# aaichert/EpipolarConsistency

Hardware: AMD Instinct MI355X
Metric: ECC evaluations/sec (N=400, 1024^2 projections) (higher is better)
Workload: dtype f32

## Files before the change

epipolarconsistency_amd/_lib.py:

```python
import ctypes as C
import os

_HERE = os.path.dirname(os.path.abspath(__file__))
LIB_PATH = os.environ.get("ECC_HIP_LIB") or os.path.join(_HERE, "libecc_hip.so")

ECC_OK = 0
FILTER_DERIVATIVE, FILTER_RAMP, FILTER_NONE = 0, 1, 2
POST_IDENTITY, POST_SQUARE_ROOT, POST_LOGARITHM = 0, 1, 2
RADON_EXACT, RADON_FMA = 0, 1
SAMPLING_AUTO, SAMPLING_POLYNOMIAL, SAMPLING_PER_SAMPLE, SAMPLING_REFERENCE = 0, 1, 2, 3
LOSS_HUBER, LOSS_TRUNCATED, LOSS_GEMAN_MCCLURE = 0, 1, 2


class EccError(RuntimeError):
    def __init__(self, code, message):
        super().__init__("libecc_hip error %d: %s" % (code, message))
        self.code = code


class PreprocessConfig(C.Structure):
    _fields_ = [("process", C.c_int32), ("normalize", C.c_int32), ("bias", C.c_double), ("scale", C.c_double),
                ("apply_log", C.c_int32), ("gaussian_sigma", C.c_double), ("half_kernel_width", C.c_int32),
                ("flip_u", C.c_int32), ("flip_v", C.c_int32), ("zero", C.c_int32 * 4), ("feather", C.c_int32 * 4),
                ("n_blanks", C.c_int32), ("blanks", C.c_void_p)]


class LineWeightsConfig(C.Structure):
    _fields_ = [("dilate_px", C.c_int32), ("guard_bins", C.c_int32), ("zero_at_px", C.c_float)]


_lib = None

_vp, _i, _i64, _d = C.c_void_p, C.c_int, C.c_int64, C.c_double
_pi, _pd, _pf = C.POINTER(C.c_int), C.POINTER(C.c_double), C.POINTER(C.c_float)
SIGNATURES = {
    "ecc_last_error": (C.c_char_p, []),
    "ecc_version": (_i, []),
    "ecc_device_count": (_i, []),
    "ecc_ctx_create": (_i, [_i, _vp, C.POINTER(_vp)]),
    "ecc_ctx_destroy": (_i, [_vp]),
    "ecc_ctx_synchronize": (_i, [_vp]),
    "ecc_radon_compute": (_i, [_vp, _vp, _i, _i, _i, _i, _i, _i, _i, C.POINTER(_vp)]),
    "ecc_radon_compute_batch": (_i, [_vp, _vp, _i, _i, _i, _i, _i, _i, _i, _i, C.POINTER(_vp)]),
    "ecc_radon_compute_into": (_i, [_vp, _vp, _i, _i, _i, _i, _i, _i, _i, _vp]),
    "ecc_radon_set_arithmetic": (_i, [_vp, _i]),
    "ecc_radon_get_arithmetic": (_i, [_vp, _pi]),
    "ecc_radon_compute_linear": (_i, [_vp, _vp, _i, _i, _i, _i, _i, _i, _vp]),
    "ecc_dtr_from_device_linear": (_i, [_vp, _vp, _i, _i, _i, _i, _i, C.POINTER(_vp)]),
    "ecc_metric_evaluate_external": (_i, [_vp, _i, _vp, _vp, _i, _vp, _vp, _vp, C.c_float, C.c_float, _i]),
    "ecc_dtr_from_host": (_i, [_vp, _vp, _i, _i, _i, _i, _i, C.POINTER(_vp)]),
    "ecc_dtr_readback": (_i, [_vp, _vp]),
    "ecc_dtr_info": (_i, [_vp, _pi, _pi, _pi, _pi, _pi, _pd, _pd]),
    "ecc_dtr_device_view": (_i, [_vp, C.POINTER(_vp), _pi, _pi]),
    "ecc_dtr_slab_floats": (_i64, [_i, _i]),
    "ecc_dtr_wrap_device": (_i, [_vp, _vp, _i, _i, _i, _i, _i, C.POINTER(_vp)]),
    "ecc_dtr_destroy": (_i, [_vp]),
    "ecc_line_weights_defaults": (None, [_vp]),
    "ecc_radon_line_weights": (_i, [_vp, _vp, _i, _i, _i, _i, _i, _i, _vp, C.POINTER(_vp)]),
    "ecc_radon_line_weights_into": (_i, [_vp, _vp, _i, _i, _i, _i, _i, _vp, _vp]),
    "ecc_dtr_line_weights": (_i, [_vp, _vp, _vp, C.POINTER(_vp)]),
    "ecc_metric_create": (_i, [_vp, _i, C.POINTER(_vp), C.POINTER(_vp)]),
    "ecc_metric_destroy": (_i, [_vp]),
    "ecc_metric_refresh_dtrs": (_i, [_vp, _i, _i]),
    "ecc_metric_set_projections": (_i, [_vp, _vp, _i]),
    "ecc_metric_debug_geometry": (_i, [_vp, _vp, _vp]),
    "ecc_metric_set_params": (_i, [_vp, _d, _d, _i]),
    "ecc_metric_set_sampling": (_i, [_vp, _i]),
    "ecc_metric_set_incremental": (_i, [_vp, _i]),
    "ecc_metric_set_record_reuse": (_i, [_vp, _i]),
    "ecc_metric_set_small_eval": (_i, [_vp, _i]),
    "ecc_metric_set_host_join": (_i, [_vp, _i]),
    "ecc_metric_publish_scalar": (_i, [_vp, _vp]),
    "ecc_metric_wait_scalar": (_i, [_vp, _pd]),
    "ecc_metric_last_evaluated_pairs": (_i, [_vp, C.POINTER(_i64)]),
    "ecc_metric_device_bytes": (_i, [_vp, C.POINTER(_i64), C.POINTER(_i64), C.POINTER(_i64)]),
    "ecc_metric_get_object_radius": (_i, [_vp, _pd]),
    "ecc_metric_evaluate_all": (_i, [_vp, _vp, _pd]),
    "ecc_metric_evaluate_poses": (_i, [_vp, _i, _vp, _i, _vp]),
    "ecc_metric_evaluate_poses_strided": (_i, [_vp, _i, _vp, _i, _i, _i, _vp]),
    "ecc_metric_evaluate_pose_deltas": (_i, [_vp, _i, _vp, _vp, _vp, _vp]),
    "ecc_metric_set_pose_batching": (_i, [_vp, _i]),
    "ecc_metric_last_batched_poses": (_i, [_vp, C.POINTER(_i64)]),
    "ecc_metric_evaluate_gradient": (_i, [_vp, _i, _i, _vp, _vp, _vp, _vp, _vp, _vp]),
    "ecc_metric_last_gradient_path": (_i, [_vp, C.POINTER(_i)]),
    "ecc_metric_evaluate_gram": (_i, [_vp, _i, _vp, _vp]),
    "ecc_metric_evaluate_view_coefficients": (_i, [_vp, _i, _vp, _pd, _vp, _vp]),
    "ecc_metric_evaluate_view_hessian": (_i, [_vp, _i, _vp, _vp]),
    "ecc_metric_evaluate_weighted": (_i, [_vp, _pd, _pd, _vp]),
    "ecc_metric_evaluate_weighted_pairs": (_i, [_vp, _vp, _i, _pd, _pd, _vp]),
    "ecc_metric_evaluate_weighted_pose_deltas": (_i, [_vp, _i, _vp, _vp, _vp, _vp, _vp]),
    "ecc_metric_evaluate_transforms": (_i, [_vp, _i, _i, _vp, _vp, _vp]),
    "ecc_metric_evaluate_weighted_transforms": (_i, [_vp, _i, _i, _vp, _vp, _vp, _vp]),
    "ecc_metric_evaluate_robust": (_i, [_vp, _i, C.c_float, _pd, _pd, _vp]),
    "ecc_metric_evaluate_robust_pairs": (_i, [_vp, _vp, _i, _i, C.c_float, _pd, _pd, _vp]),
    "ecc_host_robust_scale": (_d, [_vp, _i64, _d]),
    "ecc_metric_evaluate_robust_map": (_i, [_vp, _i, C.c_float, _vp, _i, _vp, _vp, _pd, _pd, _vp]),
    "ecc_metric_evaluate_robust_map_pairs": (_i, [_vp, _vp, _i, _i, C.c_float, _vp, _i, _vp, _vp, _pd, _pd, _vp]),
    "ecc_metric_robust_map_weights": (_i, [_vp, C.c_float, C.c_float, _vp]),
    "ecc_debug_robust_map_fixed": (_i, [_vp, _vp, _i64]),
    "ecc_metric_evaluate_weighted_robust_map": (_i, [_vp, _i, C.c_float, _vp, _i, _vp, _vp, _pd, _pd, _pd, _vp]),
    "ecc_metric_evaluate_weighted_robust_map_pairs": (_i, [_vp, _vp, _i, _i, C.c_float, _vp, _i, _vp, _vp, _pd, _pd, _pd, _vp]),
    "ecc_metric_weighted_robust_map_weights": (_i, [_vp, C.c_float, C.c_float, _vp]),
    "ecc_metric_evaluate_weighted_robust": (_i, [_vp, _i, C.c_float, _pd, _pd, _pd, _vp]),
    "ecc_metric_evaluate_weighted_robust_pairs": (_i, [_vp, _vp, _i, _i, C.c_float, _pd, _pd, _pd, _vp]),
    "ecc_host_weighted_robust_scale": (_d, [_vp, _i64, _d]),
    "ecc_metric_evaluate_robust_pose_deltas": (_i, [_vp, _i, _vp, _vp, _vp, _i, C.c_float, _vp, _vp]),
    "ecc_metric_evaluate_robust_transforms": (_i, [_vp, _i, _i, _vp, _i, C.c_float, _vp, _vp, _vp]),
    "ecc_metric_last_batched_transforms": (_i, [_vp, C.POINTER(_i64)]),
    "ecc_host_compose_transform": (None, [_vp, _vp, _vp]),
    "ecc_metric_evaluate_range": (_i, [_vp, _i64, _i64, _vp, _pd]),
    "ecc_metric_evaluate_range_async": (_i, [_vp, _i64, _i64, _vp, _vp]),
    "ecc_metric_evaluate_pairs": (_i, [_vp, _vp, _i, _vp, _pd]),
    "ecc_metric_debug_K01": (_i, [_vp, _i64, _i64, _vp]),
    "ecc_metric_debug_polynomials": (_i, [_vp, _i64, _i64, _vp]),
    "ecc_metric_pair_samples_bound": (_i, [_vp, _pi]),
    "ecc_metric_evaluate_for_image_pair": (_i, [_vp, _i, _i, _i, _pi, _vp, _vp, _vp, _vp, _vp, _vp, _pd]),
    "ecc_get_ij": (None, [_i64, _i, _pi, _pi]),
    "ecc_host_pinvT": (None, [_vp, _vp]),
    "ecc_host_source_position": (None, [_vp, _vp]),
    "ecc_host_object_radius": (_d, [_vp, _i, _i]),
    "ecc_direct_create": (_i, [_vp, _i, _vp, _i, _i, _i, C.POINTER(_vp)]),
    "ecc_direct_destroy": (_i, [_vp]),
    "ecc_direct_update_images": (_i, [_vp]),
    "ecc_direct_set_projections": (_i, [_vp, _vp, _i]),
    "ecc_direct_set_params": (_i, [_vp, _d, _d, _i]),
    "ecc_direct_get_object_radius": (_i, [_vp, _pd]),
    "ecc_direct_evaluate": (_i, [_vp, _vp, _pd]),
    "ecc_direct_lines_bound": (_i, [_vp, _pi]),
    "ecc_direct_evaluate_for_image_pair": (_i, [_vp, _i, _i, _i, _pi, _vp, _vp, _vp, _vp, _pd]),
    "ecc_direct_evaluate_for_image_pair_kappas": (_i, [_vp, _i, _i, _i, _vp, _vp, _vp, _vp, _pd]),
    "ecc_preprocess_defaults": (None, [_vp]),
    "ecc_preprocess": (_i, [_vp, _vp, _i, _vp, _i, _i, _i, _vp, _vp]),
    "ecc_host_intrinsics": (None, [_vp, _pf, _pf, _pf]),
    "ecc_host_angular_range": (None, [_vp, _vp, _d, _pd, _pd]),
    "ecc_host_angular_step": (_d, [_vp, _vp, _i, _i]),
    "ecc_host_iso_center": (None, [_vp, _i, _vp]),
    "ecc_host_line_to_sample_dtr": (_i, [_vp, C.c_float]),
    "ecc_group_create": (_i, [_i, _vp, C.POINTER(_vp)]),
    "ecc_group_destroy": (_i, [_vp]),
    "ecc_group_size": (_i, [_vp]),
    "ecc_group_ctx": (_i, [_vp, _i, C.POINTER(_vp)]),
    "ecc_group_radon_compute_batch": (_i, [_vp, _vp, _i, _i, _i, _i, _i, _i, _i, C.POINTER(_vp)]),
    "ecc_pair_shard": (None, [_i64, _i, _i, C.POINTER(_i64), C.POINTER(_i64)]),
    "ecc_pair_shards_balanced": (_i, [_vp, _i, _d, _i, _vp]),
    "ecc_metric_balanced_shards": (_i, [_vp, _i, _vp]),
    "ecc_comm_available": (_i, []),
    "ecc_comm_unique_id": (_i, [_vp]),
    "ecc_comm_create": (_i, [_vp, _vp, _i, _i, _vp]),
    "ecc_comm_destroy": (_i, [_vp]),
    "ecc_metric_evaluate_range_allreduce": (_i, [_vp, _vp, _i64, _i64, _vp]),
    "ecc_group_metric_rebalance": (_i, [_vp]),
    "ecc_group_metric_evaluate_poses": (_i, [_vp, _i, _vp, _i, _vp]),
    "ecc_group_metric_create": (_i, [_vp, _i, C.POINTER(_vp), C.POINTER(_vp)]),
    "ecc_group_debug_force_replica": (_i, [_i]),
    "ecc_group_metric_destroy": (_i, [_vp]),
    "ecc_group_metric_set_projections": (_i, [_vp, _vp, _i]),
    "ecc_group_metric_set_params": (_i, [_vp, _d, _d, _i]),
    "ecc_group_metric_set_sampling": (_i, [_vp, _i]),
    "ecc_group_metric_set_incremental": (_i, [_vp, _i]),
    "ecc_group_metric_get_object_radius": (_i, [_vp, _pd]),
    "ecc_group_metric_evaluate_all": (_i, [_vp, _vp, _pd]),
    "ecc_group_metric_rank_metric": (_i, [_vp, _i, C.POINTER(_vp)]),
    "ecc_exchange_open": (_i, [C.c_char_p, _i, _i, C.POINTER(C.c_void_p)]),
    "ecc_exchange_sum": (_i, [_vp, _d, _pd]),
    "ecc_exchange_close": (_i, [_vp]),
    "ecc_debug_set_poly_tolerance": (_i, [_vp, C.c_float]),
    "ecc_debug_set_small_eval_bound": (_i, [_vp, _i64]),
    "ecc_debug_set_result_polling": (_i, [_i]),
    "ecc_debug_set_quad_copies": (_i, [_vp, _i]),
    "ecc_debug_set_gradient_launch": (_i, [_vp, _i]),
    "ecc_ctx_set_quad_copies": (_i, [_vp, _i]),
    "ecc_debug_small_stamps": (_i, [_vp, _i]),
    "ecc_debug_step_stamps": (_i, [_vp, _vp]),
    "ecc_ctx_enable_timing": (_i, [_vp, _i]),
    "ecc_ctx_last_kernel_ms": (_i, [_vp, _i, _pf]),
}


def lib():
    global _lib
    if _lib is None:
        if not os.path.exists(LIB_PATH):
            raise ImportError(
                "%s is missing: build it with `python -m epipolarconsistency_amd.build` "
                "(hipcc, gfx950). There is no CPU fallback." % LIB_PATH)
        if not os.environ.get("ECC_NO_TORCH_PRELOAD"):
            try:
                import torch
                if torch.cuda.is_available():
                    torch.cuda.init()
            except ImportError:
                pass
        L = C.CDLL(LIB_PATH)
        for name, (res, args) in SIGNATURES.items():
            f = getattr(L, name)
            f.restype = res
            f.argtypes = args
        _lib = L
    return _lib


def check(code):
    if code != ECC_OK:
        raise EccError(code, lib().ecc_last_error().decode("utf-8", "replace"))
```

epipolarconsistency_amd/api.py:

```python
import ctypes as C

import numpy as np

from . import _lib
from ._lib import (FILTER_DERIVATIVE, FILTER_NONE, FILTER_RAMP, POST_IDENTITY, POST_LOGARITHM,
                   POST_SQUARE_ROOT, EccError, check)


def pack_projection_matrices(Ps):
    return _Ps_colmajor(Ps)


def _Ps_colmajor(Ps):
    A = np.asarray(Ps, dtype=np.float64).reshape(-1, 3, 4)
    return np.ascontiguousarray(A.transpose(0, 2, 1)).reshape(-1, 12)


def _is_torch(x):
    return type(x).__module__.startswith("torch")


class Context:

    def __init__(self, device=0, stream=None):
        self._h = C.c_void_p()
        check(_lib.lib().ecc_ctx_create(int(device), C.c_void_p(stream or 0), C.byref(self._h)))
        self.device = int(device)

    def synchronize(self):
        check(_lib.lib().ecc_ctx_synchronize(self._h))

    def enable_timing(self, on=True):
        check(_lib.lib().ecc_ctx_enable_timing(self._h, 1 if on else 0))

    def last_kernel_ms(self, which):
        ms = C.c_float()
        check(_lib.lib().ecc_ctx_last_kernel_ms(self._h, {"pairs": 0, "radon": 1, "preprocess": 2}[which], C.byref(ms)))
        return ms.value

    def debugSetQuadCopies(self, on=True):
        check(_lib.lib().ecc_debug_set_quad_copies(self._h, 1 if on else 0))
        return self

    def setQuadCopies(self, mode="auto"):
        check(_lib.lib().ecc_ctx_set_quad_copies(self._h, {"auto": -1, "off": 0, "on": 1}[mode]))
        return self

    def setRadonArithmetic(self, mode="exact"):
        check(_lib.lib().ecc_radon_set_arithmetic(self._h, {"exact": _lib.RADON_EXACT, "fma": _lib.RADON_FMA}[mode]))
        return self

    def getRadonArithmetic(self):
        v = C.c_int()
        check(_lib.lib().ecc_radon_get_arithmetic(self._h, C.byref(v)))
        return {_lib.RADON_EXACT: "exact", _lib.RADON_FMA: "fma"}[v.value]

    def close(self):
        if self._h:
            _lib.lib().ecc_ctx_destroy(self._h)
            self._h = C.c_void_p()

    def __del__(self):
        try:
            self.close()
        except Exception:
            pass


class PreProccess:

    class _NS:
        def __init__(self, **kw):
            self.__dict__.update(kw)

    def __init__(self):
        self.intensity = self._NS(normalize=False, bias=0.0, scale=1.0, apply_log=False)
        self.lowpass = self._NS(gaussian_sigma=1.84, half_kernel_width=5)
        self.image_geometry = self._NS(flip_u=False, flip_v=False)
        self.border = self._NS(zero=[1, 1, 1, 1], feather=[16, 16, 16, 16], blanks=[])

    def _config(self, process=True):
        cfg = _lib.PreprocessConfig()
        _lib.lib().ecc_preprocess_defaults(C.byref(cfg))
        cfg.process = 1 if process else 0
        cfg.normalize, cfg.bias, cfg.scale = int(self.intensity.normalize), self.intensity.bias, self.intensity.scale
        cfg.apply_log = int(self.intensity.apply_log)
        cfg.gaussian_sigma, cfg.half_kernel_width = self.lowpass.gaussian_sigma, int(self.lowpass.half_kernel_width)
        cfg.flip_u, cfg.flip_v = int(self.image_geometry.flip_u), int(self.image_geometry.flip_v)
        cfg.zero = (C.c_int32 * 4)(*[int(v) for v in self.border.zero])
        cfg.feather = (C.c_int32 * 4)(*[int(v) for v in self.border.feather])
        bl = np.ascontiguousarray(np.asarray(self.border.blanks, np.int32).reshape(-1, 4))
        cfg.n_blanks = len(bl)
        cfg.blanks = bl.ctypes.data if len(bl) else None
        return cfg, bl

    def _run(self, ctx, images, Ps, out, process):
        cfg, keep = self._config(process)
        Pp = None if Ps is None else _Ps_colmajor(Ps)
        if _is_torch(images):
            import torch
            assert images.dtype == torch.float32 and images.is_contiguous() and images.is_cuda and images.dim() == 3
            out = images if out is None else out
            assert out.shape == images.shape and out.is_contiguous() and out.is_cuda
            n, n_v, n_u = images.shape
            a, b, on_dev = images.data_ptr(), out.data_ptr(), 1
        else:
            images = np.ascontiguousarray(images, np.float32)
            assert images.ndim == 3
            out = np.empty_like(images) if out is None else out
            n, n_v, n_u = images.shape
            a, b, on_dev = images.ctypes.data, out.ctypes.data, 0
        assert Pp is None or len(Pp) == n
        check(_lib.lib().ecc_preprocess(ctx._h, C.c_void_p(a), on_dev, C.c_void_p(b), n, n_u, n_v, C.byref(cfg),
                                        C.c_void_p(Pp.ctypes.data) if Pp is not None else None))
        del keep
        return out

    def process(self, ctx, images, Ps=None, out=None):
        return self._run(ctx, images, Ps, out, True)

    def apply_weight_cos_principal_ray(self, ctx, images, Ps, out=None):
        return self._run(ctx, images, Ps, out, False)


class RadonIntermediate:
    Derivative, Ramp, None_ = FILTER_DERIVATIVE, FILTER_RAMP, FILTER_NONE
    Identity, SquareRoot, Logarithm = POST_IDENTITY, POST_SQUARE_ROOT, POST_LOGARITHM

    def __init__(self, ctx, handle):
        self.ctx = ctx
        self._h = handle
        self._keep = None

    @classmethod
    def compute(cls, ctx, image, size_alpha, size_t, filter=FILTER_DERIVATIVE, post_process=POST_IDENTITY):
        return cls.compute_batch(ctx, image[None] if not _is_torch(image) else image.unsqueeze(0),
                                 size_alpha, size_t, filter, post_process)[0]

    @classmethod
    def compute_batch(cls, ctx, images, size_alpha, size_t, filter=FILTER_DERIVATIVE, post_process=POST_IDENTITY):
        if _is_torch(images):
            import torch
            assert images.dtype == torch.float32 and images.is_contiguous() and images.is_cuda
            n, n_v, n_u = images.shape
            ptr, on_dev, keep = images.data_ptr(), 1, images
        else:
            keep = np.ascontiguousarray(images, np.float32)
            n, n_v, n_u = keep.shape
            ptr, on_dev = keep.ctypes.data, 0
        hs = (C.c_void_p * n)()
        check(_lib.lib().ecc_radon_compute_batch(ctx._h, C.c_void_p(ptr), on_dev, n, n_u, n_v, size_alpha,
                                                 size_t, filter, post_process, hs))
        if on_dev:
            ctx.synchronize()
        return [cls(ctx, C.c_void_p(h)) for h in hs]

    @classmethod
    def compute_into(cls, ctx, images, slabs, size_alpha, size_t, filter=FILTER_DERIVATIVE,
                     post_process=POST_IDENTITY):
        n, n_v, n_u = images.shape
        assert images.is_contiguous() and slabs.is_contiguous()
        assert slabs.shape[0] == n and slabs.shape[1] == slab_floats(size_alpha, size_t)
        check(_lib.lib().ecc_radon_compute_into(ctx._h, C.c_void_p(images.data_ptr()), n, n_u, n_v, size_alpha,
                                                size_t, filter, post_process, C.c_void_p(slabs.data_ptr())))
        return [cls.wrap_device(ctx, slabs[k], size_alpha, size_t, n_u, n_v, filter) for k in range(n)]

    @classmethod
    def from_host(cls, ctx, data, n_u, n_v, filter=FILTER_DERIVATIVE):
        data = np.ascontiguousarray(data, np.float32)
        n_t, n_alpha = data.shape
        h = C.c_void_p()
        check(_lib.lib().ecc_dtr_from_host(ctx._h, C.c_void_p(data.ctypes.data), n_alpha, n_t, n_u, n_v, filter,
                                           C.byref(h)))
        return cls(ctx, h)

    @classmethod
    def line_weights_from(cls, lengths_dtr, zero_at_px=1.0, guard_bins=1, ctx=None):
        ctx = lengths_dtr.ctx if ctx is None else ctx
        cfg = _line_weights_config(zero_at_px, guard_bins, 0)
        h = C.c_void_p()
        check(_lib.lib().ecc_dtr_line_weights(ctx._h, lengths_dtr._h, C.byref(cfg), C.byref(h)))
        return cls(ctx, h)

    @classmethod
    def load(cls, ctx, path):
        from . import nrrd
        data, info = nrrd.read_dtr(path)
        return cls.from_host(ctx, data, info["n_u"], info["n_v"], info["filter"]), info

    def save(self, path, projection_matrix=None):
        from . import nrrd
        nrrd.write_dtr(path, self.readback(), self.getOriginalImageSize(0), self.getOriginalImageSize(1),
                       self.getFilter(), projection_matrix)

    @classmethod
    def wrap_device(cls, ctx, slab, n_alpha, n_t, n_u, n_v, filter=FILTER_DERIVATIVE):
        h = C.c_void_p()
        check(_lib.lib().ecc_dtr_wrap_device(ctx._h, C.c_void_p(slab.data_ptr()), n_alpha, n_t, n_u, n_v, filter,
                                             C.byref(h)))
        r = cls(ctx, h)
        r._keep = slab
        return r

    def _info(self):
        a, t, u, v, f = (C.c_int() for _ in range(5))
        ba, bd = C.c_double(), C.c_double()
        check(_lib.lib().ecc_dtr_info(self._h, C.byref(a), C.byref(t), C.byref(u), C.byref(v), C.byref(f),
                                      C.byref(ba), C.byref(bd)))
        return a.value, t.value, u.value, v.value, f.value, ba.value, bd.value

    def getRadonBinNumber(self, dim):
        a, t = self._info()[:2]
        return t if dim else a

    def getOriginalImageSize(self, dim):
        u, v = self._info()[2:4]
        return v if dim else u

    def getRadonBinSize(self, dim=1):
        ba, bd = self._info()[5:7]
        return bd if dim else ba

    def getFilter(self):
        return self._info()[4]

    def isDerivative(self):
        return self.getFilter() == FILTER_DERIVATIVE

    def readback(self):
        a, t = self._info()[:2]
        out = np.empty((t, a), np.float32)
        check(_lib.lib().ecc_dtr_readback(self._h, C.c_void_p(out.ctypes.data)))
        self._raw_cpu = out
        return out

    def clearRawData(self):
        self._raw_cpu = None

    def data(self):
        return getattr(self, "_raw_cpu", None)

    def replaceRadonIntermediateData(self, radon_intermediate_image):
        a = np.ascontiguousarray(radon_intermediate_image, np.float32)
        assert a.ndim == 2
        info = self._info()
        fresh = RadonIntermediate.from_host(self.ctx, a, info[2], info[3], filter=info[4])
        self.close()
        self._h, fresh._h = fresh._h, C.c_void_p()
        self._keep = None
        self._raw_cpu = a.copy()

    def tex2D(self, s, t):
        raw = self.data()
        if raw is None:
            raise ValueError("call readback() first")
        n_t, n_alpha = raw.shape
        x, y = (n_alpha - 1) * float(np.float32(s)), (n_t - 1) * float(np.float32(t))

        def cell(v, n):
            i = int(v)
            f = v - i
            if i < 0:
                i, f = 0, 0.0
            if i > n - 2:
                i, f = n - 2, 1.0
            return i, f
        ix, fx = cell(x, n_alpha)
        iy, fy = cell(y, n_t)
        if fx == 0 and fy == 0:
            return float(np.float32(raw[iy, ix]))
        r = ((1.0 - fy) * ((1.0 - fx) * float(raw[iy, ix]) + fx * float(raw[iy, ix + 1]))
             + fy * ((1.0 - fx) * float(raw[iy + 1, ix]) + fx * float(raw[iy + 1, ix + 1])))
        return float(np.float32(r))

    def sample(self, line):
        l = np.ascontiguousarray(line, np.float32).reshape(3).copy()
        range_t = np.float32(self.getRadonBinSize(1)) * np.float32(self.getRadonBinNumber(1))
        folded = _lib.lib().ecc_host_line_to_sample_dtr(C.c_void_p(l.ctypes.data), C.c_float(float(range_t)))
        try:
            line[:3] = l
        except TypeError:
            pass
        v = self.tex2D(l[0], l[1])
        return -v if (folded and self.isDerivative()) else v

    def device_view(self):
        base, pitch, rows = C.c_void_p(), C.c_int(), C.c_int()
        check(_lib.lib().ecc_dtr_device_view(self._h, C.byref(base), C.byref(pitch), C.byref(rows)))
        return base.value, pitch.value, rows.value

    def close(self):
        if self._h and self.ctx._h:
            _lib.lib().ecc_dtr_destroy(self._h)
        self._h = C.c_void_p()

    def __del__(self):
        try:
            self.close()
        except Exception:
            pass


def _pack_pose_lists(moved_views, moved_Ps):
    off = [0]
    views = []
    rows = []
    for vk, Pk in zip(moved_views, moved_Ps):
        vk = [int(v) for v in np.atleast_1d(vk)]
        Pk = np.asarray(Pk, np.float64)
        Pk = Pk.reshape(len(vk), 12) if (Pk.shape[-1] == 12 and Pk.ndim <= 2) else _Ps_colmajor(Pk)
        views += vk
        rows.append(Pk)
        off.append(len(views))
    flat = np.concatenate(rows) if rows and len(views) else np.zeros((0, 12))
    return off, views, flat


def _check_pose_lists(moved_offsets, moved_views, moved_Ps):
    off = np.ascontiguousarray(moved_offsets, np.int32)
    views = np.ascontiguousarray(moved_views, np.int32)
    flat = np.ascontiguousarray(moved_Ps, np.float64).reshape(-1, 12)
    if len(off) < 1 or int(off[-1]) != len(views) or len(flat) != len(views):
        raise ValueError("moved_offsets / moved_views / moved_Ps disagree")
    return off, views, flat


def _ptr(a):
    return C.c_void_p(a.ctypes.data) if (a is not None and a.size) else None


def _idx4_list(idx4):
    idx = np.ascontiguousarray(idx4, np.int32)
    if idx.size % 4 or (idx.ndim == 2 and idx.shape[1] != 4) or idx.ndim > 2:
        raise ValueError("idx4 must hold (P0, P1, D0, D1) tuples")
    return idx.reshape(-1, 4)


def _transforms_colmajor(Ts):
    T = np.asarray(Ts, dtype=np.float64)
    if T.ndim == 2 and T.shape == (4, 4):
        T = T[None]
    if T.ndim != 3 or T.shape[1:] != (4, 4):
        raise ValueError("Ts must be (K, 4, 4)")
    return np.ascontiguousarray(T.transpose(0, 2, 1)).reshape(-1, 16)


def _with_pairs(results, pairs, want_pairs):
    return results + (pairs,) if want_pairs else results


def _pose_lists_call(fn, handle, moved_offsets, moved_views, moved_Ps, extra, n_results):
    off, views, flat = _check_pose_lists(moved_offsets, moved_views, moved_Ps)
    results = tuple(np.zeros(len(off) - 1, np.float64) for _ in range(n_results))
    check(fn(handle, len(off) - 1, C.c_void_p(off.ctypes.data), _ptr(views), _ptr(flat), *extra,
             *[C.c_void_p(r.ctypes.data) for r in results]))
    return results


class MetricRadonIntermediate:

    def __init__(self, ctx, Ps=None, dtrs=None):
        self.ctx = ctx
        self._h = C.c_void_p()
        self._dtrs = []
        self._Ps = None
        self._params = [0.0, 0.0, 0]
        d = type(self).default_sampling
        self._sampling = 0 if d is None else (self._SAMPLING[d] if isinstance(d, str) else int(d))
        self._incremental = False
        self._record_reuse = None
        self._small_eval = None
        self._host_join = None
        self._debug = {}
        self._ptr_cache = {}
        self._mean = C.c_double()
        self._mean_ref = C.byref(self._mean)
        if dtrs is not None:
            self.setRadonIntermediates(dtrs)
        if Ps is not None:
            self.setProjectionMatrices(Ps)

    def setRadonIntermediates(self, dtrs):
        if self._h:
            _lib.lib().ecc_metric_destroy(self._h)
            self._h = C.c_void_p()
        self._dtrs = list(dtrs)
        hs = (C.c_void_p * len(self._dtrs))(*[d._h for d in self._dtrs])
        check(_lib.lib().ecc_metric_create(self.ctx._h, len(self._dtrs), hs, C.byref(self._h)))
        check(_lib.lib().ecc_metric_set_params(self._h, *self._params))
        check(_lib.lib().ecc_metric_set_sampling(self._h, self._sampling))
        check(_lib.lib().ecc_metric_set_incremental(self._h, int(self._incremental)))
        if self._record_reuse is not None:
            check(_lib.lib().ecc_metric_set_record_reuse(self._h, int(self._record_reuse)))
        if self._small_eval is not None:
            check(_lib.lib().ecc_metric_set_small_eval(self._h, int(self._small_eval)))
        if self._host_join is not None:
            check(_lib.lib().ecc_metric_set_host_join(self._h, int(self._host_join)))
        self._apply_debug()
        if self._Ps is not None:
            self.setProjectionMatrices(self._Ps)
        return self

    def _apply_debug(self):
        if "poly_tolerance" in self._debug:
            check(_lib.lib().ecc_debug_set_poly_tolerance(self._h, float(self._debug["poly_tolerance"])))
        if "small_eval_bound" in self._debug:
            check(_lib.lib().ecc_debug_set_small_eval_bound(self._h, int(self._debug["small_eval_bound"])))
        if "gradient_launch" in self._debug:
            check(_lib.lib().ecc_debug_set_gradient_launch(self._h, int(self._debug["gradient_launch"])))

    def debugSetGradientLaunch(self, on=True):
        self._debug["gradient_launch"] = 1 if on else 0
        if self._h:
            self._apply_debug()
        return self

    def debugSetPolyTolerance(self, tol_bins):
        self._debug["poly_tolerance"] = float(tol_bins)
        if self._h:
            self._apply_debug()
        return self

    def debugSetSmallEvalBound(self, max_pairs):
        self._debug["small_eval_bound"] = int(max_pairs)
        if self._h:
            self._apply_debug()
        return self

    def getRadonIntermediates(self):
        return self._dtrs

    def refreshRadonIntermediates(self, first=0, count=None):
        count = len(self._dtrs) - first if count is None else count
        check(_lib.lib().ecc_metric_refresh_dtrs(self._h, int(first), int(count)))
        return self

    def setProjectionMatrices(self, Ps):
        hit = self._ptr_cache.get(id(Ps))
        if hit is not None and hit[0] is Ps and hit[2] == Ps.shape:
            self._Ps = Ps
            if self._h:
                check(_lib.lib().ecc_metric_set_projections(self._h, hit[1], hit[2][0]))
            return self
        if isinstance(Ps, np.ndarray) and Ps.ndim == 2 and Ps.shape[1] == 12 and Ps.dtype == np.float64 \
                and Ps.flags["C_CONTIGUOUS"]:
            self._Ps = Ps
            if len(self._ptr_cache) >= 1024:
                self._ptr_cache.clear()
            self._ptr_cache[id(Ps)] = (Ps, C.c_void_p(Ps.ctypes.data), Ps.shape)
        else:
            self._Ps = _Ps_colmajor(Ps)
        if self._h:
            check(_lib.lib().ecc_metric_set_projections(self._h, C.c_void_p(self._Ps.ctypes.data), len(self._Ps)))
        return self

    def getProjectionMatrices(self):
        return [] if self._Ps is None else [p.reshape(4, 3).T.copy() for p in self._Ps]

    def getNumberOfProjetions(self):
        return 0 if self._Ps is None else len(self._Ps)

    def _push_params(self):
        if self._h:
            check(_lib.lib().ecc_metric_set_params(self._h, *self._params))

    def setObjectRadius(self, radius_mm=0.0):
        self._params[0] = float(radius_mm)
        self._push_params()
        return self

    def getObjectRadius(self):
        r = C.c_double()
        check(_lib.lib().ecc_metric_get_object_radius(self._h, C.byref(r)))
        return r.value

    def setEpipolarPlaneStep(self, dkappa_rad=0.0):
        self._params[1] = float(dkappa_rad)
        self._push_params()
        return self

    setdKappa = setEpipolarPlaneStep

    def useCorrelation(self, corr=True):
        self._params[2] = 1 if corr else 0
        self._push_params()
        return self

    default_sampling = None
    _SAMPLING = {"auto": 0, "polynomial": 1, "per_sample": 2, "reference": 3}

    def setSampling(self, mode="auto"):
        self._sampling = self._SAMPLING[mode] if isinstance(mode, str) else int(mode)
        if self._h:
            check(_lib.lib().ecc_metric_set_sampling(self._h, self._sampling))
        return self

    def setIncremental(self, enable=True):
        self._incremental = bool(enable)
        if self._h:
            check(_lib.lib().ecc_metric_set_incremental(self._h, int(self._incremental)))
        return self

    def setRecordReuse(self, on=True, always=False):
        self._record_reuse = (2 if always else 1) if on else 0
        if self._h:
            check(_lib.lib().ecc_metric_set_record_reuse(self._h, int(self._record_reuse)))
        return self

    def setSmallEval(self, on=True):
        self._small_eval = 1 if on else 0
        if self._h:
            check(_lib.lib().ecc_metric_set_small_eval(self._h, self._small_eval))
        return self

    def setHostJoin(self, on=True):
        self._host_join = 1 if on else 0
        if self._h:
            check(_lib.lib().ecc_metric_set_host_join(self._h, self._host_join))
        return self

    def device_bytes(self):
        a, b, c = C.c_int64(0), C.c_int64(0), C.c_int64(0)
        check(_lib.lib().ecc_metric_device_bytes(self._h, C.byref(a), C.byref(b), C.byref(c)))
        return {"paired_copies": a.value, "quad_copies": b.value, "other": c.value}

    def last_evaluated_pairs(self):
        v = C.c_int64()
        check(_lib.lib().ecc_metric_last_evaluated_pairs(self._h, C.byref(v)))
        return v.value

    def evaluate(self, arg=None, out=None):
        L = _lib.lib()
        if arg is None:
            check(L.ecc_metric_evaluate_all(self._h, None, self._mean_ref))
            return self._mean.value
        mean = C.c_double()
        if arg is None or (isinstance(arg, np.ndarray) and arg.dtype == np.float32 and arg.ndim == 2
                           and out is None and arg.shape[0] == arg.shape[1] == self.getNumberOfProjetions()):
            cost = arg
            if cost is not None and not cost.flags["C_CONTIGUOUS"]:
                raise ValueError("cost image must be C-contiguous float32")
            check(L.ecc_metric_evaluate_all(self._h, C.c_void_p(cost.ctypes.data if cost is not None else 0),
                                            C.byref(mean)))
            return mean.value
        if isinstance(arg, (set, frozenset)):
            views = sorted(arg)
            idx = [(a, b, a, b) for k, a in enumerate(views) for b in views[k + 1:]]
        else:
            idx = arg
        hit_i, hit_o = self._ptr_cache.get(id(idx)), self._ptr_cache.get(id(out))
        if hit_i is not None and hit_o is not None and hit_i[0] is idx and hit_o[0] is out and hit_i[2] == idx.shape \
                and hit_o[2] == out.shape:
            check(L.ecc_metric_evaluate_pairs(self._h, hit_i[1], hit_i[2][0], hit_o[1], self._mean_ref))
            return self._mean.value
        cacheable = isinstance(idx, np.ndarray) and idx.dtype == np.int32 and idx.ndim == 2 and idx.shape[1] == 4 \
            and idx.flags["C_CONTIGUOUS"] and isinstance(out, np.ndarray) and out.flags["C_CONTIGUOUS"]
        idx0 = idx
        idx = np.ascontiguousarray(idx, np.int32).reshape(-1, 4)
        if out is None:
            out = np.empty(len(idx), np.float32)
        assert out.dtype == np.float32 and out.size >= len(idx)
        pi, po = C.c_void_p(idx.ctypes.data), C.c_void_p(out.ctypes.data)
        if cacheable:
            if len(self._ptr_cache) >= 1024:
                self._ptr_cache.clear()
            self._ptr_cache[id(idx0)] = (idx0, pi, idx0.shape)
            self._ptr_cache[id(out)] = (out, po, out.shape)
        check(L.ecc_metric_evaluate_pairs(self._h, pi, len(idx), po, C.byref(mean)))
        return mean.value

    def evaluate_poses(self, poses, first=0, stride=1):
        if isinstance(poses, np.ndarray) and poses.ndim == 3 and poses.shape[2] == 12 and poses.dtype == np.float64 \
                and poses.flags["C_CONTIGUOUS"]:
            flat = poses
        else:
            flat = np.ascontiguousarray(np.stack([p if (isinstance(p, np.ndarray) and p.ndim == 2 and p.shape[1] == 12)
                                                  else _Ps_colmajor(p) for p in poses]), np.float64)
        means = np.zeros(len(flat), np.float64)
        check(_lib.lib().ecc_metric_evaluate_poses_strided(self._h, len(flat), C.c_void_p(flat.ctypes.data), flat.shape[1],
                                                           int(first), int(stride), C.c_void_p(means.ctypes.data)))
        mine = range(int(first), len(flat), int(stride))
        if len(mine):
            self._Ps = flat[mine[-1]]
        return means

    def evaluate_pose_deltas(self, moved_views, moved_Ps):
        return self.evaluate_pose_deltas_packed(*_pack_pose_lists(moved_views, moved_Ps))

    def evaluate_pose_deltas_packed(self, moved_offsets, moved_views, moved_Ps):
        return _pose_lists_call(_lib.lib().ecc_metric_evaluate_pose_deltas, self._h, moved_offsets, moved_views, moved_Ps, (), 1)[0]

    def evaluate_weighted_pose_deltas(self, moved_views, moved_Ps):
        return self.evaluate_weighted_pose_deltas_packed(*_pack_pose_lists(moved_views, moved_Ps))

    def evaluate_weighted_pose_deltas_packed(self, moved_offsets, moved_views, moved_Ps):
        return _pose_lists_call(_lib.lib().ecc_metric_evaluate_weighted_pose_deltas, self._h, moved_offsets, moved_views, moved_Ps, (), 2)

    def evaluate_robust_pose_deltas(self, moved_views, moved_Ps, loss, delta):
        return self.evaluate_robust_pose_deltas_packed(*_pack_pose_lists(moved_views, moved_Ps), loss, delta)

    def evaluate_robust_pose_deltas_packed(self, moved_offsets, moved_views, moved_Ps, loss, delta):
        return _pose_lists_call(_lib.lib().ecc_metric_evaluate_robust_pose_deltas, self._h, moved_offsets, moved_views, moved_Ps,
                                (int(loss), float(delta)), 2)

    def evaluate_weighted_pairs(self, idx4, want_pairs=False):
        idx = _idx4_list(idx4)
        value, coverage = C.c_double(0.0), C.c_double(0.0)
        pairs = np.zeros((len(idx), 2), np.float32) if want_pairs else None
        check(_lib.lib().ecc_metric_evaluate_weighted_pairs(self._h, _ptr(idx), len(idx),
                                                            C.byref(value), C.byref(coverage),
                                                            _ptr(pairs)))
        return _with_pairs((value.value, coverage.value), pairs, want_pairs)

    def setPoseBatching(self, on=True):
        check(_lib.lib().ecc_metric_set_pose_batching(self._h, 1 if on else 0))
        return self

    def last_batched_poses(self):
        v = C.c_int64(0)
        check(_lib.lib().ecc_metric_last_batched_poses(self._h, C.byref(v)))
        return v.value

    def evaluate_gradient(self, view, Ps_plus, Ps_minus, h, want_probes=False):
        def rows(Ps):
            Ps = np.asarray(Ps, np.float64)
            return np.ascontiguousarray(Ps.reshape(-1, 12) if (Ps.shape[-1] == 12 and Ps.ndim <= 2) else _Ps_colmajor(Ps))
        plus, minus = rows(Ps_plus), rows(Ps_minus)
        h = np.ascontiguousarray(np.atleast_1d(h), np.float64)
        p = len(h)
        if p < 1 or len(plus) != p or len(minus) != p:
            raise ValueError("Ps_plus / Ps_minus / h disagree")
        value = C.c_double(0.0)
        grad, probes = np.zeros(p, np.float64), np.zeros(2 * p, np.float64)
        check(_lib.lib().ecc_metric_evaluate_gradient(self._h, int(view), p, C.c_void_p(plus.ctypes.data), C.c_void_p(minus.ctypes.data),
                                                      C.c_void_p(h.ctypes.data), C.byref(value), C.c_void_p(grad.ctypes.data),
                                                      C.c_void_p(probes.ctypes.data) if want_probes else None))
        return (value.value, grad, probes) if want_probes else (value.value, grad)

    def evaluate_gradient_rigid(self, view, steps, want_probes=False):
        from .geometry import compose_transform, rigid_transform
        steps = np.asarray(steps, np.float64)
        if steps.shape != (6,):
            raise ValueError("steps: (tx, ty, tz, rx, ry, rz)")
        if self._Ps is None or not 0 <= int(view) < len(self._Ps):
            raise ValueError("view outside the projection matrices")
        P = self._Ps[int(view)].reshape(4, 3).T
        names = ("tx", "ty", "tz", "rx", "ry", "rz")
        plus = [compose_transform(P, rigid_transform(**{names[k]: steps[k]})) for k in range(6)]
        minus = [compose_transform(P, rigid_transform(**{names[k]: -steps[k]})) for k in range(6)]
        return self.evaluate_gradient(view, plus, minus, steps, want_probes)

    def last_gradient_path(self):
        v = C.c_int(0)
        check(_lib.lib().ecc_metric_last_gradient_path(self._h, C.byref(v)))
        return v.value

    def evaluate_gram(self, n_channels, want_pairs=False):
        K = int(n_channels)
        n = 0 if self._Ps is None else len(self._Ps)
        G = np.zeros((max(K, 0), max(K, 0)), np.float64)
        pairs = np.zeros((n * (n - 1) // 2, max(K, 0) * (max(K, 0) + 1) // 2), np.float32) if want_pairs else None
        check(_lib.lib().ecc_metric_evaluate_gram(self._h, K, _ptr(pairs),
                                                  C.c_void_p(G.ctypes.data) if G.size else None))
        return (G, pairs) if want_pairs else G

    def evaluate_view_coefficients(self, coeffs, want_pairs=False):
        a = np.ascontiguousarray(coeffs, np.float32)
        if a.ndim != 2:
            raise ValueError("coeffs must be (n_channels, n_views)")
        K, n = a.shape
        if self._Ps is not None and n != len(self._Ps):
            raise ValueError("coeffs must be (n_channels, n_views)")
        value = C.c_double(0.0)
        grad = np.zeros((K, n), np.float64)
        pairs = np.zeros((n * (n - 1) // 2, 1 + 2 * K), np.float32) if want_pairs else None
        check(_lib.lib().ecc_metric_evaluate_view_coefficients(self._h, K, C.c_void_p(a.ctypes.data) if a.size else None, C.byref(value),
                                                               C.c_void_p(grad.ctypes.data) if grad.size else None,
                                                               _ptr(pairs)))
        return (value.value, grad, pairs) if want_pairs else (value.value, grad)

    def evaluate_view_hessian(self, n_channels, want_pairs=False, want_matrix=True):
        if not want_pairs and not want_matrix:
            raise ValueError("nothing asked for: want_matrix or want_pairs")
        K = int(n_channels)
        n = 0 if self._Ps is None else len(self._Ps)
        Kp = max(K, 0)
        H = np.zeros((n * Kp, n * Kp) if n * Kp else (1, 1), np.float64) if want_matrix else None
        blocks = None
        if want_pairs:
            blocks = np.zeros((n * (n - 1) // 2, Kp * (Kp + 1) + Kp * Kp) if n > 1 and Kp else (1, 1), np.float64)
        check(_lib.lib().ecc_metric_evaluate_view_hessian(self._h, K, C.c_void_p(H.ctypes.data) if want_matrix else None,
                                                          C.c_void_p(blocks.ctypes.data) if want_pairs else None))
        return (H, blocks) if (want_pairs and want_matrix) else (H if want_matrix else blocks)

    def evaluate_weighted(self, want_pairs=False):
        n = 0 if self._Ps is None else len(self._Ps)
        value, coverage = C.c_double(0.0), C.c_double(0.0)
        pairs = np.zeros((n * (n - 1) // 2, 2), np.float32) if want_pairs else None
        check(_lib.lib().ecc_metric_evaluate_weighted(self._h, C.byref(value), C.byref(coverage),
                                                      _ptr(pairs)))
        return _with_pairs((value.value, coverage.value), pairs, want_pairs)

    def evaluate_robust(self, loss, delta, want_pairs=False):
        n = 0 if self._Ps is None else len(self._Ps)
        value, mass = C.c_double(0.0), C.c_double(0.0)
        pairs = np.zeros((n * (n - 1) // 2, 3), np.float32) if want_pairs else None
        check(_lib.lib().ecc_metric_evaluate_robust(self._h, int(loss), float(delta), C.byref(value), C.byref(mass),
                                                    _ptr(pairs)))
        return _with_pairs((value.value, mass.value), pairs, want_pairs)

    def evaluate_robust_pairs(self, idx4, loss, delta, want_pairs=False):
        idx = _idx4_list(idx4)
        value, mass = C.c_double(0.0), C.c_double(0.0)
        pairs = np.zeros((len(idx), 3), np.float32) if want_pairs else None
        check(_lib.lib().ecc_metric_evaluate_robust_pairs(self._h, _ptr(idx), len(idx),
                                                          int(loss), float(delta), C.byref(value), C.byref(mass),
                                                          _ptr(pairs)))
        return _with_pairs((value.value, mass.value), pairs, want_pairs)

    def _robust_map_views(self, views):
        if views is None:
            return None, len(self._dtrs)
        v = np.ascontiguousarray(views, np.int32).reshape(-1)
        if len(v) == 0:
            raise ValueError("views: None for every view, or at least one index")
        return v, len(v)

    def _robust_map_planes(self, k):
        n_alpha, n_t = (self._dtrs[0].getRadonBinNumber(0), self._dtrs[0].getRadonBinNumber(1)) if self._dtrs else (0, 0)
        return np.zeros((k, n_t, n_alpha), np.float32), np.zeros((k, n_t, n_alpha), np.float32)

    def evaluate_robust_map(self, loss, delta, views=None, want_pairs=False):
        n = 0 if self._Ps is None else len(self._Ps)
        v, k = self._robust_map_views(views)
        if views is None:
            k = n
        hits, rejected = self._robust_map_planes(k)
        value, mass = C.c_double(0.0), C.c_double(0.0)
        pairs = np.zeros((n * (n - 1) // 2, 3), np.float32) if want_pairs else None
        check(_lib.lib().ecc_metric_evaluate_robust_map(self._h, int(loss), float(delta), _ptr(v), 0 if v is None else len(v),
                                                        _ptr(hits), _ptr(rejected), C.byref(value), C.byref(mass), _ptr(pairs)))
        self._robust_map_count = k
        return _with_pairs((value.value, mass.value, hits, rejected), pairs, want_pairs)

    def evaluate_robust_map_pairs(self, idx4, loss, delta, views=None, want_pairs=False):
        idx = _idx4_list(idx4)
        v, k = self._robust_map_views(views)
        hits, rejected = self._robust_map_planes(k)
        value, mass = C.c_double(0.0), C.c_double(0.0)
        pairs = np.zeros((len(idx), 3), np.float32) if want_pairs else None
        check(_lib.lib().ecc_metric_evaluate_robust_map_pairs(self._h, _ptr(idx), len(idx), int(loss), float(delta), _ptr(v),
                                                              0 if v is None else len(v), _ptr(hits), _ptr(rejected), C.byref(value),
                                                              C.byref(mass), _ptr(pairs)))
        self._robust_map_count = k
        return _with_pairs((value.value, mass.value, hits, rejected), pairs, want_pairs)

    def robust_map_weights(self, min_hits=1.0, gain=1.0):
        k = getattr(self, "_robust_map_count", 0)
        hs = (C.c_void_p * max(k, 1))()
        check(_lib.lib().ecc_metric_robust_map_weights(self._h, float(min_hits), float(gain), hs))
        return [RadonIntermediate(self.ctx, C.c_void_p(h)) for h in hs[:k]]

    def robust_map_fixed(self):
        k = getattr(self, "_robust_map_count", 0)
        n_alpha, n_t = self._dtrs[0].getRadonBinNumber(0), self._dtrs[0].getRadonBinNumber(1)
        pitch = slab_floats(n_alpha, n_t) // (n_alpha + 2)
        raw = np.zeros((2 * max(k, 1), n_alpha + 2, pitch), np.uint64)
        check(_lib.lib().ecc_debug_robust_map_fixed(self._h, _ptr(raw), raw.size))
        q = raw[:, :, :n_t + 2].copy()
        q[:, 1] += q[:, 0]
        q[:, -2] += q[:, -1]
        q[:, :, 1] += q[:, :, 0]
        q[:, :, -2] += q[:, :, -1]
        bins = np.ascontiguousarray(q[:2 * k, 1:-1, 1:-1].transpose(0, 2, 1))
        return bins[:k], bins[k:]

    def _weighted_map_views(self, views):
        if views is None:
            return None, len(self._dtrs) // 2
        return self._robust_map_views(views)

    def evaluate_weighted_robust_map(self, loss, delta, views=None, want_pairs=False):
        n = 0 if self._Ps is None else len(self._Ps)
        v, k = self._weighted_map_views(views)
        hits, rejected = self._robust_map_planes(k)
        value, coverage, mass = C.c_double(0.0), C.c_double(0.0), C.c_double(0.0)
        pairs = np.zeros((n * (n - 1) // 2, 4), np.float32) if want_pairs else None
        check(_lib.lib().ecc_metric_evaluate_weighted_robust_map(self._h, int(loss), float(delta), _ptr(v), 0 if v is None else len(v),
                                                                 _ptr(hits), _ptr(rejected), C.byref(value), C.byref(coverage),
                                                                 C.byref(mass), _ptr(pairs)))
        self._robust_map_count = k
        return _with_pairs((value.value, coverage.value, mass.value, hits, rejected), pairs, want_pairs)

    def evaluate_weighted_robust_map_pairs(self, idx4, loss, delta, views=None, want_pairs=False):
        idx = _idx4_list(idx4)
        v, k = self._weighted_map_views(views)
        hits, rejected = self._robust_map_planes(k)
        value, coverage, mass = C.c_double(0.0), C.c_double(0.0), C.c_double(0.0)
        pairs = np.zeros((len(idx), 4), np.float32) if want_pairs else None
        check(_lib.lib().ecc_metric_evaluate_weighted_robust_map_pairs(self._h, _ptr(idx), len(idx), int(loss), float(delta), _ptr(v),
                                                                       0 if v is None else len(v), _ptr(hits), _ptr(rejected),
                                                                       C.byref(value), C.byref(coverage), C.byref(mass), _ptr(pairs)))
        self._robust_map_count = k
        return _with_pairs((value.value, coverage.value, mass.value, hits, rejected), pairs, want_pairs)

    def weighted_robust_map_weights(self, min_hits=1.0, gain=1.0):
        k = getattr(self, "_robust_map_count", 0)
        hs = (C.c_void_p * max(k, 1))()
        check(_lib.lib().ecc_metric_weighted_robust_map_weights(self._h, float(min_hits), float(gain), hs))
        return [RadonIntermediate(self.ctx, C.c_void_p(h)) for h in hs[:k]]

    def evaluate_weighted_robust(self, loss, delta, want_pairs=False):
        n = 0 if self._Ps is None else len(self._Ps)
        value, coverage, mass = C.c_double(0.0), C.c_double(0.0), C.c_double(0.0)
        pairs = np.zeros((n * (n - 1) // 2, 4), np.float32) if want_pairs else None
        check(_lib.lib().ecc_metric_evaluate_weighted_robust(self._h, int(loss), float(delta), C.byref(value), C.byref(coverage), C.byref(mass),
                                                             _ptr(pairs)))
        return _with_pairs((value.value, coverage.value, mass.value), pairs, want_pairs)

    def evaluate_weighted_robust_pairs(self, idx4, loss, delta, want_pairs=False):
        idx = _idx4_list(idx4)
        value, coverage, mass = C.c_double(0.0), C.c_double(0.0), C.c_double(0.0)
        pairs = np.zeros((len(idx), 4), np.float32) if want_pairs else None
        check(_lib.lib().ecc_metric_evaluate_weighted_robust_pairs(self._h, _ptr(idx), len(idx),
                                                                   int(loss), float(delta), C.byref(value), C.byref(coverage), C.byref(mass),
                                                                   _ptr(pairs)))
        return _with_pairs((value.value, coverage.value, mass.value), pairs, want_pairs)

    def evaluate_transforms(self, n_source, Ts, want_pairs=False):
        flat = _transforms_colmajor(Ts)
        n_source = int(n_source)
        K, n = len(flat), self.getNumberOfProjetions()
        means = np.zeros(K, np.float64)
        pairs = np.zeros((K, max(n - n_source, 0), max(n_source, 0)), np.float32) if want_pairs else None
        check(_lib.lib().ecc_metric_evaluate_transforms(self._h, n_source, K, C.c_void_p(flat.ctypes.data if K else 0),
                                                        C.c_void_p(means.ctypes.data if K else 0),
                                                        _ptr(pairs)))
        return (means, pairs) if want_pairs else means

    def evaluate_weighted_transforms(self, n_source, Ts, want_pairs=False):
        flat = _transforms_colmajor(Ts)
        n_source = int(n_source)
        K, n = len(flat), self.getNumberOfProjetions()
        values, coverages = np.zeros(K, np.float64), np.zeros(K, np.float64)
        pairs = np.zeros((K, max(n - n_source, 0), max(n_source, 0), 2), np.float32) if want_pairs else None
        check(_lib.lib().ecc_metric_evaluate_weighted_transforms(self._h, n_source, K, C.c_void_p(flat.ctypes.data if K else 0),
                                                                 C.c_void_p(values.ctypes.data if K else 0),
                                                                 C.c_void_p(coverages.ctypes.data if K else 0),
                                                                 _ptr(pairs)))
        return _with_pairs((values, coverages), pairs, want_pairs)

    def evaluate_robust_transforms(self, n_source, Ts, loss, delta, want_pairs=False):
        flat = _transforms_colmajor(Ts)
        n_source = int(n_source)
        K, n = len(flat), self.getNumberOfProjetions()
        values, masses = np.zeros(K, np.float64), np.zeros(K, np.float64)
        pairs = np.zeros((K, max(n - n_source, 0), max(n_source, 0), 3), np.float32) if want_pairs else None
        check(_lib.lib().ecc_metric_evaluate_robust_transforms(self._h, n_source, K, C.c_void_p(flat.ctypes.data if K else 0),
                                                               int(loss), float(delta),
                                                               C.c_void_p(values.ctypes.data if K else 0),
                                                               C.c_void_p(masses.ctypes.data if K else 0),
                                                               _ptr(pairs)))
        return _with_pairs((values, masses), pairs, want_pairs)

    def last_batched_transforms(self):
        v = C.c_int64(0)
        check(_lib.lib().ecc_metric_last_batched_transforms(self._h, C.byref(v)))
        return v.value

    def evaluateForImagePair(self, i, j):
        L = _lib.lib()
        cap = C.c_int()
        check(L.ecc_metric_pair_samples_bound(self._h, C.byref(cap)))
        cap = cap.value
        s0, s1, kap = (np.empty(cap, np.float32) for _ in range(3))
        r0, r1 = np.empty((cap, 2), np.float32), np.empty((cap, 2), np.float32)
        K01 = np.empty(16, np.float32)
        n, ecc = C.c_int(), C.c_double()
        check(L.ecc_metric_evaluate_for_image_pair(
            self._h, int(i), int(j), cap, C.byref(n), C.c_void_p(s0.ctypes.data), C.c_void_p(s1.ctypes.data),
            C.c_void_p(kap.ctypes.data), C.c_void_p(r0.ctypes.data), C.c_void_p(r1.ctypes.data),
            C.c_void_p(K01.ctypes.data), C.byref(ecc)))
        n = n.value
        return ecc.value, dict(redundant_samples0=s0[:n], redundant_samples1=s1[:n], kappas=kap[:n],
                               radon_samples0=r0[:n], radon_samples1=r1[:n], K01=K01)

    def balanced_shards(self, world):
        b = np.zeros(int(world) + 1, np.int64)
        check(_lib.lib().ecc_metric_balanced_shards(self._h, int(world), C.c_void_p(b.ctypes.data)))
        return [int(v) for v in b]

    def evaluate_range(self, first, count, want_pairs=False):
        s = C.c_double()
        vals = np.empty(count, np.float32) if want_pairs else None
        check(_lib.lib().ecc_metric_evaluate_range(self._h, int(first), int(count),
                                                   C.c_void_p(vals.ctypes.data if want_pairs else 0), C.byref(s)))
        return (s.value, vals) if want_pairs else s.value

    def evaluate_range_allreduce(self, comm, first, count):
        check(_lib.lib().ecc_metric_evaluate_range_allreduce(self._h, comm._h, int(first), int(count), self._mean_ref))
        return self._mean.value

    def evaluate_range_async(self, first, count, sum_tensor, pair_tensor=None):
        check(_lib.lib().ecc_metric_evaluate_range_async(
            self._h, int(first), int(count), C.c_void_p(pair_tensor.data_ptr() if pair_tensor is not None else 0),
            C.c_void_p(sum_tensor.data_ptr())))

    def publish_scalar(self, value_tensor):
        check(_lib.lib().ecc_metric_publish_scalar(self._h, C.c_void_p(value_tensor.data_ptr())))

    def wait_scalar(self):
        v = C.c_double()
        check(_lib.lib().ecc_metric_wait_scalar(self._h, C.byref(v)))
        return v.value

    def debug_geometry(self):
        n = self.getNumberOfProjetions()
        PinvTs, Cs = np.empty((n, 12), np.float32), np.empty((n, 4), np.float32)
        check(_lib.lib().ecc_metric_debug_geometry(self._h, C.c_void_p(PinvTs.ctypes.data), C.c_void_p(Cs.ctypes.data)))
        return PinvTs, Cs

    def debug_K01(self, first, count):
        out = np.empty((count, 16), np.float32)
        check(_lib.lib().ecc_metric_debug_K01(self._h, int(first), int(count), C.c_void_p(out.ctypes.data)))
        return out

    def debug_polynomials(self, first, count):
        n = 4 + 2 * 13 + 2 * 12
        out = np.empty((count, n), np.float32)
        check(_lib.lib().ecc_metric_debug_polynomials(self._h, int(first), int(count), C.c_void_p(out.ctypes.data)))
        return [dict(poly_ok=bool(r[0]), degree=int(r[0]), clamp_free=bool(r[0] != int(r[0])), x_scale=float(r[1]), fold=r[2:4] > 0, ca=r[4:30].reshape(2, 13).astype(np.float64),
                     cd=r[30:54].reshape(2, 12).astype(np.float64)) for r in out]

    def close(self):
        if self._h and self.ctx._h:
            _lib.lib().ecc_metric_destroy(self._h)
        self._h = C.c_void_p()

    def __del__(self):
        try:
            self.close()
        except Exception:
            pass


class _BorrowedContext:

    def __init__(self, handle, device, group):
        self._h, self.device, self._group = handle, device, group

    def synchronize(self):
        check(_lib.lib().ecc_ctx_synchronize(self._h))

    def close(self):
        self._h = C.c_void_p()


class Group:

    def __init__(self, devices):
        devices = [int(d) for d in devices]
        arr = (C.c_int * len(devices))(*devices)
        self._h = C.c_void_p()
        check(_lib.lib().ecc_group_create(len(devices), arr, C.byref(self._h)))
        self.devices = devices
        self._ctxs = {}

    def __len__(self):
        return _lib.lib().ecc_group_size(self._h)

    def context(self, rank):
        if rank not in self._ctxs:
            h = C.c_void_p()
            check(_lib.lib().ecc_group_ctx(self._h, int(rank), C.byref(h)))
            self._ctxs[rank] = _BorrowedContext(h, self.devices[rank], self)
        return self._ctxs[rank]

    def compute_batch(self, images, size_alpha, size_t, filter=FILTER_DERIVATIVE, post_process=POST_IDENTITY):
        keep = np.ascontiguousarray(images, np.float32)
        n, n_v, n_u = keep.shape
        hs = (C.c_void_p * n)()
        check(_lib.lib().ecc_group_radon_compute_batch(self._h, C.c_void_p(keep.ctypes.data), n, n_u, n_v, size_alpha,
                                                       size_t, filter, post_process, hs))
        chunk = (n + len(self.devices) - 1) // len(self.devices)
        ctxs = [self.context(r) for r in range(len(self.devices))]
        return [RadonIntermediate(ctxs[k // chunk], C.c_void_p(h)) for k, h in enumerate(hs)]

    def close(self):
        if self._h:
            for c in self._ctxs.values():
                c.close()
            self._ctxs = {}
            _lib.lib().ecc_group_destroy(self._h)
            self._h = C.c_void_p()

    def __del__(self):
        try:
            self.close()
        except Exception:
            pass


def pair_shard(n_pairs, world, rank):
    a, b = C.c_int64(), C.c_int64()
    _lib.lib().ecc_pair_shard(int(n_pairs), int(world), int(rank), C.byref(a), C.byref(b))
    return a.value, b.value


def pair_shards_balanced(Ps, object_radius_mm, world):
    if isinstance(Ps, np.ndarray) and Ps.ndim == 2 and Ps.shape[1] == 12:
        flat = np.ascontiguousarray(Ps, np.float64)
    else:
        flat = _Ps_colmajor(Ps)
    b = np.zeros(int(world) + 1, np.int64)
    check(_lib.lib().ecc_pair_shards_balanced(C.c_void_p(flat.ctypes.data), len(flat), float(object_radius_mm), int(world),
                                              C.c_void_p(b.ctypes.data)))
    return [int(v) for v in b]


class GroupMetricRadonIntermediate:

    def __init__(self, group, Ps=None, dtrs=None):
        self.group = group
        self._h = C.c_void_p()
        self._dtrs = []
        self._Ps = None
        if dtrs is not None:
            self.setRadonIntermediates(dtrs)
        if Ps is not None:
            self.setProjectionMatrices(Ps)

    def setRadonIntermediates(self, dtrs):
        self.close()
        self._dtrs = list(dtrs)
        hs = (C.c_void_p * len(self._dtrs))(*[d._h for d in self._dtrs])
        check(_lib.lib().ecc_group_metric_create(self.group._h, len(self._dtrs), hs, C.byref(self._h)))
        d = MetricRadonIntermediate.default_sampling
        if d is not None:
            self.setSampling(d)
        if self._Ps is not None:
            self.setProjectionMatrices(self._Ps)
        return self

    def setProjectionMatrices(self, Ps):
        if isinstance(Ps, np.ndarray) and Ps.ndim == 2 and Ps.shape[1] == 12 and Ps.dtype == np.float64 \
                and Ps.flags["C_CONTIGUOUS"]:
            self._Ps = Ps
        else:
            self._Ps = _Ps_colmajor(Ps)
        if self._h:
            check(_lib.lib().ecc_group_metric_set_projections(self._h, C.c_void_p(self._Ps.ctypes.data), len(self._Ps)))
        return self

    def getNumberOfProjetions(self):
        return 0 if self._Ps is None else len(self._Ps)

    def setObjectRadius(self, radius_mm=0.0, dkappa=0.0, use_corr=False):
        check(_lib.lib().ecc_group_metric_set_params(self._h, float(radius_mm), float(dkappa), 1 if use_corr else 0))
        return self

    def getObjectRadius(self):
        r = C.c_double()
        check(_lib.lib().ecc_group_metric_get_object_radius(self._h, C.byref(r)))
        return r.value

    def setSampling(self, mode="auto"):
        mode = MetricRadonIntermediate._SAMPLING[mode] if isinstance(mode, str) else int(mode)
        check(_lib.lib().ecc_group_metric_set_sampling(self._h, mode))
        return self

    def setIncremental(self, enable=True):
        check(_lib.lib().ecc_group_metric_set_incremental(self._h, int(bool(enable))))
        return self

    def last_evaluated_pairs(self):
        total = 0
        for r in range(len(self.group)):
            m, v = C.c_void_p(), C.c_int64()
            check(_lib.lib().ecc_group_metric_rank_metric(self._h, r, C.byref(m)))
            check(_lib.lib().ecc_metric_last_evaluated_pairs(m, C.byref(v)))
            total += v.value
        return total

    def evaluate_poses(self, poses):
        flat = np.ascontiguousarray(np.stack([p if (isinstance(p, np.ndarray) and p.ndim == 2 and p.shape[1] == 12)
                                              else _Ps_colmajor(p) for p in poses]), np.float64)
        means = np.zeros(len(flat), np.float64)
        check(_lib.lib().ecc_group_metric_evaluate_poses(self._h, len(flat), C.c_void_p(flat.ctypes.data), flat.shape[1],
                                                         C.c_void_p(means.ctypes.data)))
        return means

    def rebalance(self):
        check(_lib.lib().ecc_group_metric_rebalance(self._h))
        return self

    def evaluate(self, cost=None):
        mean = C.c_double()
        if cost is not None:
            n = self.getNumberOfProjetions()
            assert cost.dtype == np.float32 and cost.flags["C_CONTIGUOUS"] and cost.shape == (n, n)
        check(_lib.lib().ecc_group_metric_evaluate_all(self._h, C.c_void_p(cost.ctypes.data if cost is not None else 0),
                                                       C.byref(mean)))
        return mean.value

    def close(self):
        if self._h and self.group._h:
            _lib.lib().ecc_group_metric_destroy(self._h)
        self._h = C.c_void_p()

    def __del__(self):
        try:
            self.close()
        except Exception:
            pass


class MetricDirect:

    def __init__(self, ctx, Ps, images):
        self.ctx = ctx
        self._h = C.c_void_p()
        self._params = [0.0, 0.0, 0]
        self._Ps = None
        self.setProjectionImages(images)
        if Ps is not None:
            self.setProjectionMatrices(Ps)

    def setProjectionImages(self, images):
        if self._h:
            _lib.lib().ecc_direct_destroy(self._h)
            self._h = C.c_void_p()
        if _is_torch(images):
            import torch
            assert images.dtype == torch.float32 and images.is_contiguous() and images.is_cuda and images.dim() == 3
            self._keep, ptr, on_dev = images, images.data_ptr(), 1
        else:
            self._keep = np.ascontiguousarray(images, np.float32)
            assert self._keep.ndim == 3
            ptr, on_dev = self._keep.ctypes.data, 0
        n, n_v, n_u = self._keep.shape
        self._n = n
        check(_lib.lib().ecc_direct_create(self.ctx._h, n, C.c_void_p(ptr), on_dev, n_u, n_v, C.byref(self._h)))
        check(_lib.lib().ecc_direct_set_params(self._h, *self._params))
        if self._Ps is not None:
            self.setProjectionMatrices(self._Ps)
        return self

    def setProjectionMatrices(self, Ps):
        self._Ps = _Ps_colmajor(Ps)
        check(_lib.lib().ecc_direct_set_projections(self._h, C.c_void_p(self._Ps.ctypes.data), len(self._Ps)))
        return self

    def getNumberOfProjetions(self):
        return self._n

    def updateImages(self):
        check(_lib.lib().ecc_direct_update_images(self._h))
        return self

    def _push(self):
        check(_lib.lib().ecc_direct_set_params(self._h, *self._params))
        return self

    def setObjectRadius(self, radius_mm=0.0):
        self._params[0] = float(radius_mm)
        return self._push()

    def getObjectRadius(self):
        r = C.c_double()
        check(_lib.lib().ecc_direct_get_object_radius(self._h, C.byref(r)))
        return r.value

    def setEpipolarPlaneStep(self, dkappa_rad=0.0):
        self._params[1] = float(dkappa_rad)
        return self._push()

    def setFanBeamConsistency(self, fbcc=True):
        self._params[2] = 1 if fbcc else 0
        return self._push()

    def evaluate(self, cost=None):
        s = C.c_double()
        if cost is not None:
            assert cost.dtype == np.float32 and cost.flags["C_CONTIGUOUS"] and cost.shape == (self._n, self._n)
        check(_lib.lib().ecc_direct_evaluate(self._h, C.c_void_p(cost.ctypes.data if cost is not None else 0), C.byref(s)))
        return s.value

    def evaluateForImagePair(self, i, j, kappas=None):
        L = _lib.lib()
        if kappas is not None:
            kap = np.ascontiguousarray(kappas, np.float32).reshape(-1)
            s0, s1, lines = np.empty(len(kap), np.float32), np.empty(len(kap), np.float32), np.empty((len(kap), 6), np.float32)
            m = C.c_double()
            check(L.ecc_direct_evaluate_for_image_pair_kappas(self._h, int(i), int(j), len(kap), C.c_void_p(kap.ctypes.data),
                                                              C.c_void_p(s0.ctypes.data), C.c_void_p(s1.ctypes.data),
                                                              C.c_void_p(lines.ctypes.data), C.byref(m)))
            return m.value, dict(redundant_samples0=s0, redundant_samples1=s1, kappas=kap, lines=lines)
        cap = C.c_int()
        check(L.ecc_direct_lines_bound(self._h, C.byref(cap)))
        cap = cap.value
        s0, s1, kap = (np.empty(cap, np.float32) for _ in range(3))
        lines = np.empty((cap, 6), np.float32)
        n, m = C.c_int(), C.c_double()
        check(L.ecc_direct_evaluate_for_image_pair(self._h, int(i), int(j), cap, C.byref(n), C.c_void_p(s0.ctypes.data),
                                                   C.c_void_p(s1.ctypes.data), C.c_void_p(kap.ctypes.data),
                                                   C.c_void_p(lines.ctypes.data), C.byref(m)))
        n = n.value
        return m.value, dict(redundant_samples0=s0[:n], redundant_samples1=s1[:n], kappas=kap[:n], lines=lines[:n])

    def close(self):
        if self._h and self.ctx._h:
            _lib.lib().ecc_direct_destroy(self._h)
        self._h = C.c_void_p()

    def __del__(self):
        try:
            self.close()
        except Exception:
            pass


def slab_floats(n_alpha, n_t):
    return _lib.lib().ecc_dtr_slab_floats(int(n_alpha), int(n_t))


def get_ij(ij, n):
    i, j = C.c_int(), C.c_int()
    _lib.lib().ecc_get_ij(int(ij), int(n), C.byref(i), C.byref(j))
    return i.value, j.value


def host_pinvT(P):
    P = np.ascontiguousarray(np.asarray(P, np.float64).reshape(3, 4).T).reshape(12)
    out = np.empty(12, np.float32)
    _lib.lib().ecc_host_pinvT(C.c_void_p(P.ctypes.data), C.c_void_p(out.ctypes.data))
    return out


def host_source_position(P):
    P = np.ascontiguousarray(np.asarray(P, np.float64).reshape(3, 4).T).reshape(12)
    out = np.empty(4, np.float32)
    _lib.lib().ecc_host_source_position(C.c_void_p(P.ctypes.data), C.c_void_p(out.ctypes.data))
    return out


def host_object_radius(P, n_u, n_v):
    P = np.ascontiguousarray(np.asarray(P, np.float64).reshape(3, 4).T).reshape(12)
    return _lib.lib().ecc_host_object_radius(C.c_void_p(P.ctypes.data), int(n_u), int(n_v))


def host_intrinsics(P):
    P = np.ascontiguousarray(np.asarray(P, np.float64).reshape(3, 4).T).reshape(12)
    a, b, c = C.c_float(), C.c_float(), C.c_float()
    _lib.lib().ecc_host_intrinsics(C.c_void_p(P.ctypes.data), C.byref(a), C.byref(b), C.byref(c))
    return a.value, b.value, c.value


def _P12(P):
    return np.ascontiguousarray(np.asarray(P, np.float64).reshape(3, 4).T).reshape(12)


def estimateAngularRange(P0, P1, object_radius_mm):
    a, b, A, B = C.c_double(), C.c_double(), _P12(P0), _P12(P1)
    _lib.lib().ecc_host_angular_range(C.c_void_p(A.ctypes.data), C.c_void_p(B.ctypes.data), float(object_radius_mm),
                                      C.byref(a), C.byref(b))
    return a.value, b.value


def estimateAngularStep(P0, P1, n_u, n_v):
    A, B = _P12(P0), _P12(P1)
    return _lib.lib().ecc_host_angular_step(C.c_void_p(A.ctypes.data), C.c_void_p(B.ctypes.data), int(n_u), int(n_v))


def estimateIsoCenter(Ps):
    flat = _Ps_colmajor(Ps)
    O = np.zeros(4)
    _lib.lib().ecc_host_iso_center(C.c_void_p(flat.ctypes.data), len(flat), C.c_void_p(O.ctypes.data))
    return O


estimateObjectRadius = host_object_radius


def gram_value(G, a):
    G = np.asarray(G, np.float64)
    a = np.asarray(a, np.float64).reshape(-1)
    if G.ndim != 2 or G.shape != (len(a), len(a)):
        raise ValueError("G must be (K, K) and a (K,)")
    return float(a @ (G @ a))


def gram_minimizer(G, fixed=0, value=1.0):
    G = np.asarray(G, np.float64)
    if G.ndim != 2 or G.shape[0] != G.shape[1] or G.shape[0] < 1:
        raise ValueError("G must be (K, K)")
    K = G.shape[0]
    fixed = int(fixed)
    if not 0 <= fixed < K:
        raise ValueError("fixed outside [0, K)")
    free = [c for c in range(K) if c != fixed]
    a = np.zeros(K, np.float64)
    a[fixed] = float(value)
    if free:
        H = 0.5 * (G[np.ix_(free, free)] + G[np.ix_(free, free)].T)
        np.linalg.cholesky(H)
        a[free] = np.linalg.solve(H, -float(value) * 0.5 * (G[free, fixed] + G[fixed, free]))
    return a, gram_value(G, a)


def minimize_view_coefficients(metric, K, start, free, tol=1e-4, max_iter=None):
    a = np.array(start, np.float64)
    mask = np.asarray(free, bool)
    if a.ndim != 2 or a.shape[0] != int(K) or mask.shape != a.shape:
        raise ValueError("start and free must be (K, n_views)")
    n_free = int(mask.sum())
    if max_iter is None:
        max_iter = 2 * n_free + 10

    def gradient(coeffs):
        value, grad = metric.evaluate_view_coefficients(coeffs)[:2]
        return float(value), np.asarray(grad, np.float64)[mask]
    value, g0 = gradient(a)
    scale = float(np.max(np.abs(g0))) if n_free else 0.0
    iterations = 0
    if scale == 0.0:
        return a, value, iterations
    r = -g0
    p = r.copy()
    rr = float(r @ r)
    direction = np.zeros_like(a)
    while np.max(np.abs(r)) > tol * scale:
        if iterations >= max_iter:
            raise RuntimeError("minimize_view_coefficients: %d products did not reach the tolerance" % iterations)
        direction[mask] = p
        Hp = gradient(direction)[1]
        iterations += 1
        pHp = float(p @ Hp)
        if not pHp > 0.0:
            raise np.linalg.LinAlgError("the metric has no minimum over the free coefficients: a direction with p . H p <= 0")
        alpha = rr / pHp
        a[mask] += alpha * p
        r -= alpha * Hp
        rr_new = float(r @ r)
        p = r + (rr_new / rr) * p
        rr = rr_new
    return a, metric.evaluate_view_coefficients(a)[0], iterations


def line_weights_from_lengths(lengths, zero_at_px=1.0, guard_bins=1):
    L = np.asarray(lengths, np.float32)
    if L.ndim != 2:
        raise ValueError("lengths must be (n_t, n_alpha)")
    if not zero_at_px > 0:
        raise ValueError("zero_at_px must be positive")
    g = int(guard_bins)
    if g < 0:
        raise ValueError("guard_bins must not be negative")
    w = np.clip(np.float32(1.0) - L / np.float32(zero_at_px), np.float32(0.0), np.float32(1.0)).astype(np.float32)
    if g:
        padded = np.pad(w, g, mode="edge")
        n_t, n_alpha = w.shape
        out = w
        for dj in range(2 * g + 1):
            for di in range(2 * g + 1):
                out = np.minimum(out, padded[dj:dj + n_t, di:di + n_alpha])
        w = out
    return np.ascontiguousarray(w, np.float32)


def line_weights(ctx, flagged, size_alpha, size_t, zero_at_px=1.0, guard_bins=1):
    arr = np.asarray(flagged, np.float32)
    single = arr.ndim == 2
    if arr.ndim not in (2, 3):
        raise ValueError("flagged must be (n_v, n_u) or (n, n_v, n_u)")
    stack = arr[None] if single else arr
    n_v, n_u = stack.shape[1:]
    out = []
    for d in RadonIntermediate.compute_batch(ctx, stack, size_alpha, size_t, FILTER_NONE, POST_IDENTITY):
        w = line_weights_from_lengths(d.readback(), zero_at_px, guard_bins)
        d.close()
        out.append(RadonIntermediate.from_host(ctx, w, n_u, n_v, FILTER_NONE))
    return out[0] if single else out


def robust_scale(pair_terms, k=1.0):
    rows = np.ascontiguousarray(pair_terms, np.float32)
    if rows.ndim != 2 or rows.shape[1] != 3:
        raise ValueError("pair_terms must be (n_pairs, 3) rows {c, u, r}")
    return float(_lib.lib().ecc_host_robust_scale(C.c_void_p(rows.ctypes.data) if len(rows) else None, len(rows), float(k)))


def weighted_robust_scale(pair_terms, k=1.0):
    rows = np.ascontiguousarray(pair_terms, np.float32)
    if rows.ndim != 2 or rows.shape[1] != 4:
        raise ValueError("pair_terms must be (n_pairs, 4) rows {c, u, k, r}")
    return float(_lib.lib().ecc_host_weighted_robust_scale(C.c_void_p(rows.ctypes.data) if len(rows) else None, len(rows), float(k)))


def refine_line_weights(ctx, Ps, data, weights=None, loss=_lib.LOSS_TRUNCATED, k=0.5, passes=2, min_hits=1.0, gain=1.0, sampling="auto"):
    data = list(data)
    n = len(data)
    if int(passes) < 1:
        raise ValueError("passes must be at least 1")
    if weights is not None and len(weights) != n:
        raise ValueError("weights: one intermediate per view, or None")
    current, owned = (None if weights is None else list(weights)), False
    delta, records = None, []
    try:
        for _ in range(int(passes)):
            m = MetricRadonIntermediate(ctx, Ps, data if current is None else data + current).setSampling(sampling)
            try:
                if current is None:
                    delta = robust_scale(m.evaluate_robust(loss, float("inf"), want_pairs=True)[2], k)
                    _, mass, hits, rej = m.evaluate_robust_map(loss, delta)
                    coverage, new = 1.0, m.robust_map_weights(min_hits, gain)
                else:
                    if delta is None:
                        delta = weighted_robust_scale(m.evaluate_weighted_robust(loss, float("inf"), want_pairs=True)[3], k)
                    _, coverage, mass, hits, rej = m.evaluate_weighted_robust_map(loss, delta)
                    new = m.weighted_robust_map_weights(min_hits, gain)
            finally:
                m.close()
            if owned:
                for w in current:
                    w.close()
            current, owned = new, True
            h, r = hits.astype(np.float64).sum(axis=(1, 2)), rej.astype(np.float64).sum(axis=(1, 2))
            records.append(dict(delta=delta, coverage=coverage, inlier_mass=mass, rejected_share=np.where(h > 0, r / np.where(h > 0, h, 1.0), 0.0)))
    except BaseException:
        if owned:
            for w in current:
                w.close()
        raise
    return current, records


def _line_weights_config(zero_at_px, guard_bins, dilate_px):
    cfg = _lib.LineWeightsConfig()
    _lib.lib().ecc_line_weights_defaults(C.byref(cfg))
    cfg.zero_at_px, cfg.guard_bins, cfg.dilate_px = float(zero_at_px), int(guard_bins), int(dilate_px)
    return cfg


def line_weights_device(ctx, flagged, size_alpha, size_t, zero_at_px=1.0, guard_bins=1, dilate_px=0, out=None):
    cfg = _line_weights_config(zero_at_px, guard_bins, dilate_px)
    if _is_torch(flagged):
        import torch
        assert flagged.dtype == torch.float32 and flagged.is_contiguous() and flagged.is_cuda
        stack, on_dev = flagged, 1
    else:
        stack, on_dev = np.ascontiguousarray(flagged, np.float32), 0
    if len(stack.shape) not in (2, 3):
        raise ValueError("flagged must be (n_v, n_u) or (n, n_v, n_u)")
    single = len(stack.shape) == 2
    if single:
        stack = stack[None]
    n, n_v, n_u = (int(v) for v in stack.shape)
    ptr = stack.data_ptr() if on_dev else stack.ctypes.data
    if out is not None:
        if not on_dev:
            raise ValueError("out= needs flagged on the device")
        assert out.is_contiguous() and out.is_cuda and tuple(out.shape) == (n, slab_floats(size_alpha, size_t))
        check(_lib.lib().ecc_radon_line_weights_into(ctx._h, C.c_void_p(ptr), n, n_u, n_v, size_alpha, size_t, C.byref(cfg),
                                                     C.c_void_p(out.data_ptr())))
        made = [RadonIntermediate.wrap_device(ctx, out[k], size_alpha, size_t, n_u, n_v, FILTER_NONE) for k in range(n)]
    else:
        hs = (C.c_void_p * n)()
        check(_lib.lib().ecc_radon_line_weights(ctx._h, C.c_void_p(ptr), on_dev, n, n_u, n_v, size_alpha, size_t, C.byref(cfg), hs))
        if on_dev:
            ctx.synchronize()
        made = [RadonIntermediate(ctx, C.c_void_p(h)) for h in hs]
    return made[0] if single else made


def view_hessian_value(H, a):
    H = np.asarray(H, np.float64)
    a = np.asarray(a, np.float64).reshape(-1)
    if H.ndim != 2 or H.shape != (len(a), len(a)):
        raise ValueError("H must be (n K, n K) and a hold n K coefficients")
    return float(a @ (H @ a))


def view_hessian_minimizer(H, start, free):
    H = np.asarray(H, np.float64)
    a = np.array(start, np.float64)
    mask = np.asarray(free, bool)
    if a.ndim != 2 or mask.shape != a.shape or H.shape != (a.size, a.size):
        raise ValueError("start and free must be (K, n_views) and H (n K, n K)")
    F = mask.reshape(-1)
    if F.any():
        flat = a.reshape(-1)
        HFF = 0.5 * (H[np.ix_(F, F)] + H[np.ix_(F, F)].T)
        np.linalg.cholesky(HFF)
        flat[F] = np.linalg.solve(HFF, -0.5 * (H[np.ix_(F, ~F)] + H[np.ix_(~F, F)].T) @ flat[~F])
    return a, view_hessian_value(H, a)
```

epipolarconsistency_amd/csrc/ecc_capi.hip:

```cpp
#include "ecc_capi_internal.h"

#include <condition_variable>
#include <mutex>
#include <thread>

#define ECC_EXPORT extern "C" __attribute__((visibility("default")))

namespace {
thread_local std::string g_last_error;
}

extern "C" int ecc_set_error(int code, const char* msg)
{
    g_last_error = msg ? msg : "";
    return code;
}

namespace ecc_internal {

constexpr double ECC_SPIN_SECONDS = 2.0;

double now_seconds()
{
    return std::chrono::duration<double>(std::chrono::steady_clock::now().time_since_epoch()).count();
}

hipError_t wait_stream_spin(hipStream_t stream)
{
    double t0 = 0.0;
    for (unsigned spins = 0;; ++spins) {
        const hipError_t e = hipStreamQuery(stream);
        if (e != hipErrorNotReady) return e;
        if ((spins & 0x3ff) == 0x3ff) {
            const double t = now_seconds();
            if (t0 == 0.0) t0 = t;
            else if (t - t0 > ECC_SPIN_SECONDS) return hipStreamSynchronize(stream);
        }
    }
}

constexpr uint64_t ECC_RESULT_PENDING = 0x7ff8ecc0dead0001ull;

std::atomic<bool> g_result_polling{true};
bool result_polling_enabled() { return g_result_polling.load(std::memory_order_relaxed); }

void arm_result(ecc_metric* m)
{
    if (m->small_pending_count > 0) {
        (void)hipStreamSynchronize(m->ctx->stream);
        m->small_pending_count = 0;
    }
    reinterpret_cast<volatile uint64_t*>(m->sum_h.host)[0] = ECC_RESULT_PENDING;
    std::atomic_thread_fence(std::memory_order_seq_cst);
}

hipError_t wait_result(ecc_metric* m, hipStream_t stream, double* value)
{
    if (!result_polling_enabled()) {
        const hipError_t e = wait_stream_spin(stream);
        std::memcpy(value, m->sum_h.host, sizeof(double));
        return e;
    }
    const volatile uint64_t* slot = reinterpret_cast<const volatile uint64_t*>(m->sum_h.host);
    double t0 = 0.0;
    for (unsigned spins = 0;; ++spins) {
        const uint64_t bits = *slot;
        if (bits != ECC_RESULT_PENDING) {
            std::memcpy(value, &bits, sizeof(double));
            return hipSuccess;
        }
        if ((spins & 0xfff) == 0xfff) {
            const double t = now_seconds();
            if (t0 == 0.0) t0 = t;
            else if (t - t0 > ECC_SPIN_SECONDS) {
                const hipError_t e = hipStreamSynchronize(stream);
                const uint64_t b2 = *slot;
                std::memcpy(value, &b2, sizeof(double));
                if (e == hipSuccess && b2 == ECC_RESULT_PENDING) return hipErrorUnknown;
                return e;
            }
        }
    }
}

int set_device(const ecc_ctx* ctx)
{
    HIP_TRY(hipSetDevice(ctx->device));
    return ECC_OK;
}

int ensure_poly_tables(ecc_ctx* ctx)
{
    if (ctx->poly_d) return ECC_OK;
    constexpr int N = ECC_POLY_DEG + 1;
    EccPolyTables t;
    for (int j = 0; j < N; ++j) t.nodes[j] = std::cos(3.14159265358979323846 * (j + 0.5) / N);
    const double checks[ECC_POLY_CHECKS] = {-1.0, 0.13, 1.0};
    for (int j = 0; j < ECC_POLY_CHECKS; ++j) t.checks[j] = checks[j];
    constexpr int H = ECC_POLY_DEG / 2;
    auto invert_vandermonde = [&](int n, double* out) {
        long double M[H + 1][2 * (H + 1)];
        for (int j = 0; j < n; ++j) {
            const long double z = (long double)t.nodes[j] * (long double)t.nodes[j];
            long double pw = 1;
            for (int k = 0; k < n; ++k) {
                M[j][k] = pw;
                pw *= z;
                M[j][n + k] = j == k ? 1 : 0;
            }
        }
        for (int col = 0; col < n; ++col) {
            int piv = col;
            for (int r = col + 1; r < n; ++r)
                if (fabsl(M[r][col]) > fabsl(M[piv][col])) piv = r;
            for (int k = 0; k < 2 * n; ++k) std::swap(M[col][k], M[piv][k]);
            const long double d = M[col][col];
            for (int k = 0; k < 2 * n; ++k) M[col][k] /= d;
            for (int r = 0; r < n; ++r) {
                if (r == col) continue;
                const long double f = M[r][col];
                for (int k = 0; k < 2 * n; ++k) M[r][k] -= f * M[col][k];
            }
        }
        for (int k = 0; k < n; ++k)
            for (int j = 0; j < n; ++j) out[k * n + j] = (double)M[k][n + j];
    };
    t.nodes[H] = 0.0;
    invert_vandermonde(H + 1, t.Ae);
    invert_vandermonde(H, t.Ao);
    for (int k = 0; k <= ECC_TRIG_STEPS; ++k) {
        const double a = 3.14159265358979323846 * k / (2.0 * ECC_TRIG_STEPS);
        t.sc[k][0] = k == 0 ? 0.0 : k == ECC_TRIG_STEPS ? 1.0 : std::sin(a);
        t.sc[k][1] = k == 0 ? 1.0 : k == ECC_TRIG_STEPS ? 0.0 : std::cos(a);
    }
    HIP_TRY(hipMalloc((void**)&ctx->poly_d, sizeof(EccPolyTables)));
    HIP_TRY(hipMemcpyAsync(ctx->poly_d, &t, sizeof(t), hipMemcpyHostToDevice, ctx->stream));
    HIP_TRY(hipStreamSynchronize(ctx->stream));
    return ECC_OK;
}

}

using namespace ecc_internal;
ECC_EXPORT const char* ecc_last_error(void) { return g_last_error.c_str(); }

ECC_EXPORT int ecc_version(void) { return ECC_HIP_VERSION; }
ECC_EXPORT int ecc_device_count(void)
{
    int n = 0;
    if (hipGetDeviceCount(&n) != hipSuccess) {
        (void)hipGetLastError();
        return 0;
    }
    return n;
}

ECC_EXPORT int ecc_host_line_to_sample_dtr(float* line, float range_t)
{
    const float Pi = 3.14159265359f;
    const float length = std::sqrt(line[0] * line[0] + line[1] * line[1]);
    line[0] = (float)std::atan2((double)line[1], (double)line[0]) / Pi;
    if (line[0] < 0) line[0] += 2;
    line[1] = -(line[2] / length) / range_t + 0.5f;
    if (line[0] > 1) {
        line[0] = line[0] - 1.f;
        line[1] = 1.f - line[1];
        return 1;
    }
    return 0;
}

ECC_EXPORT void ecc_get_ij(int64_t ij, int n, int* i, int* j)
{
    double nn = (double)n - 0.5;
    int64_t r = (int64_t)std::floor(nn - std::sqrt(nn * nn - 2.0 * (double)ij));
    if (r < 0) r = 0;
    if (r > n - 2) r = n - 2;
    while (r > 0 && r * n - r * (r + 1) / 2 > ij) --r;
    while ((r + 1) * n - (r + 1) * (r + 2) / 2 <= ij) ++r;
    *i = (int)r;
    *j = (int)(ij - (r * n - r * (r + 1) / 2) + r + 1);
}
ECC_EXPORT void ecc_host_pinvT(const double* P, float* PinvT12) { ecc_host::pinv_transpose(P, PinvT12); }
ECC_EXPORT void ecc_host_source_position(const double* P, float* C4) { ecc_host::source_position(P, C4); }
ECC_EXPORT double ecc_host_object_radius(const double* P, int n_u, int n_v)
{
    return ecc_host::object_radius(P, n_u, n_v);
}

ECC_EXPORT int ecc_ctx_create(int device, void* stream, ecc_ctx** out)
{
    if (!out) return fail(ECC_ERR_INVALID_ARGUMENT, "out is null");
    int n = ecc_device_count();
    if (n <= 0) return fail(ECC_ERR_NO_DEVICE, "no HIP device visible; this library has no CPU fallback");
    if (device < 0 || device >= n) return fail(ECC_ERR_INVALID_ARGUMENT, "device index out of range");
    HIP_TRY(hipSetDevice(device));
    ecc_ctx* c = new (std::nothrow) ecc_ctx();
    if (!c) return fail(ECC_ERR_OUT_OF_MEMORY, "host allocation failed");
    c->device = device;
    c->stream = (hipStream_t)stream;
    *out = c;
    return ECC_OK;
}

ECC_EXPORT int ecc_ctx_destroy(ecc_ctx* ctx)
{
    if (!ctx) return ECC_OK;
    (void)hipSetDevice(ctx->device);
    (void)hipStreamSynchronize(ctx->stream);
    if (ctx->trig_d) (void)hipFree(ctx->trig_d);
    if (ctx->ramp_d) (void)hipFree(ctx->ramp_d);
    if (ctx->poly_d) (void)hipFree(ctx->poly_d);
    if (ctx->pre_tables_d) (void)hipFree(ctx->pre_tables_d);
    if (ctx->pre_tables_h) (void)hipHostFree(ctx->pre_tables_h);
    if (ctx->pre_ev) (void)hipEventDestroy(ctx->pre_ev);
    for (float* b : ctx->pre_scratch_d)
        if (b) (void)hipFree(b);
    if (ctx->radon_T_d) (void)hipFree(ctx->radon_T_d);
    if (ctx->linear_scratch_d) (void)hipFree(ctx->linear_scratch_d);
    if (ctx->line_weights_scratch_d) (void)hipFree(ctx->line_weights_scratch_d);
    for (auto& e : ctx->ev)
        if (e) (void)hipEventDestroy(e);
    delete ctx;
    return ECC_OK;
}

ECC_EXPORT int ecc_ctx_synchronize(ecc_ctx* ctx)
{
    if (!ctx) return fail(ECC_ERR_INVALID_ARGUMENT, "ctx is null");
    int rc = set_device(ctx);
    if (rc) return rc;
    HIP_TRY(hipStreamSynchronize(ctx->stream));
    return ECC_OK;
}

ECC_EXPORT int ecc_debug_set_result_polling(int on)
{
    g_result_polling.store(on != 0, std::memory_order_relaxed);
    return ECC_OK;
}

ECC_EXPORT int ecc_ctx_set_quad_copies(ecc_ctx* ctx, int mode)
{
    if (!ctx) return fail(ECC_ERR_INVALID_ARGUMENT, "context is null");
    if (mode != ECC_QUAD_COPIES_AUTO && mode != ECC_QUAD_COPIES_OFF && mode != ECC_QUAD_COPIES_ON)
        return fail(ECC_ERR_INVALID_ARGUMENT, "quad-copy mode must be ECC_QUAD_COPIES_AUTO, _OFF or _ON");
    ctx->quad_copies = mode;
    return ECC_OK;
}

ECC_EXPORT int ecc_debug_set_quad_copies(ecc_ctx* ctx, int on) { return ecc_ctx_set_quad_copies(ctx, on ? ECC_QUAD_COPIES_ON : ECC_QUAD_COPIES_OFF); }

ECC_EXPORT int ecc_ctx_enable_timing(ecc_ctx* ctx, int enable)
{
    if (!ctx) return fail(ECC_ERR_INVALID_ARGUMENT, "ctx is null");
    int rc = set_device(ctx);
    if (rc) return rc;
    if (enable)
        for (auto& e : ctx->ev)
            if (!e) HIP_TRY(hipEventCreate(&e));
    ctx->timing = enable != 0;
    ctx->ev_valid[0] = ctx->ev_valid[1] = ctx->ev_valid[2] = false;
    return ECC_OK;
}

ECC_EXPORT int ecc_ctx_last_kernel_ms(ecc_ctx* ctx, int which, float* ms)
{
    if (!ctx || !ms || which < 0 || which > 2) return fail(ECC_ERR_INVALID_ARGUMENT, "bad argument");
    if (!ctx->timing || !ctx->ev_valid[which]) return fail(ECC_ERR_INVALID_ARGUMENT, "no timed launch recorded");
    int rc = set_device(ctx);
    if (rc) return rc;
    HIP_TRY(hipEventSynchronize(ctx->ev[2 * which + 1]));
    HIP_TRY(hipEventElapsedTime(ms, ctx->ev[2 * which], ctx->ev[2 * which + 1]));
    return ECC_OK;
}
```

epipolarconsistency_amd/csrc/ecc_capi_internal.h:

```cpp
#ifndef ECC_CAPI_INTERNAL_H
#define ECC_CAPI_INTERNAL_H

#include <hip/hip_runtime.h>

#include <algorithm>
#include <atomic>
#include <chrono>
#include <cmath>
#include <cstdio>
#include <cstdlib>
#include <cstring>
#include <functional>
#include <limits>
#include <memory>
#include <new>
#include <string>
#include <vector>

#include "../../include/ecc_hip.h"
#include "ecc_host_geometry.h"
#include "ecc_layout.h"
#include "ecc_view_changes.h"

extern "C" hipError_t ecc_launch_radon(const EccRadonParams* p, int derivative, hipStream_t stream);
extern "C" hipError_t ecc_launch_dtr_border(float* slabs, int64_t slab_stride, int n_img, int n_alpha, int n_t,
                                            int pitch, hipStream_t stream);
extern "C" hipError_t ecc_launch_ramp(float* slabs, int64_t slab_stride, int n_img, int n_alpha, int n_t, int pitch,
                                      const double* h2_d, hipStream_t stream);
extern "C" hipError_t ecc_launch_dtr_import(const float* src, float* slab, int n_alpha, int n_t, int pitch,
                                            hipStream_t stream);
extern "C" hipError_t ecc_launch_dtr_export(const float* slab, float* dst, int n_alpha, int n_t, int pitch,
                                            hipStream_t stream);
extern "C" hipError_t ecc_launch_build_paired(const float* const* slabs_tbl_d, float* paired_d, int64_t paired_stride, int n,
                                              int rows, int pitch, hipStream_t stream);
extern "C" hipError_t ecc_launch_build_quad(const float* const* slabs_tbl_d, float* quads_d, int64_t quad_stride_floats, int n,
                                            int rows, int pitch, hipStream_t stream);
extern "C" hipError_t ecc_launch_k01(const EccPairParams* p, hipStream_t stream);
extern "C" hipError_t ecc_launch_k01_radii(const EccPairParams* p, const float* radii_d, int period, hipStream_t stream);
extern "C" hipError_t ecc_launch_k01_patched(const EccPairParams* p, const EccSmallEval* x, hipStream_t stream);
extern "C" hipError_t ecc_launch_pairs(const EccPairParams* p, hipStream_t stream);
extern "C" int ecc_small_eval_plan(const EccPairParams* p, long long forced_bound, int* wpp, size_t* lds_bytes);
extern "C" hipError_t ecc_launch_small_eval(const EccPairParams* p, const EccSmallEval* x, hipStream_t stream);
extern "C" int ecc_small_poses_plan(const EccPairParams* p, int Q, int* wpp, size_t* lds_bytes);
extern "C" hipError_t ecc_launch_small_poses(const EccPairParams* p, const EccSmallEval* x, const EccSmallPoses* y, hipStream_t stream);
extern "C" hipError_t ecc_launch_preprocess(const EccPreprocessParams* p, hipStream_t stream);
extern "C" size_t ecc_preprocess_lds_bytes(int k);
extern "C" hipError_t ecc_launch_direct_views(const double* Ps_d, int n, EccDirectView* views, int n_u, int n_v,
                                              hipStream_t stream);
extern "C" hipError_t ecc_launch_direct_transpose(const float* src, float* dst, int n, int W, int H, hipStream_t stream);
extern "C" hipError_t ecc_launch_direct_batch(const EccDirectParams* p, double* total, hipStream_t stream);
extern "C" hipError_t ecc_launch_pair_samples(const EccPairSamplesParams* p, hipStream_t stream);
extern "C" hipError_t ecc_launch_sum_pairs(const float* vals, long long count, double* out, void* scratch, hipStream_t stream);
extern "C" hipError_t ecc_launch_sum_pairs_to_host(const float* vals, long long count, double* out, float* values_host, hipStream_t stream);
extern "C" hipError_t ecc_launch_publish_scalar(const double* value_d, double* host_slot_dev, hipStream_t stream);
extern "C" size_t ecc_sum_scratch_bytes();
extern "C" hipError_t ecc_launch_pairs_weighted(const EccPairParams* p, const EccWeightedParams* g, hipStream_t stream);
extern "C" hipError_t ecc_launch_pairs_robust(const EccPairParams* p, const EccRobustParams* g, hipStream_t stream);
extern "C" hipError_t ecc_launch_pairs_weighted_robust(const EccPairParams* p, const EccWeightedRobustParams* g, hipStream_t stream);
extern "C" hipError_t ecc_launch_sum_weighted_poses(const float* base_cols, long long base_stride, long long count, int n, int Q,
                                                    const int32_t* lists_d, int K, const float* val_cols, long long vals_stride, int slices,
                                                    double* partial_d, double* out_host_dev, hipStream_t stream);
extern "C" hipError_t ecc_launch_sum_weighted_transforms(const float* val_cols, long long col_stride, long long count, int K, int slices,
                                                         double* partial_d, double* out_host_dev, hipStream_t stream);
extern "C" hipError_t ecc_launch_dilate_max(const float* src, float* dst, int64_t stride, int n_img, int n_u, int n_v, int radius,
                                            hipStream_t stream);
extern "C" hipError_t ecc_launch_clip_min(const float* lengths, int64_t lengths_stride, float* dst, int64_t dst_stride, int n_img,
                                          int n_alpha, int n_t, int pitch, int radius, float zero_at_px, hipStream_t stream);
extern "C" hipError_t ecc_launch_e1(const double* Ps_d, int n, float* PinvTs_d, float* Cs_d, hipStream_t stream);

#ifndef ECC_POSE_BATCH_MAX_ENTRIES
#define ECC_POSE_BATCH_MAX_ENTRIES (1 << 20)
#endif

#define ECC_EXPORT extern "C" __attribute__((visibility("default")))

extern "C" int ecc_set_error(int code, const char* msg);
namespace {
inline int fail(int code, const std::string& msg) { return ecc_set_error(code, msg.c_str()); }
}

#define HIP_TRY(expr)                                                                             \
    do {                                                                                          \
        hipError_t _e = (expr);                                                                   \
        if (_e != hipSuccess) {                                                                   \
            (void)hipGetLastError();                                                              \
            return fail(_e == hipErrorOutOfMemory ? ECC_ERR_OUT_OF_MEMORY : ECC_ERR_HIP,          \
                        std::string(#expr) + ": " + hipGetErrorString(_e));                       \
        }                                                                                         \
    } while (0)

struct EccSlab {
    float* ptr = nullptr;
    int device = 0;
    ~EccSlab()
    {
        if (ptr) {
            (void)hipSetDevice(device);
            (void)hipFree(ptr);
        }
    }
};
typedef EccSlab Slab;

struct ecc_ctx {
    int device = 0;
    hipStream_t stream = nullptr;
    bool timing = false;
    int radon_arithmetic = ECC_RADON_EXACT;
    int quad_copies = ECC_QUAD_COPIES_AUTO;
    hipEvent_t ev[6] = {nullptr, nullptr, nullptr, nullptr, nullptr, nullptr};
    bool ev_valid[3] = {false, false, false};
    float* trig_d = nullptr;
    int trig_n_alpha = 0;
    double* ramp_d = nullptr;
    int ramp_n_t = 0;
    EccPolyTables* poly_d = nullptr;
    char* pre_tables_d = nullptr;
    char* pre_tables_h = nullptr;
    size_t pre_tables_cap = 0;
    hipEvent_t pre_ev = nullptr;
    bool pre_ev_recorded = false;
    float* pre_scratch_d[2] = {nullptr, nullptr};
    size_t pre_scratch_cap[2] = {0, 0};
    float* radon_T_d = nullptr;
    size_t radon_T_cap = 0;
    float* linear_scratch_d = nullptr;
    size_t linear_scratch_cap = 0;
    float* line_weights_scratch_d = nullptr;
    size_t line_weights_scratch_cap = 0;
};

struct ecc_dtr {
    ecc_ctx* ctx = nullptr;
    std::shared_ptr<Slab> owner;
    float* base = nullptr;
    int n_alpha = 0, n_t = 0, n_u = 0, n_v = 0, filter = 0, pitch = 0;
};

namespace ecc_internal {
hipError_t wait_stream_spin(hipStream_t stream);

template <class T>
struct DeviceArray {
    T* ptr = nullptr;
    int64_t cap = 0;
    DeviceArray() = default;
    DeviceArray(const DeviceArray&) = delete;
    DeviceArray& operator=(const DeviceArray&) = delete;
    ~DeviceArray() { reset(); }
    void reset()
    {
        if (ptr) (void)hipFree((void*)ptr);
        ptr = nullptr;
        cap = 0;
    }
    int ensure(int64_t need, hipStream_t stream)
    {
        if (cap >= need && ptr) return ECC_OK;
        if (ptr) {
            HIP_TRY(hipStreamSynchronize(stream));
            HIP_TRY(hipFree((void*)ptr));
            ptr = nullptr;
            cap = 0;
        }
        HIP_TRY(alloc(need));
        return ECC_OK;
    }
    hipError_t alloc(int64_t n)
    {
        const hipError_t e = hipMalloc((void**)&ptr, (size_t)n * sizeof(T));
        if (e != hipSuccess) ptr = nullptr;
        cap = e == hipSuccess ? n : 0;
        return e;
    }
    int64_t bytes() const { return cap * (int64_t)sizeof(T); }
};

template <class T>
struct PinnedArray {
    T* host = nullptr;
    T* dev = nullptr;
    int64_t cap = 0;
    unsigned flags;
    explicit PinnedArray(unsigned alloc_flags = hipHostMallocMapped) : flags(alloc_flags) {}
    PinnedArray(const PinnedArray&) = delete;
    PinnedArray& operator=(const PinnedArray&) = delete;
    ~PinnedArray()
    {
        if (host) (void)hipHostFree(host);
    }
    int ensure(int64_t need, int64_t floor, hipStream_t stream)
    {
        if (cap >= need) return ECC_OK;
        if (host) {
            HIP_TRY(wait_stream_spin(stream));
            HIP_TRY(hipHostFree(host));
            host = dev = nullptr;
            cap = 0;
        }
        HIP_TRY(alloc(std::max<int64_t>(2 * need, floor)));
        return ECC_OK;
    }
    hipError_t alloc(int64_t n)
    {
        hipError_t e = hipHostMalloc((void**)&host, sizeof(T) * (size_t)n, flags);
        if (e != hipSuccess) host = nullptr;
        else e = hipHostGetDevicePointer((void**)&dev, host, 0);
        if (e == hipSuccess) cap = n;
        return e;
    }
};

template <class Key>
struct Kept {
    bool valid = false;
    int64_t first = 0, count = 0;
    int n_views = 0;
    Key key{};
    std::vector<double> Ps;
    bool matches(int64_t f, int64_t c, int n, const Key& k) const
    {
        return valid && first == f && count == c && n_views == n && key == k && (int64_t)Ps.size() == 12 * (int64_t)n;
    }
    void take(int64_t f, int64_t c, int n, const Key& k, const double* Pcur)
    {
        Ps.assign(Pcur, Pcur + 12 * (size_t)n);
        first = f;
        count = c;
        n_views = n;
        key = k;
    }
    void update(const std::vector<int>& views, const double* Pcur)
    {
        for (int v : views) std::memcpy(Ps.data() + 12 * (size_t)v, Pcur + 12 * (size_t)v, sizeof(double) * 12);
    }
};
struct RecordKey {
    int mode;
    float radius, dkappa, tol;
    bool operator==(const RecordKey& o) const { return mode == o.mode && radius == o.radius && dkappa == o.dkappa && tol == o.tol; }
};
struct ValueKey {
    int use_corr, sampling;
    double radius, dkappa;
    bool operator==(const ValueKey& o) const
    {
        return use_corr == o.use_corr && sampling == o.sampling && radius == o.radius && dkappa == o.dkappa;
    }
};
}

struct ecc_metric {
    template <class T>
    using DeviceArray = ecc_internal::DeviceArray<T>;
    template <class T>
    using PinnedArray = ecc_internal::PinnedArray<T>;
    ecc_ctx* ctx = nullptr;
    std::vector<ecc_dtr*> dtrs;
    int n_alpha = 0, n_t = 0, n_u = 0, n_v = 0, pitch = 0;
    bool is_derivative = true;
    float step_alpha = 0, step_t = 0;
    double object_radius_mm = 0, dkappa = 0;
    int use_corr = 0;
    int sampling = ECC_SAMPLING_AUTO;
    int n_views = 0;
    std::vector<double> P_first;
    DeviceArray<const float*> dtr_table_d;
    DeviceArray<float> paired_d;
    DeviceArray<const float*> paired_table_d;
    DeviceArray<float> quads_d;
    DeviceArray<const float*> quads_table_d;
    int64_t quad_floats = 0;
    std::vector<const float*> quads_table_h;
    bool quads_possible = false;
    bool quads_decided = true;
    DeviceArray<float> Cs_d;
    DeviceArray<float> PinvTs_d;
    int geom_capacity = 0;
    DeviceArray<float> pair_values_d;
    DeviceArray<float> cost_d;
    DeviceArray<int32_t> indices_d;
    DeviceArray<float> K01_d;
    DeviceArray<EccPairRecord> records_d;
    DeviceArray<double> sum_d;
    DeviceArray<char> sum_scratch_d;
    PinnedArray<double> Ps_h[2];
    uint64_t set_generation = 0;
    uint64_t done_generation = 0;
    PinnedArray<double> sum_h{hipHostMallocMapped | hipHostMallocCoherent};
    int incremental = 0;
    ecc_internal::Kept<ecc_internal::ValueKey> cache;
    DeviceArray<float> cache_values_d;
    PinnedArray<int32_t> list_h;
    std::vector<int> scratch_changed;
    ecc_view_changes::PairList scratch_pairs;
    int64_t last_evaluated_pairs = 0;
    int record_reuse = 1;
    bool e1_pending = false;
    std::vector<double> dev_Ps;
    bool dev_valid = false;
    mutable double radius_cache = 0.0;
    mutable double radius_cache_P[12] = {0};
    mutable bool radius_cache_valid = false;
    bool eager_e1 = false;
    ecc_internal::Kept<ecc_internal::RecordKey> rec;
    PinnedArray<int32_t> reuse_h[2];
    hipEvent_t reuse_ev[2] = {nullptr, nullptr};
    bool reuse_ev_used[2] = {false, false};
    uint64_t reuse_gen = 0;
    std::vector<int> scratch_patched;
    std::vector<int> scratch_stale;
    std::vector<int32_t> scratch_patch_of;
    hipStream_t side_stream = nullptr;
    hipEvent_t fork_ev = nullptr, join_ev = nullptr;
    int host_join = 1;
    bool quiet = false;
    uint64_t queue_seq = 0, publish_seq = 0, publish_generation = 0;
    int small_eval = 1;
    int64_t small_max_pairs = -1;
    float economise_tol = ECC_POLY_ECONOMISE_TOL_BINS;
    PinnedArray<int32_t> sidx_h;
    PinnedArray<float> svals_h;
    DeviceArray<unsigned> small_ticket_d;
    int64_t small_pending_count = 0;
    int pose_batching = 1;
    PinnedArray<char> pose_h;
    DeviceArray<float> pose_PinvTs_d;
    DeviceArray<float> pose_Cs_d;
    DeviceArray<int32_t> pose_idx_d;
    DeviceArray<EccPairRecord> pose_records_d;
    DeviceArray<float> pose_values_d;
    DeviceArray<double> pose_partial_d;
    DeviceArray<int32_t> pose_lists_d;
    int64_t last_batched_poses = 0;
    int gradient_launch = 0;
    int last_gradient_path = 0;
    DeviceArray<EccPairRecord> gram_records_d;
    DeviceArray<float> gram_values_d;
    DeviceArray<double> gram_partial_d;
    DeviceArray<float> coeff_d;
    DeviceArray<double> coeff_sums_d;
    DeviceArray<double> view_moments_d;
    DeviceArray<double> view_hessian_d;
    DeviceArray<float> transform_radii_d;
    int64_t last_batched_transforms = 0;
    DeviceArray<unsigned long long> map_fixed_d;
    DeviceArray<int32_t> map_slot_d;
    DeviceArray<float> map_planes_d;
    int map_n_mapped = 0;
    bool map_valid = false;
    bool map_weighted = false;
    int map_n_slots = 0;
    double stamps[ECC_STEP_STAMPS] = {0};
};

inline void ecc_mark_busy(ecc_metric* m)
{
    m->quiet = false;
    ++m->queue_seq;
}

inline void ecc_stamp(ecc_metric* m, int k)
{
    m->stamps[k] = std::chrono::duration<double>(std::chrono::steady_clock::now().time_since_epoch()).count();
}

namespace ecc_internal {

int radon_check_args(ecc_ctx* ctx, const float* image, int n, int n_u, int n_v, int n_alpha, int n_t, int filter, int post,
                     ecc_dtr** out);
int radon_launch_stack(ecc_ctx* ctx, const float* images_d, int n, int n_u, int n_v, int n_alpha, int n_t, int filter, int post,
                       float* slabs, int64_t slab_stride);
int make_weight_handles(ecc_ctx* ctx, const std::shared_ptr<Slab>& owner, int n, int n_alpha, int n_t, int n_u, int n_v, ecc_dtr** out);
void arm_result(ecc_metric* m);
hipError_t wait_result(ecc_metric* m, hipStream_t stream, double* value);
int set_device(const ecc_ctx* ctx);
int ensure_poly_tables(ecc_ctx* ctx);
void decide_quad_copies(ecc_metric* m);
int ensure_e1(ecc_metric* m);
int fill_pair_params(ecc_metric* m, EccPairParams* p, int64_t mode_count, bool need_e1 = true);
int launch_range(ecc_metric* m, int64_t first, int64_t count, float* pair_values_d, float* cost_d, float* K01_d, double* sum_d,
                 bool synchronous = false, bool host_join = false);
int evaluate_cached(ecc_metric* m, int64_t first, int64_t count, double* sum_d, float** vals_out);

int sum_poses(ecc_metric* m, const float* base_vals_d, int K, int Q, volatile uint64_t* out, double* out_dev, double* sums);
bool pose_keeps_radius(const ecc_metric* m, double base_radius, int c, const int32_t* views, const double* moved_Ps);
int check_lists(const ecc_metric* m, int n_poses, const int32_t* off, const int32_t* views);
int stage_pose_grid(ecc_metric* m, const double* base, int K, const int32_t* off, const int32_t* views, const double* moved_Ps,
                    int result_words, volatile uint64_t** out, double** out_dev);
hipError_t launch_pose_list(ecc_metric* m, int K, int Q, int result_words);
void arm_pose_results(volatile uint64_t* out, int K);
int wait_pose_results(ecc_ctx* ctx, volatile uint64_t* out, int K, double* sums, const char* batch_noun = "pose");
int pose_deltas_sequential(ecc_metric* m, const std::vector<int>& rest, const int32_t* off, const int32_t* views, const double* moved_Ps,
                           const std::function<int(int)>& evaluate_pose);
float radius_of_transform(const ecc_metric* m, const double* base, const double* T);
int stage_transform_grid(ecc_metric* m, const double* base, int n_source, int K, const double* Ts, int result_words,
                         volatile uint64_t** out, double** out_dev);
hipError_t launch_transform_list(ecc_metric* m, int n_source, int K, long long seg, int result_words);
int transforms_sequential(ecc_metric* m, const std::vector<double>& base, int n_source, int n_transforms, const double* Ts,
                          const std::function<int(int, const int32_t*, int)>& evaluate_list);
int transforms_batched(ecc_metric* m, int64_t count, int n_transforms, int64_t max_per_batch, const std::function<int(int64_t, int)>& run_batch);
int channel_form_check(const ecc_metric* m, int n_channels, const char* range_text, const char* corr_text);
int weighted_check(const ecc_metric* m);
int robust_check(const ecc_metric* m, const double* value, int loss, float delta);
int weighted_robust_check(const ecc_metric* m, const double* value, int loss, float delta);

template <class Params>
inline void set_channel_strides(const ecc_metric* m, Params* g)
{
    const int64_t n = m->n_views;
    const int64_t paired_bytes = (int64_t)(m->n_alpha + 1) * m->pitch * 2 * (int64_t)sizeof(float);
    g->paired_channel_bytes = n * paired_bytes;
    g->quad_channel_bytes = n * m->quad_floats * (int64_t)sizeof(float);
}

template <class Launch>
inline hipError_t launch_timed(ecc_ctx* ctx, Launch&& launch)
{
    if (ctx->timing) {
        const hipError_t e = hipEventRecord(ctx->ev[0], ctx->stream);
        if (e != hipSuccess) return e;
    }
    const hipError_t e = launch(ctx->stream);
    if (e != hipSuccess || !ctx->timing) return e;
    const hipError_t e1 = hipEventRecord(ctx->ev[1], ctx->stream);
    if (e1 == hipSuccess) ctx->ev_valid[0] = true;
    return e1;
}

inline hipError_t launch_pairs_timed(ecc_ctx* ctx, const EccPairParams* p, const EccSmallEval* x = nullptr)
{
    return launch_timed(ctx, [&](hipStream_t s) { return x ? ecc_launch_small_eval(p, x, s) : ecc_launch_pairs(p, s); });
}

}

#endif
```

epipolarconsistency_amd/csrc/ecc_pose_diff.h:

```cpp
#ifndef ECC_POSE_DIFF_H
#define ECC_POSE_DIFF_H

#include <algorithm>
#include <cstdint>
#include <cstring>
#include <thread>
#include <vector>

namespace ecc_pose_diff {

struct Result {
    std::vector<int32_t> off;
    std::vector<int32_t> views;
    std::vector<int> batch_pose;
    std::vector<int> rest;
};

inline void diff(const double* Ps_batch, int n_views, const std::vector<int>& mine, const double* base, int max_moved,
                 unsigned max_threads, Result* out)
{
    const size_t pose_doubles = 12 * (size_t)n_views, count = mine.size();
    const size_t bytes = count * pose_doubles * sizeof(double);
    const unsigned hw = std::max(1u, std::thread::hardware_concurrency());
    const size_t T = (bytes < ((size_t)4 << 20) || max_threads < 2) ? 1 : std::min<size_t>({(size_t)max_threads, (size_t)hw, count / 32 + 1});
    std::vector<std::vector<int32_t>> part_views(T);
    std::vector<std::vector<int32_t>> part_count(T);
    auto work = [&](size_t t) {
        const size_t lo = count * t / T, hi = count * (t + 1) / T;
        std::vector<int32_t>&pv = part_views[t], &pc = part_count[t];
        pc.reserve(hi - lo);
        for (size_t q = lo; q < hi; ++q) {
            const double* Pp = Ps_batch + pose_doubles * (size_t)mine[q];
            const size_t before = pv.size();
            for (int v0 = 0; v0 < n_views && pv.size() - before <= (size_t)max_moved; v0 += 8) {
                const int v1 = std::min(n_views, v0 + 8);
                if (std::memcmp(Pp + 12 * (size_t)v0, base + 12 * (size_t)v0, sizeof(double) * 12 * (size_t)(v1 - v0)) == 0) continue;
                for (int v = v0; v < v1; ++v)
                    if (std::memcmp(Pp + 12 * (size_t)v, base + 12 * (size_t)v, sizeof(double) * 12) != 0) pv.push_back(v);
            }
            if (pv.size() - before > (size_t)max_moved) {
                pv.resize(before);
                pc.push_back(-1);
            } else pc.push_back((int32_t)(pv.size() - before));
        }
    };
    if (T == 1) work(0);
    else {
        std::vector<std::thread> th;
        for (size_t t = 1; t < T; ++t) th.emplace_back(work, t);
        work(0);
        for (std::thread& x : th) x.join();
    }
    out->off.assign(1, 0);
    out->views.clear();
    out->batch_pose.clear();
    out->rest.clear();
    for (size_t t = 0; t < T; ++t) {
        const size_t lo = count * t / T;
        size_t at = 0;
        for (size_t q = 0; q < part_count[t].size(); ++q) {
            const int32_t c = part_count[t][q];
            if (c < 0) out->rest.push_back(mine[lo + q]);
            else {
                out->views.insert(out->views.end(), part_views[t].begin() + at, part_views[t].begin() + at + c);
                at += (size_t)c;
                out->batch_pose.push_back(mine[lo + q]);
                out->off.push_back((int32_t)out->views.size());
            }
        }
    }
}

}

#endif
```

epipolarconsistency_amd/csrc/ecc_poses.hip:

```cpp
#include "ecc_capi_internal.h"
#include "ecc_pose_batches.h"
#include "ecc_pose_diff.h"
#include "ecc_sum_order.h"

using namespace ecc_internal;

namespace {

constexpr int SUM_THREADS = ecc_sum::THREADS, SUM_SLICES = ecc_sum::SLICES;
constexpr int STAGE_F4 = 2 * SUM_THREADS;
constexpr size_t POSE_BATCH_MAX_POSES = (1 << 19) / SUM_SLICES;
static_assert(POSE_BATCH_MAX_POSES < 65536, "poses are the y dimension of sum_poses_kernel's grid");

struct PoseLists {
    const int32_t* off;
    const int32_t* views;
};

__global__ __launch_bounds__(256) void pose_list_kernel(PoseLists in, int n, int n_poses, int Q, int32_t* __restrict__ idx,
                                                        int32_t* __restrict__ lists_d, const double* __restrict__ Ps_ext,
                                                        float* __restrict__ PinvTs, float* __restrict__ Cs)
{
    __shared__ int M[ECC_POSE_BATCH_MAX_MOVED];
    if ((int)blockIdx.x >= n_poses) {
        const int role = threadIdx.x >> 6;
        const int v = ((int)blockIdx.x - n_poses) * 64 + (threadIdx.x & 63);
        if (role > 1 || v >= n + Q) return;
        double P[12];
#pragma unroll
        for (int q = 0; q < 12; ++q) P[q] = Ps_ext[12 * (size_t)v + q];
        if (role == 0) {
            float pinvT[12];
            ecc_host::pinv_transpose(P, pinvT);
#pragma unroll
            for (int q = 0; q < 12; ++q) PinvTs[12 * (size_t)v + q] = pinvT[q];
        } else {
            float C[4];
            ecc_host::source_position(P, C);
#pragma unroll
            for (int q = 0; q < 4; ++q) Cs[4 * (size_t)v + q] = C[q];
        }
        return;
    }
    const int k = blockIdx.x;
    const int o0 = in.off[k], c = in.off[k + 1] - o0;
    if ((int)threadIdx.x < c) {
        M[threadIdx.x] = in.views[o0 + threadIdx.x];
        lists_d[n_poses + 1 + o0 + threadIdx.x] = M[threadIdx.x];
    }
    if (threadIdx.x == 0) {
        lists_d[k] = o0;
        if (k == n_poses - 1) lists_d[n_poses] = o0 + c;
    }
    __syncthreads();
    for (int e = threadIdx.x; e < c * n; e += 256) {
        const int a = e / n, u = e - a * n, v = M[a];
        bool hole = u == v;
        int pu = u;
        for (int b = 0; b < c; ++b)
            if (M[b] == u) {
                if (b < a) hole = true;
                else pu = n + o0 + b;
            }
        int4 t = make_int4(0, 0, 0, 0);
        if (!hole) {
            const int pv = n + o0 + a;
            t = u < v ? make_int4(pu, pv, u, v) : make_int4(pv, pu, v, u);
        }
        reinterpret_cast<int4*>(idx)[(size_t)u * Q + o0 + a] = t;
    }
}

template <int SLICES>
__global__ __launch_bounds__(SUM_THREADS) void sum_poses_kernel(const float* __restrict__ base, long long count, int n, int Q,
                                                                const int32_t* __restrict__ lists_d, int n_poses,
                                                                const float* __restrict__ vals, double* __restrict__ partial,
                                                                double* __restrict__ out_host)
{
    __shared__ float stage[4 * STAGE_F4];
    __shared__ float tail[4];
    __shared__ int M[ECC_POSE_BATCH_MAX_MOVED];
    __shared__ double s[SUM_THREADS / 64];
    const int k = blockIdx.y, slice = blockIdx.x, t = threadIdx.x;
    const int o0 = lists_d[k], c = lists_d[k + 1] - o0;
    if (t < c) M[t] = lists_d[n_poses + 1 + o0 + t];
    const long long n4 = count >> 2;
    long long lo, hi;
    ecc_sum::slice_bounds(n4, SLICES, slice, &lo, &hi);
    const bool owns_tail = slice == SLICES - 1;
    const float4* __restrict__ b4 = reinterpret_cast<const float4*>(base);
    ecc_sum::Acc4 a;
    if (owns_tail && t < 4) tail[t] = (n4 << 2) + t < count ? base[(n4 << 2) + t] : 0.f;
    bool first_chunk = true;
    for (long long c0 = lo; c0 < hi || first_chunk; c0 += STAGE_F4) {
        const long long ce = min(hi, c0 + STAGE_F4);
        for (long long kk = c0 + t; kk < ce; kk += SUM_THREADS) reinterpret_cast<float4*>(stage)[kk - c0] = b4[kk];
        __syncthreads();
        for (int e = t; e < c * n; e += SUM_THREADS) {
            const int a = e / n, u = e - a * n, v = M[a];
            bool hole = u == v;
            for (int b = 0; b < a; ++b) hole = hole || M[b] == u;
            if (hole) continue;
            const long long i = u < v ? u : v, j = u < v ? v : u;
            const long long ij = i * n - i * (i + 1) / 2 + (j - i - 1);
            const bool in_chunk = ij >= (c0 << 2) && ij < (ce << 2);
            const bool in_tail = owns_tail && first_chunk && ij >= (n4 << 2);
            if (in_chunk || in_tail) {
                const float val = vals[(size_t)u * Q + o0 + a];
                if (in_chunk) stage[ij - (c0 << 2)] = val;
                else tail[ij - (n4 << 2)] = val;
            }
        }
        __syncthreads();
        for (long long kk = c0 + t; kk < ce; kk += SUM_THREADS) ecc_sum::add(a, reinterpret_cast<const float4*>(stage)[kk - c0]);
        __syncthreads();
        first_chunk = false;
    }
    double acc = ecc_sum::combine(a);
    if (owns_tail && t == 0) ecc_sum::add_tail(acc, tail, n4, count);
    ecc_sum::stage_wave_sums(acc, s);
    if (t == 0) {
        const double part = ecc_sum::waves_in_order(s);
        if (SLICES == 1)
            __hip_atomic_store(reinterpret_cast<unsigned long long*>(out_host) + k, (unsigned long long)__double_as_longlong(part),
                               __ATOMIC_RELAXED, __HIP_MEMORY_SCOPE_SYSTEM);
        else partial[(size_t)k * SLICES + slice] = part;
    }
}

__global__ __launch_bounds__(256) void finish_poses_kernel(const double* __restrict__ partial, int slices, int n_poses,
                                                           double* __restrict__ out_host)
{
    const int k = blockIdx.x * blockDim.x + threadIdx.x;
    if (k >= n_poses) return;
    double tot = 0.0;
    for (int b = 0; b < slices; ++b) tot += partial[(size_t)k * slices + b];
    __hip_atomic_store(reinterpret_cast<unsigned long long*>(out_host) + k, (unsigned long long)__double_as_longlong(tot),
                       __ATOMIC_RELAXED, __HIP_MEMORY_SCOPE_SYSTEM);
}

double clock_now() { return std::chrono::duration<double>(std::chrono::steady_clock::now().time_since_epoch()).count(); }
constexpr uint64_t POSE_PENDING = 0x7ff8ecc0dead0002ull;

size_t align64(size_t x) { return (x + 63) & ~(size_t)63; }

struct PoseBlock {
    size_t Ps, out, off, views, end;
};
PoseBlock pose_block(int64_t n, int K, int Q, int result_words)
{
    PoseBlock b;
    b.Ps = 0;
    b.out = align64(sizeof(double) * 12 * (size_t)(n + Q));
    b.off = b.out + align64(sizeof(double) * (size_t)result_words);
    b.views = b.off + align64(sizeof(int32_t) * (size_t)(K + 1));
    b.end = b.views + align64(sizeof(int32_t) * (size_t)std::max(Q, 1));
    return b;
}

}
namespace ecc_internal {
void arm_pose_results(volatile uint64_t* out, int K)
{
    for (int k = 0; k < K; ++k) out[k] = POSE_PENDING;
    std::atomic_thread_fence(std::memory_order_seq_cst);
}

int wait_pose_results(ecc_ctx* ctx, volatile uint64_t* out, int K, double* sums, const char* batch_noun)
{
    double t0 = 0.0;
    for (unsigned spins = 0;; ++spins) {
        int k = K - 1;
        while (k >= 0 && out[k] != POSE_PENDING) --k;
        if (k < 0) break;
        if ((spins & 0xfff) == 0xfff) {
            const double t = clock_now();
            if (t0 == 0.0) t0 = t;
            else if (t - t0 > 2.0) {
                HIP_TRY(hipStreamSynchronize(ctx->stream));
                for (k = 0; k < K; ++k)
                    if (out[k] == POSE_PENDING) return fail(ECC_ERR_HIP, std::string("the ") + batch_noun + " batch ran and stored no result");
                break;
            }
        }
    }
    std::atomic_thread_fence(std::memory_order_acquire);
    for (int k = 0; k < K; ++k) {
        const uint64_t bits = out[k];
        std::memcpy(&sums[k], &bits, sizeof(double));
    }
    return ECC_OK;
}

int sum_poses(ecc_metric* m, const float* base_vals_d, int K, int Q, volatile uint64_t* out, double* out_dev, double* sums)
{
    ecc_ctx* ctx = m->ctx;
    const int64_t n = m->n_views, n_pairs = n * (n - 1) / 2;
    arm_pose_results(out, K);
    const int slices = ecc_sum::slices(n_pairs, m->sum_scratch_d.ptr != nullptr);
    hipLaunchKernelGGL(slices == 1 ? sum_poses_kernel<1> : sum_poses_kernel<SUM_SLICES>, dim3((unsigned)slices, (unsigned)K), dim3(SUM_THREADS), 0,
                       ctx->stream, base_vals_d, (long long)n_pairs, (int)n, Q, m->pose_lists_d.ptr, K, m->pose_values_d.ptr,
                       m->pose_partial_d.ptr, out_dev);
    HIP_TRY(hipGetLastError());
    if (slices > 1) {
        hipLaunchKernelGGL(finish_poses_kernel, dim3((unsigned)((K + 255) / 256)), dim3(256), 0, ctx->stream, m->pose_partial_d.ptr, slices, K, out_dev);
        HIP_TRY(hipGetLastError());
    }
    return wait_pose_results(ctx, out, K, sums);
}

bool pose_keeps_radius(const ecc_metric* m, double base_radius, int c, const int32_t* views, const double* moved_Ps)
{
    if (m->object_radius_mm > 0 || c < 1 || views[0] != 0) return true;
    return (float)ecc_host::object_radius(moved_Ps, m->n_u, m->n_v) == (float)base_radius;
}

int stage_pose_grid(ecc_metric* m, const double* base, int K, const int32_t* off, const int32_t* views, const double* moved_Ps,
                    int result_words, volatile uint64_t** out, double** out_dev)
{
    ecc_ctx* ctx = m->ctx;
    const int64_t n = m->n_views;
    const int Q = off[K];
    const int64_t entries = n * (int64_t)Q;
    const PoseBlock b = pose_block(n, K, Q, result_words);
    int rc = m->pose_h.ensure((int64_t)b.end, 1 << 16, ctx->stream);
    if (rc) return rc;
    char* const pose_h = m->pose_h.host;
    double* Ps_ext = reinterpret_cast<double*>(pose_h + b.Ps);
    std::memcpy(Ps_ext, base, sizeof(double) * 12 * (size_t)n);
    if (Q > 0) std::memcpy(Ps_ext + 12 * (size_t)n, moved_Ps, sizeof(double) * 12 * (size_t)Q);
    std::memcpy(pose_h + b.off, off, sizeof(int32_t) * (size_t)(K + 1));
    if (Q > 0) std::memcpy(pose_h + b.views, views, sizeof(int32_t) * (size_t)Q);
    std::atomic_thread_fence(std::memory_order_seq_cst);
    *out = reinterpret_cast<volatile uint64_t*>(pose_h + b.out);
    *out_dev = reinterpret_cast<double*>(m->pose_h.dev + b.out);

    rc = m->pose_PinvTs_d.ensure(12 * (n + Q), ctx->stream);
    if (!rc) rc = m->pose_Cs_d.ensure(4 * (n + Q), ctx->stream);
    if (!rc) rc = m->pose_idx_d.ensure(4 * std::max<int64_t>(entries, 1), ctx->stream);
    if (!rc) rc = m->pose_records_d.ensure(std::max<int64_t>(entries, 1), ctx->stream);
    if (!rc) rc = m->pose_lists_d.ensure((int64_t)K + 1 + std::max(Q, 1), ctx->stream);
    return rc;
}

hipError_t launch_pose_list(ecc_metric* m, int K, int Q, int result_words)
{
    const int64_t n = m->n_views;
    const PoseBlock b = pose_block(n, K, Q, result_words);
    const char* const pose_h_dev = m->pose_h.dev;
    PoseLists in = {reinterpret_cast<const int32_t*>(pose_h_dev + b.off), reinterpret_cast<const int32_t*>(pose_h_dev + b.views)};
    const unsigned e1_blocks = n * (int64_t)Q > 0 ? (unsigned)((n + Q + 63) / 64) : 0u;
    hipLaunchKernelGGL(pose_list_kernel, dim3((unsigned)K + e1_blocks), dim3(256), 0, m->ctx->stream, in, (int)n, K, Q, m->pose_idx_d.ptr,
                       m->pose_lists_d.ptr, reinterpret_cast<const double*>(pose_h_dev + b.Ps), m->pose_PinvTs_d.ptr, m->pose_Cs_d.ptr);
    return hipGetLastError();
}
}
namespace {

int run_batch(ecc_metric* m, const double* base, const float* base_vals_d, int K, const int32_t* off, const int32_t* views,
              const double* moved_Ps, double* sums)
{
    ecc_ctx* ctx = m->ctx;
    const int64_t n = m->n_views, n_pairs = n * (n - 1) / 2;
    const int Q = off[K];
    const int64_t entries = n * (int64_t)Q;
    volatile uint64_t* out = nullptr;
    double* out_dev = nullptr;
    int rc = stage_pose_grid(m, base, K, off, views, moved_Ps, K, &out, &out_dev);
    if (!rc) rc = m->pose_values_d.ensure(std::max<int64_t>(entries, 1), ctx->stream);
    if (!rc) rc = m->pose_partial_d.ensure((int64_t)K * SUM_SLICES, ctx->stream);
    if (rc) return rc;

    EccPairParams p;
    rc = fill_pair_params(m, &p, n_pairs, false);
    if (rc) return rc;
    HIP_TRY(launch_pose_list(m, K, Q, K));
    if (entries > 0) {
        p.PinvTs = m->pose_PinvTs_d.ptr;
        p.Cs = m->pose_Cs_d.ptr;
        p.indices = m->pose_idx_d.ptr;
        p.records = m->pose_records_d.ptr;
        p.pair_values = m->pose_values_d.ptr;
        p.first = 0;
        p.count = entries;
        HIP_TRY(ecc_launch_k01(&p, ctx->stream));
        HIP_TRY(launch_pairs_timed(ctx, &p));
    }
    return sum_poses(m, base_vals_d, K, Q, out, out_dev, sums);
}

int poses_two_deep(ecc_metric* m, const std::vector<int>& which, const double* Ps_batch, int n_views, double* means)
{
    ecc_ctx* ctx = m->ctx;
    const int64_t n = n_views, n_pairs = n * (n - 1) / 2;
    const int count = (int)which.size();
    if (count == 0) return ECC_OK;
    int rc = ECC_OK;
    if (m->incremental || !m->sum_h.host || n_pairs <= ECC_SMALL_EVAL_MAX_PAIRS) {
        for (int q = 0; q < count; ++q) {
            rc = ecc_metric_set_projections(m, Ps_batch + (size_t)12 * n * which[q], n_views);
            if (rc) return rc;
            rc = ecc_metric_evaluate_all(m, nullptr, &means[which[q]]);
            if (rc) return rc;
        }
        return ECC_OK;
    }
    rc = m->pair_values_d.ensure(n_pairs, ctx->stream);
    if (rc) return rc;
    volatile uint64_t* slots = reinterpret_cast<volatile uint64_t*>(m->sum_h.host);
    uint64_t gen_of[2] = {0, 0};
    auto collect = [&](int q) -> int {
        const int sl = q & 1;
        double t0 = 0.0;
        for (unsigned spins = 0;; ++spins) {
            const uint64_t bits = slots[sl];
            if (bits != POSE_PENDING) {
                double v;
                std::memcpy(&v, &bits, sizeof(v));
                means[which[q]] = v / (double)n_pairs;
                m->done_generation = gen_of[sl];
                return ECC_OK;
            }
            if ((spins & 0xfff) == 0xfff) {
                const double t = clock_now();
                if (t0 == 0.0) t0 = t;
                else if (t - t0 > 2.0) {
                    HIP_TRY(hipStreamSynchronize(ctx->stream));
                    if (slots[sl] == POSE_PENDING) return fail(ECC_ERR_HIP, "an evaluation ran and stored no result");
                }
            }
        }
    };
    for (int q = 0; q < count; ++q) {
        rc = ecc_metric_set_projections(m, Ps_batch + (size_t)12 * n * which[q], n_views);
        if (rc) return rc;
        const int sl = q & 1;
        slots[sl] = POSE_PENDING;
        std::atomic_thread_fence(std::memory_order_seq_cst);
        gen_of[sl] = m->set_generation;
        rc = launch_range(m, 0, n_pairs, m->pair_values_d.ptr, nullptr, nullptr, m->sum_h.dev + sl, false);
        if (rc) return rc;
        m->small_pending_count = 0;
        if (q >= 1) {
            rc = collect(q - 1);
            if (rc) return rc;
        }
    }
    rc = collect(count - 1);
    if (rc) return rc;
    m->last_evaluated_pairs = n_pairs;
    return ECC_OK;
}

int evaluate_deltas(ecc_metric* m, int n_poses, const int32_t* off, const int32_t* views, const double* moved_Ps, double* means,
                    std::vector<int>* not_batched)
{
    ecc_ctx* ctx = m->ctx;
    const int64_t n = m->n_views, n_pairs = n * (n - 1) / 2;
    ecc_mark_busy(m);
    const double* Pcur = m->Ps_h[m->set_generation & 1].host;
    std::vector<double> base(Pcur, Pcur + 12 * n);
    double base_radius = 0.0;
    ecc_metric_get_object_radius(m, &base_radius);
    float* base_vals_d = nullptr;
    int rc = evaluate_cached(m, 0, n_pairs, nullptr, &base_vals_d);
    if (rc) return rc;
    std::vector<double> sums;
    const int64_t max_cols = std::max<int64_t>(ECC_POSE_BATCH_MAX_ENTRIES / n, ECC_POSE_BATCH_MAX_MOVED);
    rc = ecc_pose_batches::pack(
        n_poses, off, views, moved_Ps, max_cols, POSE_BATCH_MAX_POSES,
        [&](int c, const int32_t* vk, const double* Pk) { return pose_keeps_radius(m, base_radius, c, vk, Pk); },
        [&](const ecc_pose_batches::Batch& b) -> int {
            sums.resize(b.pose.size());
            const int e = run_batch(m, base.data(), base_vals_d, (int)b.pose.size(), b.off.data(), b.views.data(), b.Ps.data(), sums.data());
            if (e) return e;
            for (size_t q = 0; q < b.pose.size(); ++q) means[b.pose[q]] = sums[q] / (double)n_pairs;
            m->last_batched_poses += (int64_t)b.pose.size();
            return ECC_OK;
        },
        not_batched);
    if (rc) return rc;
    HIP_TRY(wait_stream_spin(ctx->stream));
    m->quiet = true;
    return ECC_OK;
}

}
namespace ecc_internal {
int check_lists(const ecc_metric* m, int n_poses, const int32_t* off, const int32_t* views)
{
    if (off[0] != 0) return fail(ECC_ERR_INVALID_ARGUMENT, "moved_offsets[0] must be 0");
    for (int k = 0; k < n_poses; ++k) {
        if (off[k + 1] < off[k]) return fail(ECC_ERR_INVALID_ARGUMENT, "moved_offsets must not decrease");
        for (int q = off[k]; q < off[k + 1]; ++q) {
            if (views[q] < 0 || views[q] >= m->n_views) return fail(ECC_ERR_INVALID_ARGUMENT, "moved view outside [0, n_views)");
            if (q > off[k] && views[q] <= views[q - 1])
                return fail(ECC_ERR_INVALID_ARGUMENT, "the moved views of a pose must be strictly ascending");
        }
    }
    return ECC_OK;
}

int pose_deltas_sequential(ecc_metric* m, const std::vector<int>& rest, const int32_t* off, const int32_t* views, const double* moved_Ps,
                           const std::function<int(int)>& evaluate_pose)
{
    if (rest.empty()) return ECC_OK;
    const int64_t n = m->n_views;
    const double* Pcur = m->Ps_h[m->set_generation & 1].host;
    const std::vector<double> base(Pcur, Pcur + 12 * n);
    std::vector<double> full(base);
    int rc = ECC_OK;
    for (int k : rest) {
        for (int q = off[k]; q < off[k + 1]; ++q) std::memcpy(full.data() + 12 * (size_t)views[q], moved_Ps + 12 * (size_t)q, sizeof(double) * 12);
        rc = ecc_metric_set_projections(m, full.data(), (int)n);
        if (!rc) rc = evaluate_pose(k);
        if (rc) break;
        for (int q = off[k]; q < off[k + 1]; ++q)
            std::memcpy(full.data() + 12 * (size_t)views[q], base.data() + 12 * (size_t)views[q], sizeof(double) * 12);
    }
    const int rb = ecc_metric_set_projections(m, base.data(), (int)n);
    return rc ? rc : rb;
}
}

ECC_EXPORT int ecc_metric_set_pose_batching(ecc_metric* m, int on)
{
    if (!m) return fail(ECC_ERR_INVALID_ARGUMENT, "metric is null");
    m->pose_batching = on ? 1 : 0;
    return ECC_OK;
}

ECC_EXPORT int ecc_metric_last_batched_poses(const ecc_metric* m, int64_t* poses)
{
    if (!m || !poses) return fail(ECC_ERR_INVALID_ARGUMENT, "null argument");
    *poses = m->last_batched_poses;
    return ECC_OK;
}

ECC_EXPORT int ecc_metric_evaluate_pose_deltas(ecc_metric* m, int n_poses, const int32_t* moved_offsets, const int32_t* moved_views,
                                               const double* moved_Ps, double* means)
{
    if (!m || !moved_offsets || !means) return fail(ECC_ERR_INVALID_ARGUMENT, "null argument");
    if (n_poses < 1) return ECC_OK;
    if (moved_offsets[n_poses] > 0 && (!moved_views || !moved_Ps)) return fail(ECC_ERR_INVALID_ARGUMENT, "null argument");
    if (m->n_views < 2) return fail(ECC_ERR_INVALID_ARGUMENT, "need at least two views (the reference divides 0/0 here)");
    if ((int)m->dtrs.size() < m->n_views) return fail(ECC_ERR_INVALID_ARGUMENT, "fewer Radon intermediates than projection matrices");
    int rc = set_device(m->ctx);
    if (rc) return rc;
    rc = check_lists(m, n_poses, moved_offsets, moved_views);
    if (rc) return rc;
    m->last_batched_poses = 0;
    std::vector<int> rest;
    if (m->pose_batching) {
        rc = evaluate_deltas(m, n_poses, moved_offsets, moved_views, moved_Ps, means, &rest);
        if (rc) return rc;
    } else {
        for (int k = 0; k < n_poses; ++k) rest.push_back(k);
    }
    return pose_deltas_sequential(m, rest, moved_offsets, moved_views, moved_Ps,
                                  [&](int k) { return ecc_metric_evaluate_all(m, nullptr, &means[k]); });
}

ECC_EXPORT int ecc_metric_evaluate_poses_strided(ecc_metric* m, int n_poses, const double* Ps_batch, int n_views, int first, int stride,
                                                 double* means)
{
    if (m) ecc_mark_busy(m);
    if (!m || !Ps_batch || !means) return fail(ECC_ERR_INVALID_ARGUMENT, "null argument");
    if (first < 0 || stride < 1) return fail(ECC_ERR_INVALID_ARGUMENT, "first must be >= 0 and stride >= 1");
    if (n_poses < 1 || first >= n_poses) return ECC_OK;
    if (n_views < 2) return fail(ECC_ERR_INVALID_ARGUMENT, "need at least two views (the reference divides 0/0 here)");
    int rc = set_device(m->ctx);
    if (rc) return rc;
    m->last_batched_poses = 0;
    const int64_t n = n_views;
    const size_t pose_doubles = 12 * (size_t)n;
    std::vector<int> mine;
    for (int p = first; p < n_poses; p += stride) mine.push_back(p);
    const int last = mine.back();
    if (!m->pose_batching || mine.size() < 2) return poses_two_deep(m, mine, Ps_batch, n_views, means);

    ecc_pose_diff::Result d;
    std::vector<int32_t>&off = d.off, &views = d.views;
    std::vector<int>&batch_pose = d.batch_pose, &rest = d.rest;
    auto diff_against = [&](const double* base) { ecc_pose_diff::diff(Ps_batch, n_views, mine, base, ECC_POSE_BATCH_MAX_MOVED, 8, &d); };
    bool have_base = m->n_views == n_views && m->set_generation > 0 && (int)m->dtrs.size() >= n_views;
    if (have_base) diff_against(m->Ps_h[m->set_generation & 1].host);
    if (!have_base || 2 * batch_pose.size() < mine.size()) {
        if ((int)m->dtrs.size() < n_views) return fail(ECC_ERR_INVALID_ARGUMENT, "fewer Radon intermediates than projection matrices");
        diff_against(Ps_batch + pose_doubles * (size_t)mine[0]);
        if (2 * batch_pose.size() < mine.size()) return poses_two_deep(m, mine, Ps_batch, n_views, means);
        rc = ecc_metric_set_projections(m, Ps_batch + pose_doubles * (size_t)mine[0], n_views);
        if (rc) return rc;
    }
    std::vector<double> moved_Ps(12 * views.size());
    std::vector<double> batch_means(batch_pose.size());
    for (size_t b = 0; b < batch_pose.size(); ++b)
        for (int q = off[b]; q < off[b + 1]; ++q)
            std::memcpy(moved_Ps.data() + 12 * (size_t)q, Ps_batch + pose_doubles * (size_t)batch_pose[b] + 12 * (size_t)views[q], sizeof(double) * 12);
    std::vector<int> unbatched;
    rc = evaluate_deltas(m, (int)batch_pose.size(), off.data(), views.data(), moved_Ps.data(), batch_means.data(), &unbatched);
    if (rc) return rc;
    for (size_t b = 0; b < batch_pose.size(); ++b) means[batch_pose[b]] = batch_means[b];
    for (int b : unbatched) rest.push_back(batch_pose[b]);
    std::sort(rest.begin(), rest.end());
    rc = poses_two_deep(m, rest, Ps_batch, n_views, means);
    if (rc) return rc;
    if (rest.empty() || rest.back() != last) rc = ecc_metric_set_projections(m, Ps_batch + pose_doubles * (size_t)last, n_views);
    return rc;
}

ECC_EXPORT int ecc_metric_evaluate_poses(ecc_metric* m, int n_poses, const double* Ps_batch, int n_views, double* means)
{
    return ecc_metric_evaluate_poses_strided(m, n_poses, Ps_batch, n_views, 0, 1, means);
}
```

include/ecc_hip.h:

```cpp
#ifndef ECC_HIP_H
#define ECC_HIP_H

#include <stdint.h>

#ifdef __cplusplus
extern "C" {
#endif

#define ECC_HIP_VERSION 100

enum {
    ECC_OK = 0,
    ECC_ERR_INVALID_ARGUMENT = 1,
    ECC_ERR_HIP = 2,
    ECC_ERR_OUT_OF_MEMORY = 3,
    ECC_ERR_NO_DEVICE = 4,
    ECC_ERR_UNSUPPORTED = 5
};

enum { ECC_FILTER_DERIVATIVE = 0, ECC_FILTER_RAMP = 1, ECC_FILTER_NONE = 2 };
enum { ECC_POST_IDENTITY = 0, ECC_POST_SQUARE_ROOT = 1, ECC_POST_LOGARITHM = 2 };

typedef struct ecc_ctx ecc_ctx;
typedef struct ecc_dtr ecc_dtr;
typedef struct ecc_metric ecc_metric;

const char* ecc_last_error(void);
int ecc_version(void);
int ecc_device_count(void);


int ecc_ctx_create(int device, void* stream, ecc_ctx** out);
int ecc_ctx_destroy(ecc_ctx* ctx);
int ecc_ctx_synchronize(ecc_ctx* ctx);

int ecc_radon_compute(ecc_ctx* ctx, const float* image, int image_on_device, int n_u, int n_v,
                      int n_alpha, int n_t, int filter, int post_process, ecc_dtr** out);

int ecc_radon_compute_batch(ecc_ctx* ctx, const float* images, int images_on_device, int n, int n_u,
                            int n_v, int n_alpha, int n_t, int filter, int post_process,
                            ecc_dtr** out);

int ecc_radon_compute_into(ecc_ctx* ctx, const float* images_d, int n, int n_u, int n_v, int n_alpha,
                           int n_t, int filter, int post_process, float* slabs_d);

enum { ECC_RADON_EXACT = 0, ECC_RADON_FMA = 1 };
int ecc_radon_set_arithmetic(ecc_ctx* ctx, int mode);
int ecc_radon_get_arithmetic(const ecc_ctx* ctx, int* mode);

int ecc_radon_compute_linear(ecc_ctx* ctx, const float* image_d, int n_u, int n_v, int n_alpha, int n_t, int filter,
                             int post_process, float* out_linear_d);
int ecc_dtr_from_device_linear(ecc_ctx* ctx, const float* data_d, int n_alpha, int n_t, int n_u, int n_v, int filter,
                               ecc_dtr** out);

int ecc_dtr_from_host(ecc_ctx* ctx, const float* data, int n_alpha, int n_t, int n_u, int n_v,
                      int filter, ecc_dtr** out);
int ecc_dtr_readback(ecc_dtr* dtr, float* host_out);
int ecc_dtr_info(const ecc_dtr* dtr, int* n_alpha, int* n_t, int* n_u, int* n_v, int* filter,
                 double* bin_size_angle, double* bin_size_distance);
int ecc_dtr_device_view(const ecc_dtr* dtr, float** base, int* pitch, int* rows);
int64_t ecc_dtr_slab_floats(int n_alpha, int n_t);
int ecc_dtr_wrap_device(ecc_ctx* ctx, float* base, int n_alpha, int n_t, int n_u, int n_v, int filter,
                        ecc_dtr** out);
int ecc_dtr_destroy(ecc_dtr* dtr);

typedef struct ecc_line_weights_config { int32_t dilate_px; int32_t guard_bins; float zero_at_px; } ecc_line_weights_config;
void ecc_line_weights_defaults(ecc_line_weights_config* cfg);
int ecc_radon_line_weights(ecc_ctx* ctx, const float* flagged, int on_device, int n, int n_u, int n_v,
                           int n_alpha, int n_t, const ecc_line_weights_config* cfg, ecc_dtr** out);
int ecc_radon_line_weights_into(ecc_ctx* ctx, const float* flagged_d, int n, int n_u, int n_v,
                                int n_alpha, int n_t, const ecc_line_weights_config* cfg, float* slabs_d);
int ecc_dtr_line_weights(ecc_ctx* ctx, const ecc_dtr* lengths, const ecc_line_weights_config* cfg, ecc_dtr** out);

typedef struct ecc_preprocess_config {
    int32_t process;
    int32_t normalize;
    double bias, scale;
    int32_t apply_log;
    double gaussian_sigma;
    int32_t half_kernel_width;
    int32_t flip_u, flip_v;
    int32_t zero[4];
    int32_t feather[4];
    int32_t n_blanks;
    const int32_t* blanks;
} ecc_preprocess_config;
void ecc_preprocess_defaults(ecc_preprocess_config* cfg);

int ecc_preprocess(ecc_ctx* ctx, const float* images, int on_device, float* out, int n, int n_u, int n_v,
                   const ecc_preprocess_config* cfg, const double* Ps);
void ecc_host_intrinsics(const double* P, float* sdd_px, float* ppu, float* ppv);

int ecc_metric_create(ecc_ctx* ctx, int n_dtrs, ecc_dtr* const* dtrs, ecc_metric** out);
int ecc_metric_destroy(ecc_metric* m);
int ecc_metric_refresh_dtrs(ecc_metric* m, int first, int count);

int ecc_metric_set_projections(ecc_metric* m, const double* Ps, int n_views);
int ecc_metric_evaluate_external(ecc_metric* m, int num_Ps, const float* Cs_d, const float* PinvTs_d, int num_pairs,
                                 const int32_t* indices_d, float* K01s_d, float* out_d, float object_radius_mm, float dkappa,
                                 int use_corr);
int ecc_metric_debug_geometry(ecc_metric* m, float* PinvTs, float* Cs);

int ecc_metric_set_params(ecc_metric* m, double object_radius_mm, double dkappa, int use_corr);
enum { ECC_SAMPLING_AUTO = 0, ECC_SAMPLING_POLYNOMIAL = 1, ECC_SAMPLING_PER_SAMPLE = 2, ECC_SAMPLING_REFERENCE = 3 };
#define ECC_SAMPLING_AUTO_REFERENCE_PAIRS 512
int ecc_metric_set_sampling(ecc_metric* m, int mode);
int ecc_metric_set_incremental(ecc_metric* m, int enable);
int ecc_metric_last_evaluated_pairs(const ecc_metric* m, int64_t* pairs);
#define ECC_RECORD_REUSE_MIN_PAIRS 4096
#ifndef ECC_RECORD_REUSE_SPLIT_PAIRS
#define ECC_RECORD_REUSE_SPLIT_PAIRS 8192
#endif
int ecc_metric_set_record_reuse(ecc_metric* m, int on);
int ecc_metric_set_host_join(ecc_metric* m, int on);

int ecc_metric_set_small_eval(ecc_metric* m, int on);
int ecc_metric_get_object_radius(const ecc_metric* m, double* radius_mm);

int ecc_metric_evaluate_all(ecc_metric* m, float* cost_nxn, double* mean);
int ecc_metric_evaluate_pose_deltas(ecc_metric* m, int n_poses, const int32_t* moved_offsets, const int32_t* moved_views,
                                    const double* moved_Ps, double* means);
int ecc_metric_evaluate_poses(ecc_metric* m, int n_poses, const double* Ps_batch, int n_views, double* means);
int ecc_metric_evaluate_poses_strided(ecc_metric* m, int n_poses, const double* Ps_batch, int n_views, int first, int stride,
                                      double* means);
int ecc_metric_set_pose_batching(ecc_metric* m, int on);
int ecc_metric_last_batched_poses(const ecc_metric* m, int64_t* poses);

int ecc_metric_evaluate_gradient(ecc_metric* m, int view, int n_params, const double* Ps_plus, const double* Ps_minus,
                                 const double* h, double* value, double* grad, double* probes);
int ecc_metric_last_gradient_path(const ecc_metric* m, int* path);

#define ECC_GRAM_MAX_CHANNELS 4
int ecc_metric_evaluate_gram(ecc_metric* m, int n_channels, float* pair_grams, double* gram);

#define ECC_VIEW_COEFF_MAX_CHANNELS 4
int ecc_metric_evaluate_view_coefficients(ecc_metric* m, int n_channels, const float* coeffs,
                                          double* value, double* grad, float* pair_terms);

#define ECC_VIEW_HESSIAN_MAX_CHANNELS 4
#define ECC_VIEW_HESSIAN_MAX_DIM 8192
int ecc_metric_evaluate_view_hessian(ecc_metric* m, int n_channels, double* hessian, double* pair_blocks);

int ecc_metric_evaluate_weighted(ecc_metric* m, double* value, double* coverage, float* pair_terms);

int ecc_metric_evaluate_weighted_pairs(ecc_metric* m, const int32_t* idx4, int n_pairs, double* value, double* coverage, float* pair_terms);
int ecc_metric_evaluate_weighted_pose_deltas(ecc_metric* m, int n_poses, const int32_t* moved_offsets, const int32_t* moved_views,
                                             const double* moved_Ps, double* values, double* coverages);

int ecc_metric_evaluate_transforms(ecc_metric* m, int n_source, int n_transforms, const double* Ts, double* means,
                                   float* pair_values);
int ecc_metric_last_batched_transforms(const ecc_metric* m, int64_t* transforms);
void ecc_host_compose_transform(const double* P12, const double* T16, double* out12);

int ecc_metric_evaluate_weighted_transforms(ecc_metric* m, int n_source, int n_transforms, const double* Ts, double* values,
                                            double* coverages, float* pair_terms);

enum { ECC_LOSS_HUBER = 0, ECC_LOSS_TRUNCATED = 1, ECC_LOSS_GEMAN_MCCLURE = 2 };
int ecc_metric_evaluate_robust(ecc_metric* m, int loss, float delta, double* value, double* inlier_mass, float* pair_terms);
int ecc_metric_evaluate_robust_pairs(ecc_metric* m, const int32_t* idx4, int n_pairs, int loss, float delta, double* value,
                                     double* inlier_mass, float* pair_terms);
double ecc_host_robust_scale(const float* pair_terms, int64_t n_pairs, double k);

int ecc_metric_evaluate_robust_map(ecc_metric* m, int loss, float delta, const int32_t* views, int n_mapped, float* hits, float* rejected,
                                   double* value, double* inlier_mass, float* pair_terms);
int ecc_metric_evaluate_robust_map_pairs(ecc_metric* m, const int32_t* idx4, int n_pairs, int loss, float delta, const int32_t* views,
                                         int n_mapped, float* hits, float* rejected, double* value, double* inlier_mass, float* pair_terms);
int ecc_metric_robust_map_weights(ecc_metric* m, float min_hits, float gain, ecc_dtr** out);
int ecc_debug_robust_map_fixed(ecc_metric* m, uint64_t* out, int64_t capacity);

int ecc_metric_evaluate_robust_pose_deltas(ecc_metric* m, int n_poses, const int32_t* moved_offsets, const int32_t* moved_views,
                                           const double* moved_Ps, int loss, float delta, double* values, double* inlier_masses);
int ecc_metric_evaluate_robust_transforms(ecc_metric* m, int n_source, int n_transforms, const double* Ts, int loss, float delta,
                                          double* values, double* inlier_masses, float* pair_terms);

int ecc_metric_evaluate_weighted_robust(ecc_metric* m, int loss, float delta, double* value, double* coverage,
                                        double* inlier_mass, float* pair_terms);
int ecc_metric_evaluate_weighted_robust_pairs(ecc_metric* m, const int32_t* idx4, int n_pairs, int loss, float delta,
                                              double* value, double* coverage, double* inlier_mass, float* pair_terms);
double ecc_host_weighted_robust_scale(const float* pair_terms, int64_t n_pairs, double k);

int ecc_metric_evaluate_weighted_robust_map(ecc_metric* m, int loss, float delta, const int32_t* views, int n_mapped,
        float* hits, float* rejected, double* value, double* coverage, double* inlier_mass, float* pair_terms);
int ecc_metric_evaluate_weighted_robust_map_pairs(ecc_metric* m, const int32_t* idx4, int n_pairs, int loss, float delta,
        const int32_t* views, int n_mapped, float* hits, float* rejected,
        double* value, double* coverage, double* inlier_mass, float* pair_terms);
int ecc_metric_weighted_robust_map_weights(ecc_metric* m, float min_hits, float gain, ecc_dtr** out);

int ecc_metric_evaluate_range(ecc_metric* m, int64_t first, int64_t count, float* pair_values,
                              double* partial_sum);

int ecc_metric_evaluate_range_async(ecc_metric* m, int64_t first, int64_t count,
                                    float* pair_values_d, double* sum_d);

int ecc_metric_publish_scalar(ecc_metric* m, const double* value_d);
int ecc_metric_wait_scalar(ecc_metric* m, double* value);

int ecc_metric_evaluate_pairs(ecc_metric* m, const int32_t* idx4, int n_pairs, float* out,
                              double* mean);

int ecc_metric_pair_samples_bound(const ecc_metric* m, int* capacity);
int ecc_metric_evaluate_for_image_pair(ecc_metric* m, int i, int j, int capacity, int* n_samples,
                                       float* redundant_samples0, float* redundant_samples1, float* kappas,
                                       float* radon_samples0, float* radon_samples1, float* K01,
                                       double* ecc);

int ecc_metric_debug_K01(ecc_metric* m, int64_t first, int64_t count, float* K01s);

typedef struct ecc_direct ecc_direct;
int ecc_direct_create(ecc_ctx* ctx, int n_images, const float* images, int on_device, int n_u, int n_v,
                      ecc_direct** out);
int ecc_direct_destroy(ecc_direct* d);
int ecc_direct_update_images(ecc_direct* d);
int ecc_direct_set_projections(ecc_direct* d, const double* Ps, int n_views);
int ecc_direct_set_params(ecc_direct* d, double object_radius_mm, double dkappa, int use_fbcc);
int ecc_direct_get_object_radius(const ecc_direct* d, double* radius_mm);
int ecc_direct_evaluate(ecc_direct* d, float* cost_nxn, double* cost_sum);
int ecc_direct_lines_bound(const ecc_direct* d, int* capacity);
int ecc_direct_evaluate_for_image_pair(ecc_direct* d, int i, int j, int capacity, int* n_lines,
                                       float* redundant_samples0, float* redundant_samples1, float* kappas,
                                       float* lines01, double* metric);

int ecc_direct_evaluate_for_image_pair_kappas(ecc_direct* d, int i, int j, int n_kappas, const float* kappas_in,
                                              float* redundant_samples0, float* redundant_samples1, float* lines01,
                                              double* metric);

#define ECC_POLY_RECORD_FLOATS (4 + 2 * 13 + 2 * 12)
int ecc_metric_debug_polynomials(ecc_metric* m, int64_t first, int64_t count, float* out);

void ecc_get_ij(int64_t ij, int n, int* i, int* j);
void ecc_host_pinvT(const double* P, float* PinvT12);
void ecc_host_source_position(const double* P, float* C4);
double ecc_host_object_radius(const double* P, int n_u, int n_v);

int ecc_host_line_to_sample_dtr(float* line3, float range_t);

void ecc_host_angular_range(const double* P0, const double* P1, double object_radius_mm, double* kappa_first,
                            double* kappa_second);
double ecc_host_angular_step(const double* P0, const double* P1, int n_u, int n_v);
void ecc_host_iso_center(const double* Ps, int n_views, double* O);

typedef struct ecc_group ecc_group;
typedef struct ecc_group_metric ecc_group_metric;
int ecc_group_create(int n_dev, const int* devices, ecc_group** out);
int ecc_group_destroy(ecc_group* g);
int ecc_group_size(const ecc_group* g);
int ecc_group_ctx(ecc_group* g, int rank, ecc_ctx** ctx);
int ecc_group_radon_compute_batch(ecc_group* g, const float* images, int n, int n_u, int n_v, int n_alpha, int n_t,
                                  int filter, int post_process, ecc_dtr** out);
void ecc_pair_shard(int64_t n_pairs, int world, int rank, int64_t* first, int64_t* count);
int ecc_pair_shards_balanced(const double* Ps, int n_views, double object_radius_mm, int world, int64_t* bounds);
int ecc_metric_balanced_shards(ecc_metric* m, int world, int64_t* bounds);

int ecc_group_metric_create(ecc_group* g, int n_dtrs, ecc_dtr* const* dtrs, ecc_group_metric** out);
int ecc_group_debug_force_replica(int on);
int ecc_group_metric_destroy(ecc_group_metric* gm);
int ecc_group_metric_set_projections(ecc_group_metric* gm, const double* Ps, int n_views);
int ecc_group_metric_set_params(ecc_group_metric* gm, double object_radius_mm, double dkappa, int use_corr);
int ecc_group_metric_set_incremental(ecc_group_metric* gm, int enable);
int ecc_group_metric_set_sampling(ecc_group_metric* gm, int mode);
int ecc_group_metric_get_object_radius(ecc_group_metric* gm, double* radius_mm);
int ecc_group_metric_evaluate_all(ecc_group_metric* gm, float* cost_nxn, double* mean);
int ecc_group_metric_evaluate_poses(ecc_group_metric* gm, int n_poses, const double* Ps_batch, int n_views, double* means);
int ecc_group_metric_rebalance(ecc_group_metric* gm);
int ecc_group_metric_rank_metric(ecc_group_metric* gm, int rank, ecc_metric** m);

typedef struct ecc_comm ecc_comm;
#define ECC_COMM_ID_BYTES 128
int ecc_comm_available(void);
int ecc_comm_unique_id(void* id128);
int ecc_comm_create(ecc_ctx* ctx, const void* id128, int rank, int world, ecc_comm** out);
int ecc_comm_destroy(ecc_comm* c);
int ecc_metric_evaluate_range_allreduce(ecc_metric* m, ecc_comm* comm, int64_t first, int64_t count, double* sum_all);
#define ECC_EXCHANGE_MAX_RANKS 64
typedef struct ecc_exchange ecc_exchange;
int ecc_exchange_open(const char* name, int rank, int world, ecc_exchange** out);
int ecc_exchange_sum(ecc_exchange* ex, double partial, double* total);
int ecc_exchange_close(ecc_exchange* ex);

int ecc_ctx_enable_timing(ecc_ctx* ctx, int enable);
int ecc_ctx_last_kernel_ms(ecc_ctx* ctx, int which, float* ms);

#define ECC_POLY_ECONOMISE_TOL_BINS 2e-8f
int ecc_debug_set_poly_tolerance(ecc_metric* m, float tol_bins);
int ecc_debug_set_small_eval_bound(ecc_metric* m, int64_t max_pairs);
int ecc_debug_set_result_polling(int on);
int ecc_debug_set_quad_copies(ecc_ctx* ctx, int on);
int ecc_debug_set_gradient_launch(ecc_metric* m, int on);
#define ECC_QUAD_COPIES_AUTO (-1)
#define ECC_QUAD_COPIES_OFF 0
#define ECC_QUAD_COPIES_ON 1
int ecc_ctx_set_quad_copies(ecc_ctx* ctx, int mode);
int ecc_metric_device_bytes(const ecc_metric* m, int64_t* paired_bytes, int64_t* quad_bytes, int64_t* other_bytes);
int ecc_debug_small_stamps(unsigned long long* out, int n_blocks);
#define ECC_STEP_STAMPS 9
int ecc_debug_step_stamps(const ecc_metric* m, double* out);

#ifdef __cplusplus
}
#endif
#endif
```

Before: 3172.

## Pipeline host pose diffing with GPU pose-batch evaluation in slot ring

```diff
diff --git a/epipolarconsistency_amd/_lib.py b/epipolarconsistency_amd/_lib.py
--- a/epipolarconsistency_amd/_lib.py
+++ b/epipolarconsistency_amd/_lib.py
@@ -169,6 +169,7 @@
     "ecc_debug_set_result_polling": (_i, [_i]),
     "ecc_debug_set_quad_copies": (_i, [_vp, _i]),
     "ecc_debug_set_gradient_launch": (_i, [_vp, _i]),
+    "ecc_debug_set_pose_pipeline": (_i, [_vp, _i, _i]),
     "ecc_ctx_set_quad_copies": (_i, [_vp, _i]),
     "ecc_debug_small_stamps": (_i, [_vp, _i]),
     "ecc_debug_step_stamps": (_i, [_vp, _vp]),
diff --git a/epipolarconsistency_amd/api.py b/epipolarconsistency_amd/api.py
--- a/epipolarconsistency_amd/api.py
+++ b/epipolarconsistency_amd/api.py
@@ -408,6 +408,14 @@
             check(_lib.lib().ecc_debug_set_small_eval_bound(self._h, int(self._debug["small_eval_bound"])))
         if "gradient_launch" in self._debug:
             check(_lib.lib().ecc_debug_set_gradient_launch(self._h, int(self._debug["gradient_launch"])))
+        if "pose_pipeline" in self._debug:
+            check(_lib.lib().ecc_debug_set_pose_pipeline(self._h, *self._debug["pose_pipeline"]))
+
+    def debugSetPosePipeline(self, run_poses, group_poses):
+        self._debug["pose_pipeline"] = (int(run_poses), int(group_poses))
+        if self._h:
+            self._apply_debug()
+        return self
 
     def debugSetGradientLaunch(self, on=True):
         self._debug["gradient_launch"] = 1 if on else 0
diff --git a/epipolarconsistency_amd/csrc/ecc_capi.hip b/epipolarconsistency_amd/csrc/ecc_capi.hip
--- a/epipolarconsistency_amd/csrc/ecc_capi.hip
+++ b/epipolarconsistency_amd/csrc/ecc_capi.hip
@@ -221,6 +221,7 @@
     if (ctx->line_weights_scratch_d) (void)hipFree(ctx->line_weights_scratch_d);
     for (auto& e : ctx->ev)
         if (e) (void)hipEventDestroy(e);
+    for (hipEvent_t e : ctx->group_ev) (void)hipEventDestroy(e);
     delete ctx;
     return ECC_OK;
 }
@@ -261,6 +262,7 @@
             if (!e) HIP_TRY(hipEventCreate(&e));
     ctx->timing = enable != 0;
     ctx->ev_valid[0] = ctx->ev_valid[1] = ctx->ev_valid[2] = false;
+    ctx->group_ms_valid = false;
     return ECC_OK;
 }
 
@@ -270,6 +272,10 @@
     if (!ctx->timing || !ctx->ev_valid[which]) return fail(ECC_ERR_INVALID_ARGUMENT, "no timed launch recorded");
     int rc = set_device(ctx);
     if (rc) return rc;
+    if (which == 0 && ctx->group_ms_valid) {
+        *ms = ctx->group_ms;
+        return ECC_OK;
+    }
     HIP_TRY(hipEventSynchronize(ctx->ev[2 * which + 1]));
     HIP_TRY(hipEventElapsedTime(ms, ctx->ev[2 * which], ctx->ev[2 * which + 1]));
     return ECC_OK;
diff --git a/epipolarconsistency_amd/csrc/ecc_capi_internal.h b/epipolarconsistency_amd/csrc/ecc_capi_internal.h
--- a/epipolarconsistency_amd/csrc/ecc_capi_internal.h
+++ b/epipolarconsistency_amd/csrc/ecc_capi_internal.h
@@ -21,6 +21,7 @@
 #include "ecc_host_geometry.h"
 #include "ecc_layout.h"
 #include "ecc_view_changes.h"
+#include "ecc_worker_pool.h"
 
 extern "C" hipError_t ecc_launch_radon(const EccRadonParams* p, int derivative, hipStream_t stream);
 extern "C" hipError_t ecc_launch_dtr_border(float* slabs, int64_t slab_stride, int n_img, int n_alpha, int n_t,
@@ -110,6 +111,9 @@
     int quad_copies = ECC_QUAD_COPIES_AUTO;
     hipEvent_t ev[6] = {nullptr, nullptr, nullptr, nullptr, nullptr, nullptr};
     bool ev_valid[3] = {false, false, false};
+    std::vector<hipEvent_t> group_ev;
+    float group_ms = 0.f;
+    bool group_ms_valid = false;
     float* trig_d = nullptr;
     int trig_n_alpha = 0;
     double* ramp_d = nullptr;
@@ -172,6 +176,14 @@
         if (e != hipSuccess) ptr = nullptr;
         cap = e == hipSuccess ? n : 0;
         return e;
+    }
+    int ensure_grown(int64_t need, hipStream_t stream)
+    {
+        if (cap >= need && ptr) return ECC_OK;
+        const int64_t grown = std::max(need, cap + cap / 2);
+        int rc = ensure(grown, stream);
+        if (rc == ECC_ERR_OUT_OF_MEMORY && grown > need) rc = ensure(need, stream);
+        return rc;
     }
     int64_t bytes() const { return cap * (int64_t)sizeof(T); }
 };
@@ -332,6 +344,8 @@
     DeviceArray<float> pose_values_d;
     DeviceArray<double> pose_partial_d;
     DeviceArray<int32_t> pose_lists_d;
+    std::unique_ptr<EccWorkerPool> pose_pool;
+    int pipeline_run_poses = 0, pipeline_group_poses = 0;
     int64_t last_batched_poses = 0;
     int gradient_launch = 0;
     int last_gradient_path = 0;
@@ -383,12 +397,21 @@
                  bool synchronous = false, bool host_join = false);
 int evaluate_cached(ecc_metric* m, int64_t first, int64_t count, double* sum_d, float** vals_out);
 
+struct PoseSlot {
+    int64_t h = 0;
+    int64_t geom = 0;
+    int64_t entries = 0;
+    int64_t lists = 0;
+    int64_t partial = 0;
+};
+int queue_sum_poses(ecc_metric* m, const float* base_vals_d, int K, int Q, volatile uint64_t* out, double* out_dev,
+                    const PoseSlot& at = PoseSlot());
 int sum_poses(ecc_metric* m, const float* base_vals_d, int K, int Q, volatile uint64_t* out, double* out_dev, double* sums);
 bool pose_keeps_radius(const ecc_metric* m, double base_radius, int c, const int32_t* views, const double* moved_Ps);
 int check_lists(const ecc_metric* m, int n_poses, const int32_t* off, const int32_t* views);
 int stage_pose_grid(ecc_metric* m, const double* base, int K, const int32_t* off, const int32_t* views, const double* moved_Ps,
-                    int result_words, volatile uint64_t** out, double** out_dev);
-hipError_t launch_pose_list(ecc_metric* m, int K, int Q, int result_words);
+                    int result_words, volatile uint64_t** out, double** out_dev, const PoseSlot& at = PoseSlot());
+hipError_t launch_pose_list(ecc_metric* m, int K, int Q, int result_words, const PoseSlot& at = PoseSlot());
 void arm_pose_results(volatile uint64_t* out, int K);
 int wait_pose_results(ecc_ctx* ctx, volatile uint64_t* out, int K, double* sums, const char* batch_noun = "pose");
 int pose_deltas_sequential(ecc_metric* m, const std::vector<int>& rest, const int32_t* off, const int32_t* views, const double* moved_Ps,
@@ -420,6 +443,7 @@
     if (ctx->timing) {
         const hipError_t e = hipEventRecord(ctx->ev[0], ctx->stream);
         if (e != hipSuccess) return e;
+        ctx->group_ms_valid = false;
     }
     const hipError_t e = launch(ctx->stream);
     if (e != hipSuccess || !ctx->timing) return e;
diff --git a/epipolarconsistency_amd/csrc/ecc_pose_diff.h b/epipolarconsistency_amd/csrc/ecc_pose_diff.h
--- a/epipolarconsistency_amd/csrc/ecc_pose_diff.h
+++ b/epipolarconsistency_amd/csrc/ecc_pose_diff.h
@@ -2,8 +2,10 @@
 #define ECC_POSE_DIFF_H
 
 #include <algorithm>
+#include <atomic>
 #include <cstdint>
 #include <cstring>
+#include <memory>
 #include <thread>
 #include <vector>
 
@@ -16,33 +18,38 @@
     std::vector<int> rest;
 };
 
+constexpr size_t SINGLE_THREAD_BYTES = (size_t)4 << 20;
+
+inline int32_t compare_pose(const double* Pp, const double* base, int n_views, int max_moved, std::vector<int32_t>* pv)
+{
+    const size_t before = pv->size();
+    for (int v0 = 0; v0 < n_views && pv->size() - before <= (size_t)max_moved; v0 += 8) {
+        const int v1 = std::min(n_views, v0 + 8);
+        if (std::memcmp(Pp + 12 * (size_t)v0, base + 12 * (size_t)v0, sizeof(double) * 12 * (size_t)(v1 - v0)) == 0) continue;
+        for (int v = v0; v < v1; ++v)
+            if (std::memcmp(Pp + 12 * (size_t)v, base + 12 * (size_t)v, sizeof(double) * 12) != 0) pv->push_back(v);
+    }
+    if (pv->size() - before > (size_t)max_moved) {
+        pv->resize(before);
+        return -1;
+    }
+    return (int32_t)(pv->size() - before);
+}
+
 inline void diff(const double* Ps_batch, int n_views, const std::vector<int>& mine, const double* base, int max_moved,
                  unsigned max_threads, Result* out)
 {
     const size_t pose_doubles = 12 * (size_t)n_views, count = mine.size();
     const size_t bytes = count * pose_doubles * sizeof(double);
     const unsigned hw = std::max(1u, std::thread::hardware_concurrency());
-    const size_t T = (bytes < ((size_t)4 << 20) || max_threads < 2) ? 1 : std::min<size_t>({(size_t)max_threads, (size_t)hw, count / 32 + 1});
+    const size_t T = (bytes < SINGLE_THREAD_BYTES || max_threads < 2) ? 1 : std::min<size_t>({(size_t)max_threads, (size_t)hw, count / 32 + 1});
     std::vector<std::vector<int32_t>> part_views(T);
     std::vector<std::vector<int32_t>> part_count(T);
     auto work = [&](size_t t) {
         const size_t lo = count * t / T, hi = count * (t + 1) / T;
         std::vector<int32_t>&pv = part_views[t], &pc = part_count[t];
         pc.reserve(hi - lo);
-        for (size_t q = lo; q < hi; ++q) {
-            const double* Pp = Ps_batch + pose_doubles * (size_t)mine[q];
-            const size_t before = pv.size();
-            for (int v0 = 0; v0 < n_views && pv.size() - before <= (size_t)max_moved; v0 += 8) {
-                const int v1 = std::min(n_views, v0 + 8);
-                if (std::memcmp(Pp + 12 * (size_t)v0, base + 12 * (size_t)v0, sizeof(double) * 12 * (size_t)(v1 - v0)) == 0) continue;
-                for (int v = v0; v < v1; ++v)
-                    if (std::memcmp(Pp + 12 * (size_t)v, base + 12 * (size_t)v, sizeof(double) * 12) != 0) pv.push_back(v);
-            }
-            if (pv.size() - before > (size_t)max_moved) {
-                pv.resize(before);
-                pc.push_back(-1);
-            } else pc.push_back((int32_t)(pv.size() - before));
-        }
+        for (size_t q = lo; q < hi; ++q) pc.push_back(compare_pose(Ps_batch + pose_doubles * (size_t)mine[q], base, n_views, max_moved, &pv));
     };
     if (T == 1) work(0);
     else {
@@ -71,6 +78,88 @@
     }
 }
 
+struct Run {
+    std::vector<int32_t> count;
+    std::vector<int32_t> views;
+    std::vector<double> Ps;
+    int small = 0;
+};
+
+class Runs {
+public:
+    void start(const double* Ps_batch, int n_views, const std::vector<int>* mine, const double* base, int max_moved, size_t run_len)
+    {
+        Ps_batch_ = Ps_batch;
+        n_views_ = n_views;
+        mine_ = mine;
+        base_ = base;
+        max_moved_ = max_moved;
+        run_len_ = std::max<size_t>(run_len, 1);
+        const size_t R = (mine->size() + run_len_ - 1) / run_len_;
+        runs_.assign(R, Run());
+        done_.reset(new std::atomic<int>[std::max<size_t>(R, 1)]);
+        for (size_t r = 0; r < R; ++r) done_[r].store(0, std::memory_order_relaxed);
+        next_.store(0, std::memory_order_release);
+    }
+    size_t n_runs() const { return runs_.size(); }
+    size_t lo(size_t r) const { return r * run_len_; }
+    size_t hi(size_t r) const { return std::min(mine_->size(), (r + 1) * run_len_); }
+
+    bool work_one()
+    {
+        const size_t r = next_.fetch_add(1, std::memory_order_acq_rel);
+        if (r >= runs_.size()) return false;
+        Run& run = runs_[r];
+        const size_t pose_doubles = 12 * (size_t)n_views_;
+        run.count.reserve(hi(r) - lo(r));
+        for (size_t q = lo(r); q < hi(r); ++q) {
+            const double* Pp = Ps_batch_ + pose_doubles * (size_t)(*mine_)[q];
+            const size_t before = run.views.size();
+            const int32_t c = compare_pose(Pp, base_, n_views_, max_moved_, &run.views);
+            run.count.push_back(c);
+            if (c < 0) continue;
+            ++run.small;
+            for (size_t e = before; e < run.views.size(); ++e) run.Ps.insert(run.Ps.end(), Pp + 12 * (size_t)run.views[e], Pp + 12 * (size_t)run.views[e] + 12);
+        }
+        done_[r].store(1, std::memory_order_release);
+        return true;
+    }
+    void work()
+    {
+        while (work_one()) {}
+    }
+    void cancel() { next_.store(runs_.size(), std::memory_order_release); }
+    const Run* published(size_t r) const { return done_[r].load(std::memory_order_acquire) ? &runs_[r] : nullptr; }
+
+    void append(size_t r, Result* out, std::vector<double>* moved_Ps) const
+    {
+        const Run& run = runs_[r];
+        size_t at = 0;
+        for (size_t q = 0; q < run.count.size(); ++q) {
+            const int32_t c = run.count[q];
+            const int pose = (*mine_)[lo(r) + q];
+            if (c < 0) out->rest.push_back(pose);
+            else {
+                out->views.insert(out->views.end(), run.views.begin() + at, run.views.begin() + at + c);
+                at += (size_t)c;
+                out->batch_pose.push_back(pose);
+                out->off.push_back((int32_t)out->views.size());
+            }
+        }
+        moved_Ps->insert(moved_Ps->end(), run.Ps.begin(), run.Ps.end());
+    }
+
+private:
+    const double* Ps_batch_ = nullptr;
+    const double* base_ = nullptr;
+    const std::vector<int>* mine_ = nullptr;
+    int n_views_ = 0, max_moved_ = 0;
+    size_t run_len_ = 1;
+    std::vector<Run> runs_;
+    std::unique_ptr<std::atomic<int>[]> done_;
+    std::atomic<size_t> next_{0};
+};
+
 }
 
 #endif
diff --git a/epipolarconsistency_amd/csrc/ecc_poses.hip b/epipolarconsistency_amd/csrc/ecc_poses.hip
--- a/epipolarconsistency_amd/csrc/ecc_poses.hip
+++ b/epipolarconsistency_amd/csrc/ecc_poses.hip
@@ -192,21 +192,28 @@
     return ECC_OK;
 }
 
-int sum_poses(ecc_metric* m, const float* base_vals_d, int K, int Q, volatile uint64_t* out, double* out_dev, double* sums)
+int queue_sum_poses(ecc_metric* m, const float* base_vals_d, int K, int Q, volatile uint64_t* out, double* out_dev, const PoseSlot& at)
 {
     ecc_ctx* ctx = m->ctx;
     const int64_t n = m->n_views, n_pairs = n * (n - 1) / 2;
     arm_pose_results(out, K);
     const int slices = ecc_sum::slices(n_pairs, m->sum_scratch_d.ptr != nullptr);
+    double* const partial = m->pose_partial_d.ptr + at.partial;
     hipLaunchKernelGGL(slices == 1 ? sum_poses_kernel<1> : sum_poses_kernel<SUM_SLICES>, dim3((unsigned)slices, (unsigned)K), dim3(SUM_THREADS), 0,
-                       ctx->stream, base_vals_d, (long long)n_pairs, (int)n, Q, m->pose_lists_d.ptr, K, m->pose_values_d.ptr,
-                       m->pose_partial_d.ptr, out_dev);
+                       ctx->stream, base_vals_d, (long long)n_pairs, (int)n, Q, m->pose_lists_d.ptr + at.lists, K,
+                       m->pose_values_d.ptr + at.entries, partial, out_dev);
     HIP_TRY(hipGetLastError());
     if (slices > 1) {
-        hipLaunchKernelGGL(finish_poses_kernel, dim3((unsigned)((K + 255) / 256)), dim3(256), 0, ctx->stream, m->pose_partial_d.ptr, slices, K, out_dev);
+        hipLaunchKernelGGL(finish_poses_kernel, dim3((unsigned)((K + 255) / 256)), dim3(256), 0, ctx->stream, partial, slices, K, out_dev);
         HIP_TRY(hipGetLastError());
     }
-    return wait_pose_results(ctx, out, K, sums);
+    return ECC_OK;
+}
+
+int sum_poses(ecc_metric* m, const float* base_vals_d, int K, int Q, volatile uint64_t* out, double* out_dev, double* sums)
+{
+    const int rc = queue_sum_poses(m, base_vals_d, K, Q, out, out_dev);
+    return rc ? rc : wait_pose_results(m->ctx, out, K, sums);
 }
 
 bool pose_keeps_radius(const ecc_metric* m, double base_radius, int c, const int32_t* views, const double* moved_Ps)
@@ -216,16 +223,16 @@
 }
 
 int stage_pose_grid(ecc_metric* m, const double* base, int K, const int32_t* off, const int32_t* views, const double* moved_Ps,
-                    int result_words, volatile uint64_t** out, double** out_dev)
+                    int result_words, volatile uint64_t** out, double** out_dev, const PoseSlot& at)
 {
     ecc_ctx* ctx = m->ctx;
     const int64_t n = m->n_views;
     const int Q = off[K];
     const int64_t entries = n * (int64_t)Q;
     const PoseBlock b = pose_block(n, K, Q, result_words);
-    int rc = m->pose_h.ensure((int64_t)b.end, 1 << 16, ctx->stream);
-    if (rc) return rc;
-    char* const pose_h = m->pose_h.host;
+    int rc = m->pose_h.ensure(at.h + (int64_t)b.end, 1 << 16, ctx->stream);
+    if (rc) return rc;
+    char* const pose_h = m->pose_h.host + at.h;
     double* Ps_ext = reinterpret_cast<double*>(pose_h + b.Ps);
     std::memcpy(Ps_ext, base, sizeof(double) * 12 * (size_t)n);
     if (Q > 0) std::memcpy(Ps_ext + 12 * (size_t)n, moved_Ps, sizeof(double) * 12 * (size_t)Q);
@@ -233,60 +240,78 @@
     if (Q > 0) std::memcpy(pose_h + b.views, views, sizeof(int32_t) * (size_t)Q);
     std::atomic_thread_fence(std::memory_order_seq_cst);
     *out = reinterpret_cast<volatile uint64_t*>(pose_h + b.out);
-    *out_dev = reinterpret_cast<double*>(m->pose_h.dev + b.out);
-
-    rc = m->pose_PinvTs_d.ensure(12 * (n + Q), ctx->stream);
-    if (!rc) rc = m->pose_Cs_d.ensure(4 * (n + Q), ctx->stream);
-    if (!rc) rc = m->pose_idx_d.ensure(4 * std::max<int64_t>(entries, 1), ctx->stream);
-    if (!rc) rc = m->pose_records_d.ensure(std::max<int64_t>(entries, 1), ctx->stream);
-    if (!rc) rc = m->pose_lists_d.ensure((int64_t)K + 1 + std::max(Q, 1), ctx->stream);
+    *out_dev = reinterpret_cast<double*>(m->pose_h.dev + at.h + b.out);
+
+    rc = m->pose_PinvTs_d.ensure_grown(12 * (at.geom + n + Q), ctx->stream);
+    if (!rc) rc = m->pose_Cs_d.ensure_grown(4 * (at.geom + n + Q), ctx->stream);
+    if (!rc) rc = m->pose_idx_d.ensure_grown(4 * (at.entries + std::max<int64_t>(entries, 1)), ctx->stream);
+    if (!rc) rc = m->pose_records_d.ensure_grown(at.entries + std::max<int64_t>(entries, 1), ctx->stream);
+    if (!rc) rc = m->pose_lists_d.ensure_grown(at.lists + (int64_t)K + 1 + std::max(Q, 1), ctx->stream);
     return rc;
 }
 
-hipError_t launch_pose_list(ecc_metric* m, int K, int Q, int result_words)
+hipError_t launch_pose_list(ecc_metric* m, int K, int Q, int result_words, const PoseSlot& at)
 {
     const int64_t n = m->n_views;
     const PoseBlock b = pose_block(n, K, Q, result_words);
-    const char* const pose_h_dev = m->pose_h.dev;
+    const char* const pose_h_dev = m->pose_h.dev + at.h;
     PoseLists in = {reinterpret_cast<const int32_t*>(pose_h_dev + b.off), reinterpret_cast<const int32_t*>(pose_h_dev + b.views)};
     const unsigned e1_blocks = n * (int64_t)Q > 0 ? (unsigned)((n + Q + 63) / 64) : 0u;
-    hipLaunchKernelGGL(pose_list_kernel, dim3((unsigned)K + e1_blocks), dim3(256), 0, m->ctx->stream, in, (int)n, K, Q, m->pose_idx_d.ptr,
-                       m->pose_lists_d.ptr, reinterpret_cast<const double*>(pose_h_dev + b.Ps), m->pose_PinvTs_d.ptr, m->pose_Cs_d.ptr);
+    hipLaunchKernelGGL(pose_list_kernel, dim3((unsigned)K + e1_blocks), dim3(256), 0, m->ctx->stream, in, (int)n, K, Q,
+                       m->pose_idx_d.ptr + 4 * at.entries, m->pose_lists_d.ptr + at.lists, reinterpret_cast<const double*>(pose_h_dev + b.Ps),
+                       m->pose_PinvTs_d.ptr + 12 * at.geom, m->pose_Cs_d.ptr + 4 * at.geom);
     return hipGetLastError();
 }
 }
 namespace {
 
-int run_batch(ecc_metric* m, const double* base, const float* base_vals_d, int K, const int32_t* off, const int32_t* views,
-              const double* moved_Ps, double* sums)
+int queue_batch(ecc_metric* m, const double* base, const float* base_vals_d, int K, const int32_t* off, const int32_t* views,
+                const double* moved_Ps, const PoseSlot& at, int group, volatile uint64_t** out)
 {
     ecc_ctx* ctx = m->ctx;
     const int64_t n = m->n_views, n_pairs = n * (n - 1) / 2;
     const int Q = off[K];
     const int64_t entries = n * (int64_t)Q;
-    volatile uint64_t* out = nullptr;
     double* out_dev = nullptr;
-    int rc = stage_pose_grid(m, base, K, off, views, moved_Ps, K, &out, &out_dev);
-    if (!rc) rc = m->pose_values_d.ensure(std::max<int64_t>(entries, 1), ctx->stream);
-    if (!rc) rc = m->pose_partial_d.ensure((int64_t)K * SUM_SLICES, ctx->stream);
+    int rc = stage_pose_grid(m, base, K, off, views, moved_Ps, K, out, &out_dev, at);
+    if (!rc) rc = m->pose_values_d.ensure_grown(at.entries + std::max<int64_t>(entries, 1), ctx->stream);
+    if (!rc) rc = m->pose_partial_d.ensure_grown(at.partial + (int64_t)K * SUM_SLICES, ctx->stream);
     if (rc) return rc;
 
     EccPairParams p;
     rc = fill_pair_params(m, &p, n_pairs, false);
     if (rc) return rc;
-    HIP_TRY(launch_pose_list(m, K, Q, K));
+    HIP_TRY(launch_pose_list(m, K, Q, K, at));
     if (entries > 0) {
-        p.PinvTs = m->pose_PinvTs_d.ptr;
-        p.Cs = m->pose_Cs_d.ptr;
-        p.indices = m->pose_idx_d.ptr;
-        p.records = m->pose_records_d.ptr;
-        p.pair_values = m->pose_values_d.ptr;
+        p.PinvTs = m->pose_PinvTs_d.ptr + 12 * at.geom;
+        p.Cs = m->pose_Cs_d.ptr + 4 * at.geom;
+        p.indices = m->pose_idx_d.ptr + 4 * at.entries;
+        p.records = m->pose_records_d.ptr + at.entries;
+        p.pair_values = m->pose_values_d.ptr + at.entries;
         p.first = 0;
         p.count = entries;
         HIP_TRY(ecc_launch_k01(&p, ctx->stream));
-        HIP_TRY(launch_pairs_timed(ctx, &p));
-    }
-    return sum_poses(m, base_vals_d, K, Q, out, out_dev, sums);
+        if (group < 0 || !ctx->timing) HIP_TRY(launch_pairs_timed(ctx, &p));
+        else {
+            while ((int)ctx->group_ev.size() < 2 * (group + 1)) {
+                hipEvent_t e = nullptr;
+                HIP_TRY(hipEventCreate(&e));
+                ctx->group_ev.push_back(e);
+            }
+            HIP_TRY(hipEventRecord(ctx->group_ev[2 * group], ctx->stream));
+            HIP_TRY(ecc_launch_pairs(&p, ctx->stream));
+            HIP_TRY(hipEventRecord(ctx->group_ev[2 * group + 1], ctx->stream));
+        }
+    }
+    return queue_sum_poses(m, base_vals_d, K, Q, *out, out_dev, at);
+}
+
+int run_batch(ecc_metric* m, const double* base, const float* base_vals_d, int K, const int32_t* off, const int32_t* views,
+              const double* moved_Ps, double* sums)
+{
+    volatile uint64_t* out = nullptr;
+    const int rc = queue_batch(m, base, base_vals_d, K, off, views, moved_Ps, PoseSlot(), -1, &out);
+    return rc ? rc : wait_pose_results(m->ctx, out, K, sums);
 }
 
 int poses_two_deep(ecc_metric* m, const std::vector<int>& which, const double* Ps_batch, int n_views, double* means)
@@ -461,6 +486,259 @@
                                   [&](int k) { return ecc_metric_evaluate_all(m, nullptr, &means[k]); });
 }
 
+namespace {
+
+struct PipelinePlan {
+    size_t run_poses, group_min;
+    int threads;
+    bool exact_groups;
+};
+PipelinePlan plan_pipeline(const ecc_metric* m, size_t count, size_t pose_bytes)
+{
+    const int hw = (int)std::max(1u, std::thread::hardware_concurrency());
+    PipelinePlan pl;
+    if (m->pipeline_run_poses > 0) {
+        pl.run_poses = (size_t)m->pipeline_run_poses;
+        pl.group_min = m->pipeline_group_poses > 0 ? (size_t)m->pipeline_group_poses : count;
+        pl.threads = std::min(8, hw);
+        pl.exact_groups = true;
+    } else if (count * pose_bytes < ecc_pose_diff::SINGLE_THREAD_BYTES) {
+        pl.run_poses = pl.group_min = count;
+        pl.threads = 1;
+        pl.exact_groups = false;
+    } else {
+        pl.run_poses = std::max<size_t>(1, ((size_t)512 << 10) / pose_bytes);
+        pl.group_min = std::max<size_t>(32, (count + 3) / 4);
+        pl.threads = (int)std::min<size_t>({(size_t)8, (size_t)hw, count / 32 + 1});
+        pl.exact_groups = false;
+    }
+    return pl;
+}
+
+int64_t round_up(int64_t x, int64_t to) { return (x + to - 1) / to * to; }
+PoseSlot slot_need(int64_t n, int K, int Q)
+{
+    PoseSlot s;
+    s.h = (int64_t)pose_block(n, K, Q, K).end;
+    s.geom = n + Q;
+    s.entries = std::max<int64_t>(n * (int64_t)Q, 1);
+    s.lists = (int64_t)K + 1 + std::max(Q, 1);
+    s.partial = (int64_t)K * SUM_SLICES;
+    return s;
+}
+PoseSlot slot_behind(const PoseSlot& at, const PoseSlot& need)
+{
+    PoseSlot s;
+    s.h = at.h + need.h;
+    s.geom = round_up(at.geom + need.geom, 16);
+    s.entries = round_up(at.entries + need.entries, 64);
+    s.lists = round_up(at.lists + need.lists, 16);
+    s.partial = at.partial + need.partial;
+    return s;
+}
+bool slot_fits(const ecc_metric* m, const PoseSlot& at, const PoseSlot& need)
+{
+    return m->pose_h.cap >= at.h + need.h && m->pose_PinvTs_d.cap >= 12 * (at.geom + need.geom) && m->pose_Cs_d.cap >= 4 * (at.geom + need.geom) &&
+           m->pose_idx_d.cap >= 4 * (at.entries + need.entries) && m->pose_records_d.cap >= at.entries + need.entries &&
+           m->pose_values_d.cap >= at.entries + need.entries && m->pose_lists_d.cap >= at.lists + need.lists &&
+           m->pose_partial_d.cap >= at.partial + need.partial;
+}
+int reserve_pose_scratch(ecc_metric* m, const PoseSlot& end)
+{
+    hipStream_t s = m->ctx->stream;
+    int rc = m->pose_h.ensure(end.h, 1 << 16, s);
+    if (!rc) rc = m->pose_PinvTs_d.ensure_grown(12 * end.geom, s);
+    if (!rc) rc = m->pose_Cs_d.ensure_grown(4 * end.geom, s);
+    if (!rc) rc = m->pose_idx_d.ensure_grown(4 * end.entries, s);
+    if (!rc) rc = m->pose_records_d.ensure_grown(end.entries, s);
+    if (!rc) rc = m->pose_values_d.ensure_grown(end.entries, s);
+    if (!rc) rc = m->pose_lists_d.ensure_grown(end.lists, s);
+    if (!rc) rc = m->pose_partial_d.ensure_grown(end.partial, s);
+    return rc;
+}
+
+void cpu_relax()
+{
+#if defined(__x86_64__) || defined(__i386__)
+    __builtin_ia32_pause();
+#endif
+}
+
+struct GroupInFlight {
+    volatile uint64_t* out;
+    std::vector<int> pose;
+};
+
+int pipeline_poses(ecc_metric* m, const std::vector<int>& mine, const double* Ps_batch, int n_views, const double* base,
+                   bool base_is_first_pose, double* means, std::vector<int>* rest, bool* decided_out)
+{
+    ecc_ctx* ctx = m->ctx;
+    const int64_t n = n_views, n_pairs = n * (n - 1) / 2;
+    const size_t count = mine.size();
+    const PipelinePlan plan = plan_pipeline(m, count, sizeof(double) * 12 * (size_t)n);
+    ecc_pose_diff::Runs runs;
+    runs.start(Ps_batch, n_views, &mine, base, ECC_POSE_BATCH_MAX_MOVED, plan.run_poses);
+
+    ecc_pose_diff::Result d;
+    d.off.assign(1, 0);
+    std::vector<double> moved_Ps;
+    std::vector<int32_t> small_upto(1, 0);
+    size_t merged_runs = 0, pos = 0, queued_pos = 0;
+    bool decided = false;
+    std::vector<double> base_copy, sums;
+    double base_radius = 0.0;
+    float* base_vals_d = nullptr;
+    std::vector<GroupInFlight> flight;
+    PoseSlot at;
+    int timed_groups = 0;
+    std::vector<int32_t> group_off;
+    std::vector<int> unbatched;
+    const int64_t max_cols = std::max<int64_t>(ECC_POSE_BATCH_MAX_ENTRIES / n, ECC_POSE_BATCH_MAX_MOVED);
+
+    auto collect_all = [&]() -> int {
+        for (const GroupInFlight& g : flight) {
+            const int K = (int)g.pose.size();
+            sums.resize((size_t)K);
+            const int rc = wait_pose_results(ctx, g.out, K, sums.data());
+            if (rc) return rc;
+            for (int q = 0; q < K; ++q) means[g.pose[q]] = sums[q] / (double)n_pairs;
+            m->last_batched_poses += K;
+        }
+        flight.clear();
+        at = PoseSlot();
+        return ECC_OK;
+    };
+    auto on_decided = [&]() -> int {
+        int rc = base_is_first_pose ? ecc_metric_set_projections(m, base, n_views) : ECC_OK;
+        if (rc) return rc;
+        ecc_mark_busy(m);
+        const double* Pcur = m->Ps_h[m->set_generation & 1].host;
+        base_copy.assign(Pcur, Pcur + 12 * n);
+        ecc_metric_get_object_radius(m, &base_radius);
+        rc = evaluate_cached(m, 0, n_pairs, nullptr, &base_vals_d);
+        if (rc || plan.group_min >= count) return rc;
+        const double cols_per_pose = (double)d.off.back() / (double)std::max<size_t>(pos, 1);
+        const size_t quarter = (count + 3) / 4 + plan.run_poses;
+        PoseSlot end;
+        for (int g = 0; g < 5; ++g) end = slot_behind(end, slot_need(n, (int)quarter, (int)std::ceil(cols_per_pose * (double)quarter) + 1));
+        return reserve_pose_scratch(m, end);
+    };
+    auto queue_group = [&](size_t p0, size_t p1) -> int {
+        const int b0 = small_upto[p0], b1 = small_upto[p1];
+        if (b0 == b1) return ECC_OK;
+        group_off.resize((size_t)(b1 - b0) + 1);
+        for (int b = b0; b <= b1; ++b) group_off[(size_t)(b - b0)] = d.off[(size_t)b] - d.off[(size_t)b0];
+        const int32_t* group_views = d.views.data() + d.off[(size_t)b0];
+        const double* group_Ps = moved_Ps.data() + 12 * (size_t)d.off[(size_t)b0];
+        std::vector<int> not_batched;
+        const int rc = ecc_pose_batches::pack(
+            b1 - b0, group_off.data(), group_views, group_Ps, max_cols, POSE_BATCH_MAX_POSES,
+            [&](int c, const int32_t* vk, const double* Pk) { return pose_keeps_radius(m, base_radius, c, vk, Pk); },
+            [&](const ecc_pose_batches::Batch& b) -> int {
+                const int K = (int)b.pose.size(), Q = b.off[(size_t)K];
+                const PoseSlot need = slot_need(n, K, Q);
+                if (!flight.empty() && !slot_fits(m, at, need)) {
+                    const int e = collect_all();
+                    if (e) return e;
+                }
+                GroupInFlight g;
+                const int e = queue_batch(m, base_copy.data(), base_vals_d, K, b.off.data(), b.views.data(), b.Ps.data(), at, timed_groups, &g.out);
+                if (e) return e;
+                if (n * (int64_t)Q > 0) ++timed_groups;
+                for (int q : b.pose) g.pose.push_back(d.batch_pose[(size_t)(b0 + q)]);
+                flight.push_back(std::move(g));
+                at = slot_behind(at, need);
+                return ECC_OK;
+            },
+            &not_batched);
+        for (int q : not_batched) unbatched.push_back(d.batch_pose[(size_t)(b0 + q)]);
+        return rc;
+    };
+    auto consumer = [&]() -> int {
+        const size_t R = runs.n_runs();
+        for (;;) {
+            while (merged_runs < R && runs.published(merged_runs)) {
+                const ecc_pose_diff::Run* run = runs.published(merged_runs);
+                runs.append(merged_runs, &d, &moved_Ps);
+                int32_t small = small_upto.back();
+                for (int32_t c : run->count) small_upto.push_back(small += c >= 0 ? 1 : 0);
+                pos = runs.hi(merged_runs++);
+            }
+            const bool all = merged_runs == R;
+            if (!decided && 2 * d.batch_pose.size() >= count) {
+                decided = true;
+                const int rc = on_decided();
+                if (rc) return rc;
+            }
+            if (decided && pos > queued_pos) {
+                const size_t avail = pos - queued_pos;
+                size_t take = 0;
+                if (plan.exact_groups) take = avail >= plan.group_min || all ? std::min(avail, plan.group_min) : 0;
+                else take = queued_pos == 0 || avail >= plan.group_min || all ? avail : 0;
+                if (take > 0) {
+                    const int rc = queue_group(queued_pos, queued_pos + take);
+                    if (rc) return rc;
+                    queued_pos += take;
+                    continue;
+                }
+            }
+            if (all) return ECC_OK;
+            if ((decided && plan.threads > 1) || !runs.work_one()) cpu_relax();
+        }
+    };
+
+    int rc = ECC_OK;
+    if (plan.threads > 1) {
+        if (!m->pose_pool) {
+            m->pose_pool.reset(new EccWorkerPool());
+            m->pose_pool->start(std::min(8, (int)std::max(1u, std::thread::hardware_concurrency())), nullptr, nullptr);
+        }
+        EccWorkerPool& pool = *m->pose_pool;
+        const int threw = pool.run_all(
+            [&](int rank) -> int {
+                if (rank == 0) {
+                    rc = consumer();
+                    if (rc) runs.cancel();
+                } else if (rank < plan.threads) runs.work();
+                return 0;
+            },
+            ECC_ERR_OUT_OF_MEMORY);
+        if (threw >= 0) return fail(pool.status(threw), "the pose comparison failed: " + pool.message(threw));
+    } else rc = consumer();
+    if (rc) return rc;
+    *decided_out = decided;
+    if (!decided) return ECC_OK;
+    rc = collect_all();
+    if (rc) return rc;
+    if (ctx->timing && timed_groups > 0) {
+        float total = 0.f;
+        for (int g = 0; g < timed_groups; ++g) {
+            float ms = 0.f;
+            HIP_TRY(hipEventSynchronize(ctx->group_ev[(size_t)(2 * g + 1)]));
+            HIP_TRY(hipEventElapsedTime(&ms, ctx->group_ev[(size_t)(2 * g)], ctx->group_ev[(size_t)(2 * g + 1)]));
+            total += ms;
+        }
+        ctx->group_ms = total;
+        ctx->group_ms_valid = ctx->ev_valid[0] = true;
+    }
+    HIP_TRY(wait_stream_spin(ctx->stream));
+    m->quiet = true;
+    *rest = d.rest;
+    rest->insert(rest->end(), unbatched.begin(), unbatched.end());
+    return ECC_OK;
+}
+
+}
+
+ECC_EXPORT int ecc_debug_set_pose_pipeline(ecc_metric* m, int run_poses, int group_poses)
+{
+    if (!m) return fail(ECC_ERR_INVALID_ARGUMENT, "metric is null");
+    if (run_poses < 0 || group_poses < 0) return fail(ECC_ERR_INVALID_ARGUMENT, "run_poses and group_poses must be >= 0");
+    m->pipeline_run_poses = run_poses;
+    m->pipeline_group_poses = group_poses;
+    return ECC_OK;
+}
+
 ECC_EXPORT int ecc_metric_evaluate_poses_strided(ecc_metric* m, int n_poses, const double* Ps_batch, int n_views, int first, int stride,
                                                  double* means)
 {
@@ -479,29 +757,19 @@
     const int last = mine.back();
     if (!m->pose_batching || mine.size() < 2) return poses_two_deep(m, mine, Ps_batch, n_views, means);
 
-    ecc_pose_diff::Result d;
-    std::vector<int32_t>&off = d.off, &views = d.views;
-    std::vector<int>&batch_pose = d.batch_pose, &rest = d.rest;
-    auto diff_against = [&](const double* base) { ecc_pose_diff::diff(Ps_batch, n_views, mine, base, ECC_POSE_BATCH_MAX_MOVED, 8, &d); };
-    bool have_base = m->n_views == n_views && m->set_generation > 0 && (int)m->dtrs.size() >= n_views;
-    if (have_base) diff_against(m->Ps_h[m->set_generation & 1].host);
-    if (!have_base || 2 * batch_pose.size() < mine.size()) {
+    std::vector<int> rest;
+    bool decided = false;
+    const bool have_base = m->n_views == n_views && m->set_generation > 0 && (int)m->dtrs.size() >= n_views;
+    if (have_base) {
+        rc = pipeline_poses(m, mine, Ps_batch, n_views, m->Ps_h[m->set_generation & 1].host, false, means, &rest, &decided);
+        if (rc) return rc;
+    }
+    if (!decided) {
         if ((int)m->dtrs.size() < n_views) return fail(ECC_ERR_INVALID_ARGUMENT, "fewer Radon intermediates than projection matrices");
-        diff_against(Ps_batch + pose_doubles * (size_t)mine[0]);
-        if (2 * batch_pose.size() < mine.size()) return poses_two_deep(m, mine, Ps_batch, n_views, means);
-        rc = ecc_metric_set_projections(m, Ps_batch + pose_doubles * (size_t)mine[0], n_views);
+        rc = pipeline_poses(m, mine, Ps_batch, n_views, Ps_batch + pose_doubles * (size_t)mine[0], true, means, &rest, &decided);
         if (rc) return rc;
-    }
-    std::vector<double> moved_Ps(12 * views.size());
-    std::vector<double> batch_means(batch_pose.size());
-    for (size_t b = 0; b < batch_pose.size(); ++b)
-        for (int q = off[b]; q < off[b + 1]; ++q)
-            std::memcpy(moved_Ps.data() + 12 * (size_t)q, Ps_batch + pose_doubles * (size_t)batch_pose[b] + 12 * (size_t)views[q], sizeof(double) * 12);
-    std::vector<int> unbatched;
-    rc = evaluate_deltas(m, (int)batch_pose.size(), off.data(), views.data(), moved_Ps.data(), batch_means.data(), &unbatched);
-    if (rc) return rc;
-    for (size_t b = 0; b < batch_pose.size(); ++b) means[batch_pose[b]] = batch_means[b];
-    for (int b : unbatched) rest.push_back(batch_pose[b]);
+        if (!decided) return poses_two_deep(m, mine, Ps_batch, n_views, means);
+    }
     std::sort(rest.begin(), rest.end());
     rc = poses_two_deep(m, rest, Ps_batch, n_views, means);
     if (rc) return rc;
diff --git a/include/ecc_hip.h b/include/ecc_hip.h
--- a/include/ecc_hip.h
+++ b/include/ecc_hip.h
@@ -286,6 +286,7 @@
 int ecc_debug_set_result_polling(int on);
 int ecc_debug_set_quad_copies(ecc_ctx* ctx, int on);
 int ecc_debug_set_gradient_launch(ecc_metric* m, int on);
+int ecc_debug_set_pose_pipeline(ecc_metric* m, int run_poses, int group_poses);
 #define ECC_QUAD_COPIES_AUTO (-1)
 #define ECC_QUAD_COPIES_OFF 0
 #define ECC_QUAD_COPIES_ON 1
```

New measurement: 3188, median of 2. About the same (+0.5%).
